# rainerzufalldererste/limg

Measured on AMD Instinct MI355X. Metric: encode Mpixels/s, 8K RGBA (limg_encode3d_test-equivalent: all 11 planes stored), higher is better.
Workload: dtype u8/i32 integer stage + f32 float stage (bit-exact vs the reference's strict SSE build)

## Files before the change

include/limg_hip_test_hooks.h:

```cpp
#ifndef LIMG_HIP_TEST_HOOKS_H
#define LIMG_HIP_TEST_HOOKS_H

#include "limg_hip.h"

#ifdef __cplusplus
extern "C" {
#endif

typedef struct limg_hip_test_options
{
  uint32_t struct_size;
  int32_t record_limit;
  int32_t batch_chunk;
  int32_t wg_per_cu;
  int32_t whole_image_ragged;
  int32_t pipeline;
  int32_t fail_chain_phase1;
  int32_t blocked_no_bound;
  int32_t lookback_spins;
  int32_t base_error_strip;
  int32_t skip_publish_strip;
  int32_t blocked_no_order;
  int32_t blocked_no_vec_store;
  int32_t resize_tile_pixels;
} limg_hip_test_options;

void limg_hip_default_test_options_sized(limg_hip_test_options *pOptions, size_t structSize);
static inline void limg_hip_default_test_options(limg_hip_test_options *pOptions) { limg_hip_default_test_options_sized(pOptions, sizeof(limg_hip_test_options)); }
limg_hip_result limg_hip_set_test_options(limg_hip_context *pCtx, const limg_hip_test_options *pOptions);

void limg_hip_test_live_resources(uint64_t out[5]);

#ifdef __cplusplus
}
#endif
#endif
```

limg_amd/__init__.py:

```python
import ctypes as C
import os

import numpy as np

HERE = os.path.dirname(os.path.abspath(__file__))
TEST_LIB_PATH = os.path.join(HERE, "liblimg_hip_test.so")
LIB_PATH = os.environ.get("LIMG_HIP_LIB") or os.path.join(HERE, "liblimg_hip.so")
if LIB_PATH == "test":
    LIB_PATH = TEST_LIB_PATH

P32 = ("pDecoded", "pShiftABCX", "pColAMin", "pColAMax", "pColBMin", "pColBMax", "pColCMin", "pColCMax")
P8 = ("pFactorsA", "pFactorsB", "pFactorsC")
PLANES = P32 + P8

ABI_SYMBOLS = (
    "limg_hip_init", "limg_hip_shutdown", "limg_hip_default_options_sized", "limg_hip_set_options", "limg_hip_get_options", "limg_hip_encode3d", "limg_hip_encode3d_perf",
    "limg_hip_encode3d_stats", "limg_hip_blocked_encode3d_stats",
    "limg_hip_encode3d_device", "limg_hip_encode3d_batch_device", "limg_hip_last_stats", "limg_hip_compare", "limg_hip_compare_device", "limg_hip_synth_random_gradient_device",
    "limg_hip_synth_photo_noise_device", "limg_hip_context_device_bytes", "limg_hip_version", "limg_hip_profile_begin", "limg_hip_profile_end",
    "limg_hip_host_noise_table", "limg_hip_noise_table_device", "limg_hip_host_chain_call", "limg_hip_host_chain_checkpoints", "limg_hip_host_dense_checkpoints", "limg_hip_host_partition", "limg_hip_check_device_status",
    "limg_hip_stream_bound", "limg_hip_encode_stream_device", "limg_hip_decode_stream_device", "limg_hip_encode_stream", "limg_hip_decode_stream",
    "limg_hip_stream_info", "limg_hip_encode_stream_batch_device", "limg_hip_encode_stream_batch",
    "limg_hip_stream_sizes_device", "limg_hip_stream_sizes", "limg_hip_encode_stream_budget_device", "limg_hip_encode_stream_budget",
    "limg_hip_encode_stream_budget_batch_device", "limg_hip_encode_stream_budget_batch",
    "limg_hip_blocked_stream_bound", "limg_hip_blocked_encode_stream_device", "limg_hip_blocked_decode_stream_device", "limg_hip_blocked_encode_stream",
    "limg_hip_blocked_decode_stream", "limg_hip_blocked_stream_info", "limg_hip_blocked_last_stream",
    "limg_hip_decode_stream_window_device", "limg_hip_blocked_decode_stream_window_device", "limg_hip_decode_stream_window", "limg_hip_blocked_decode_stream_window",
    "limg_hip_decode_stream_windows_device", "limg_hip_blocked_decode_stream_windows_device", "limg_hip_decode_stream_windows", "limg_hip_blocked_decode_stream_windows",
    "limg_hip_decode_stream_windows_tensor_device", "limg_hip_blocked_decode_stream_windows_tensor_device", "limg_hip_decode_stream_windows_tensor",
    "limg_hip_blocked_decode_stream_windows_tensor",
    "limg_hip_decode_stream_windows_scaled_device", "limg_hip_blocked_decode_stream_windows_scaled_device", "limg_hip_decode_stream_windows_scaled_tensor_device",
    "limg_hip_blocked_decode_stream_windows_scaled_tensor_device", "limg_hip_decode_stream_windows_scaled", "limg_hip_blocked_decode_stream_windows_scaled",
    "limg_hip_decode_stream_windows_scaled_tensor", "limg_hip_blocked_decode_stream_windows_scaled_tensor",
    "limg_hip_decode_stream_windows_resized_device", "limg_hip_blocked_decode_stream_windows_resized_device", "limg_hip_decode_stream_windows_resized_tensor_device",
    "limg_hip_blocked_decode_stream_windows_resized_tensor_device", "limg_hip_decode_stream_windows_resized", "limg_hip_blocked_decode_stream_windows_resized",
    "limg_hip_decode_stream_windows_resized_tensor", "limg_hip_blocked_decode_stream_windows_resized_tensor",
    "limg_hip_blocked_encode3d", "limg_hip_blocked_encode3d_device", "limg_hip_blocked_regions", "limg_hip_blocked_timing", "limg_hip_blocked_kernel_timing", "limg_hip_blocked_match_bits", "limg_hip_host_blocked_matches",
    "limg_hip_host_blocked_merge", "limg_hip_host_blocked_match_words", "limg_hip_host_blocked_match_bits",
    "limg_hip_comm_unique_id", "limg_hip_comm_init", "limg_hip_comm_destroy", "limg_hip_comm_info", "limg_hip_gather_stream", "limg_hip_encode3d_single_chain_device",
    "limg_hip_encode3d_chain_device", "limg_hip_host_gather_offsets", "limg_hip_host_chain_bases",
)
TEST_ABI_SYMBOLS = ("limg_hip_default_test_options_sized", "limg_hip_set_test_options", "limg_hip_test_live_resources")
COMM_ID_BYTES = 128

BLOCKED_PLANES = (("pDecoded", np.uint32), ("pFactorsA", np.uint8), ("pFactorsB", np.uint8), ("pFactorsC", np.uint8), ("pBlockError", np.uint8), ("pBitsPerPixel", np.uint8),
                  ("pShiftABCX", np.uint32), ("pColAMin", np.uint32), ("pColAMax", np.uint32), ("pColBMin", np.uint32), ("pColBMax", np.uint32), ("pColCMin", np.uint32),
                  ("pColCMax", np.uint32), ("pBlockIndex", np.uint32))
REGION_DTYPE = np.dtype([("ox", "<u4"), ("oy", "<u4"), ("rx", "<u4"), ("ry", "<u4")])

STREAM_HEADER_DTYPE = np.dtype([("magic", "<u4"), ("version", "<u4"), ("sizeX", "<u4"), ("sizeY", "<u4"), ("channels", "<u4"), ("errorFactor", "<u4"),
                                ("blocksX", "<u4"), ("blocksY", "<u4"), ("payloadWords", "<u8"), ("totalBytes", "<u8"), ("flags", "<u4"), ("reserved", "<u4", 3)])
STREAM_BLOCK_DTYPE = np.dtype([("dirA_min", "<i2", 4), ("dirA_max", "<i2", 4), ("dirB_offset", "<i2", 4), ("dirB_mag", "<i2", 4), ("dirC_offset", "<i2", 4),
                               ("dirC_mag", "<i2", 4), ("shift", "<u4"), ("payloadWord", "<u4")])

STREAM_VERSION_BLOCKED = 2
STREAM_FLAG_MERGED = 4
STREAM_RECT_DTYPE = np.dtype([("dirA_min", "<i2", 4), ("dirA_max", "<i2", 4), ("dirB_offset", "<i2", 4), ("dirB_mag", "<i2", 4), ("dirC_offset", "<i2", 4),
                              ("dirC_mag", "<i2", 4), ("shift", "<u4"), ("payloadWord", "<u4"), ("ox", "<u2"), ("oy", "<u2"), ("rx", "<u2"), ("ry", "<u2")])

RECORD_DTYPE = np.dtype([("avg", "<f4", 4), ("dirA_min", "<i2", 4), ("dirA_max", "<i2", 4), ("dirB_offset", "<i2", 4),
                         ("dirB_mag", "<i2", 4), ("dirC_offset", "<i2", 4), ("dirC_mag", "<i2", 4)])


class LimgHipError(RuntimeError):
    pass


class Info(C.Structure):
    _fields_ = [(k, C.c_void_p) for k in PLANES]


class CompactOut(C.Structure):
    _fields_ = [("pRecords", C.c_void_p), ("pShifts", C.c_void_p)]


class Window(C.Structure):
    _fields_ = [("x0", C.c_size_t), ("y0", C.c_size_t), ("width", C.c_size_t), ("height", C.c_size_t), ("pOut", C.c_void_p), ("outStridePixels", C.c_size_t)]


class WindowJob(C.Structure):
    _fields_ = [("pStream", C.c_void_p), ("streamBytes", C.c_size_t), ("sizeX", C.c_size_t), ("sizeY", C.c_size_t), ("window", Window)]


TENSOR_F32, TENSOR_F16 = 0, 1


class TensorFormat(C.Structure):
    _fields_ = [("type", C.c_uint32), ("planes", C.c_uint32), ("scale", C.c_float * 4), ("bias", C.c_float * 4)]


class TensorWindow(C.Structure):
    _fields_ = [("x0", C.c_size_t), ("y0", C.c_size_t), ("width", C.c_size_t), ("height", C.c_size_t), ("pOut", C.c_void_p), ("rowStride", C.c_size_t),
                ("planeStride", C.c_size_t)]


class TensorWindowJob(C.Structure):
    _fields_ = [("pStream", C.c_void_p), ("streamBytes", C.c_size_t), ("sizeX", C.c_size_t), ("sizeY", C.c_size_t), ("window", TensorWindow)]


class ScaledWindow(C.Structure):
    _fields_ = Window._fields_ + [("log2Scale", C.c_uint32)]


class ScaledWindowJob(C.Structure):
    _fields_ = [("pStream", C.c_void_p), ("streamBytes", C.c_size_t), ("sizeX", C.c_size_t), ("sizeY", C.c_size_t), ("window", ScaledWindow)]


class ScaledTensorWindow(C.Structure):
    _fields_ = TensorWindow._fields_ + [("log2Scale", C.c_uint32)]


class ScaledTensorWindowJob(C.Structure):
    _fields_ = [("pStream", C.c_void_p), ("streamBytes", C.c_size_t), ("sizeX", C.c_size_t), ("sizeY", C.c_size_t), ("window", ScaledTensorWindow)]


RESIZE_AUTO, RESIZE_FLIP_X = 0xFFFFFFFF, 1


class ResizedWindow(C.Structure):
    _fields_ = Window._fields_ + [("outWidth", C.c_size_t), ("outHeight", C.c_size_t), ("log2Scale", C.c_uint32), ("flags", C.c_uint32)]


class ResizedWindowJob(C.Structure):
    _fields_ = [("pStream", C.c_void_p), ("streamBytes", C.c_size_t), ("sizeX", C.c_size_t), ("sizeY", C.c_size_t), ("window", ResizedWindow)]


class ResizedTensorWindow(C.Structure):
    _fields_ = TensorWindow._fields_ + [("outWidth", C.c_size_t), ("outHeight", C.c_size_t), ("log2Scale", C.c_uint32), ("flags", C.c_uint32)]


class ResizedTensorWindowJob(C.Structure):
    _fields_ = [("pStream", C.c_void_p), ("streamBytes", C.c_size_t), ("sizeX", C.c_size_t), ("sizeY", C.c_size_t), ("window", ResizedTensorWindow)]


_WINDOW_TYPES = {(False, False): (Window, WindowJob), (False, True): (TensorWindow, TensorWindowJob),
                 (True, False): (ScaledWindow, ScaledWindowJob), (True, True): (ScaledTensorWindow, ScaledTensorWindowJob)}


def tensor_format(dtype, planes, scale, bias):
    name = str(dtype).split(".")[-1].replace("'>", "")
    assert name in ("float32", "float16"), dtype
    scale, bias = list(scale) + [1.0] * (4 - len(scale)), list(bias) + [0.0] * (4 - len(bias))
    return TensorFormat(TENSOR_F16 if name == "float16" else TENSOR_F32, planes, (C.c_float * 4)(*scale[:4]), (C.c_float * 4)(*bias[:4]))


class BudgetResult(C.Structure):
    _fields_ = [("struct_size", C.c_uint32), ("errorFactor", C.c_uint32), ("probes", C.c_uint32), ("withinBudget", C.c_uint32), ("bytes", C.c_uint64)]


class Options(C.Structure):
    _fields_ = [("struct_size", C.c_uint32), ("forced_shift", C.c_int32 * 3), ("force_split_kernels", C.c_int32), ("dither_pcg", C.c_int32), ("float_mode", C.c_int32),
                ("legacy_float_stage", C.c_int32), ("collect_stats", C.c_int32), ("host_noise_table", C.c_int32), ("batch_sub_images", C.c_int32), ("ragged_bands", C.c_int32),
                ("ragged_walk_threads", C.c_int32)]


class TestOptions(C.Structure):
    _fields_ = [("struct_size", C.c_uint32), ("record_limit", C.c_int32), ("batch_chunk", C.c_int32), ("wg_per_cu", C.c_int32), ("whole_image_ragged", C.c_int32),
                ("pipeline", C.c_int32), ("fail_chain_phase1", C.c_int32), ("blocked_no_bound", C.c_int32), ("lookback_spins", C.c_int32), ("base_error_strip", C.c_int32),
                ("skip_publish_strip", C.c_int32), ("blocked_no_order", C.c_int32), ("blocked_no_vec_store", C.c_int32), ("resize_tile_pixels", C.c_int32)]


def load_library(path=None):
    path = path or LIB_PATH
    if not os.path.exists(path):
        raise LimgHipError("%s not built: run `python -c 'import __graft_entry__ as g; g.build()'` (hipcc, gfx950). There is no CPU fallback." % path)
    try:
        import torch
    except ImportError:
        pass
    L = C.CDLL(path)
    L.limg_hip_version.restype = C.c_char_p
    L.limg_hip_init.restype = C.c_int
    L.limg_hip_init.argtypes = [C.c_int, C.POINTER(C.c_void_p)]
    L.limg_hip_shutdown.argtypes = [C.POINTER(C.c_void_p)]
    L.limg_hip_default_options_sized.argtypes = [C.c_void_p, C.c_size_t]
    if hasattr(L, "limg_hip_set_test_options"):
        L.limg_hip_default_test_options_sized.argtypes = [C.c_void_p, C.c_size_t]
        L.limg_hip_set_test_options.restype = C.c_int
        L.limg_hip_set_test_options.argtypes = [C.c_void_p, C.c_void_p]
        L.limg_hip_test_live_resources.restype = None
        L.limg_hip_test_live_resources.argtypes = [C.POINTER(C.c_uint64)]
    L.limg_hip_set_options.restype = C.c_int
    L.limg_hip_set_options.argtypes = [C.c_void_p, C.c_void_p]
    L.limg_hip_get_options.restype = C.c_int
    L.limg_hip_get_options.argtypes = [C.c_void_p, C.c_void_p]
    L.limg_hip_encode3d_stats.restype = C.c_int
    L.limg_hip_encode3d_stats.argtypes = [C.c_void_p, C.c_void_p, C.c_size_t, C.c_size_t, C.c_int, C.c_void_p, C.c_uint32, C.c_int, C.c_int, C.c_void_p, C.c_void_p]
    L.limg_hip_blocked_encode3d_stats.restype = C.c_int
    L.limg_hip_blocked_encode3d_stats.argtypes = [C.c_void_p, C.c_void_p, C.c_size_t, C.c_size_t, C.c_int, C.c_void_p, C.c_uint32, C.c_int, C.c_void_p, C.c_void_p]
    L.limg_hip_encode3d.restype = C.c_int
    L.limg_hip_encode3d.argtypes = [C.c_void_p, C.c_void_p, C.c_size_t, C.c_size_t, C.c_int, C.c_void_p, C.c_uint32, C.c_int, C.c_int]
    L.limg_hip_encode3d_perf.restype = C.c_int
    L.limg_hip_encode3d_perf.argtypes = [C.c_void_p, C.c_void_p, C.c_size_t, C.c_size_t, C.c_int, C.c_uint32, C.c_int, C.c_int]
    L.limg_hip_encode3d_device.restype = C.c_int
    L.limg_hip_encode3d_device.argtypes = [C.c_void_p, C.c_void_p, C.c_size_t, C.c_size_t, C.c_int, C.c_void_p, C.c_void_p, C.c_uint32, C.c_int, C.c_int, C.c_void_p]
    L.limg_hip_encode3d_batch_device.restype = C.c_int
    L.limg_hip_encode3d_batch_device.argtypes = [C.c_void_p, C.c_size_t, C.c_void_p, C.c_size_t, C.c_size_t, C.c_int, C.c_void_p, C.c_uint32, C.c_int, C.c_int, C.c_void_p]
    L.limg_hip_compare.restype = C.c_double
    L.limg_hip_compare.argtypes = [C.c_void_p, C.c_void_p, C.c_void_p, C.c_size_t, C.c_size_t, C.c_int, C.c_void_p, C.c_void_p]
    L.limg_hip_compare_device.restype = C.c_double
    L.limg_hip_compare_device.argtypes = [C.c_void_p, C.c_void_p, C.c_void_p, C.c_size_t, C.c_size_t, C.c_int, C.c_void_p, C.c_void_p, C.c_void_p]
    L.limg_hip_synth_random_gradient_device.restype = C.c_int
    L.limg_hip_synth_random_gradient_device.argtypes = [C.c_void_p, C.c_size_t, C.c_size_t, C.c_uint64, C.c_int, C.c_size_t, C.c_void_p]
    L.limg_hip_synth_photo_noise_device.restype = C.c_int
    L.limg_hip_synth_photo_noise_device.argtypes = [C.c_void_p, C.c_size_t, C.c_size_t, C.c_uint64, C.c_size_t, C.c_void_p]
    L.limg_hip_profile_begin.restype = C.c_int
    L.limg_hip_profile_begin.argtypes = [C.c_void_p]
    L.limg_hip_profile_end.restype = C.c_int
    L.limg_hip_profile_end.argtypes = [C.c_void_p, C.c_void_p, C.c_int]
    L.limg_hip_check_device_status.restype = C.c_int
    L.limg_hip_check_device_status.argtypes = [C.c_void_p]
    L.limg_hip_host_noise_table.restype = C.c_int
    L.limg_hip_host_noise_table.argtypes = [C.c_void_p, C.c_size_t]
    L.limg_hip_last_stats.restype = C.c_int
    L.limg_hip_last_stats.argtypes = [C.c_void_p, C.c_void_p, C.c_void_p]
    L.limg_hip_noise_table_device.restype = C.c_int
    L.limg_hip_noise_table_device.argtypes = [C.c_void_p, C.c_void_p, C.c_size_t, C.c_void_p]
    L.limg_hip_host_chain_call.restype = C.c_uint64
    L.limg_hip_host_chain_call.argtypes = [C.c_uint64, C.c_size_t, C.c_void_p, C.c_int]
    L.limg_hip_host_chain_checkpoints.restype = C.c_uint64
    L.limg_hip_host_chain_checkpoints.argtypes = [C.c_size_t, C.c_size_t, C.c_void_p, C.c_int]
    L.limg_hip_host_dense_checkpoints.restype = C.c_int
    L.limg_hip_host_dense_checkpoints.argtypes = [C.c_size_t, C.c_size_t, C.c_void_p]
    L.limg_hip_host_partition.restype = C.c_int
    L.limg_hip_host_partition.argtypes = [C.c_size_t, C.c_int, C.POINTER(C.c_uint32), C.POINTER(C.c_uint32)]
    L.limg_hip_context_device_bytes.restype = C.c_size_t
    L.limg_hip_context_device_bytes.argtypes = [C.c_void_p]
    L.limg_hip_blocked_encode3d.restype = C.c_int
    L.limg_hip_blocked_encode3d.argtypes = [C.c_void_p, C.c_void_p, C.c_size_t, C.c_size_t, C.c_int, C.c_void_p, C.c_uint32, C.c_int]
    L.limg_hip_blocked_encode3d_device.restype = C.c_int
    L.limg_hip_blocked_encode3d_device.argtypes = [C.c_void_p, C.c_void_p, C.c_size_t, C.c_size_t, C.c_int, C.c_void_p, C.c_uint32, C.c_int, C.c_void_p]
    L.limg_hip_blocked_regions.restype = C.c_int
    L.limg_hip_blocked_regions.argtypes = [C.c_void_p, C.c_void_p, C.c_size_t, C.POINTER(C.c_size_t)]
    L.limg_hip_blocked_timing.restype = C.c_int
    L.limg_hip_blocked_timing.argtypes = [C.c_void_p, C.c_void_p]
    L.limg_hip_blocked_match_bits.restype = C.c_int
    L.limg_hip_blocked_match_bits.argtypes = [C.c_void_p, C.c_void_p, C.c_size_t, C.POINTER(C.c_size_t)]
    L.limg_hip_blocked_kernel_timing.restype = C.c_int
    L.limg_hip_blocked_kernel_timing.argtypes = [C.c_void_p, C.c_void_p]
    L.limg_hip_host_blocked_matches.restype = C.c_int
    L.limg_hip_host_blocked_matches.argtypes = [C.c_int, C.c_void_p, C.c_void_p]
    L.limg_hip_host_blocked_merge.restype = C.c_int
    L.limg_hip_host_blocked_merge.argtypes = [C.c_void_p, C.c_void_p, C.c_size_t, C.c_size_t, C.c_int, C.c_void_p, C.c_size_t, C.POINTER(C.c_size_t)]
    L.limg_hip_host_blocked_match_words.restype = C.c_size_t
    L.limg_hip_host_blocked_match_bits.restype = C.c_int
    L.limg_hip_host_blocked_match_bits.argtypes = [C.c_void_p, C.c_size_t, C.c_size_t, C.c_int, C.c_void_p]
    L.limg_hip_stream_bound.restype = C.c_size_t
    L.limg_hip_stream_bound.argtypes = [C.c_size_t, C.c_size_t]
    L.limg_hip_encode_stream_device.restype = C.c_int
    L.limg_hip_encode_stream_device.argtypes = [C.c_void_p, C.c_void_p, C.c_size_t, C.c_size_t, C.c_int, C.c_void_p, C.c_size_t, C.POINTER(C.c_size_t), C.c_uint32, C.c_int, C.c_int,
                                                C.c_void_p]
    L.limg_hip_decode_stream_device.restype = C.c_int
    L.limg_hip_decode_stream_device.argtypes = [C.c_void_p, C.c_void_p, C.c_size_t, C.c_void_p, C.c_size_t, C.c_size_t, C.c_void_p]
    L.limg_hip_encode_stream.restype = C.c_int
    L.limg_hip_encode_stream.argtypes = [C.c_void_p, C.c_void_p, C.c_size_t, C.c_size_t, C.c_int, C.c_void_p, C.c_size_t, C.POINTER(C.c_size_t), C.c_uint32, C.c_int, C.c_int]
    L.limg_hip_decode_stream.restype = C.c_int
    L.limg_hip_decode_stream.argtypes = [C.c_void_p, C.c_void_p, C.c_size_t, C.c_void_p, C.c_size_t]
    L.limg_hip_stream_info.restype = C.c_int
    L.limg_hip_stream_info.argtypes = [C.c_void_p, C.c_size_t, C.POINTER(C.c_size_t), C.POINTER(C.c_size_t), C.POINTER(C.c_int), C.POINTER(C.c_size_t)]
    L.limg_hip_encode_stream_batch_device.restype = C.c_int
    L.limg_hip_encode_stream_batch_device.argtypes = [C.c_void_p, C.c_size_t, C.c_void_p, C.c_size_t, C.c_size_t, C.c_int, C.c_void_p, C.c_size_t, C.c_void_p, C.c_uint32, C.c_int,
                                                      C.c_int, C.c_void_p]
    L.limg_hip_encode_stream_batch.restype = C.c_int
    L.limg_hip_encode_stream_batch.argtypes = [C.c_void_p, C.c_size_t, C.c_void_p, C.c_size_t, C.c_size_t, C.c_int, C.c_void_p, C.c_size_t, C.c_void_p, C.c_uint32, C.c_int, C.c_int]
    L.limg_hip_stream_sizes_device.restype = C.c_int
    L.limg_hip_stream_sizes_device.argtypes = [C.c_void_p, C.c_void_p, C.c_size_t, C.c_size_t, C.c_int, C.c_void_p, C.c_size_t, C.c_void_p, C.c_int, C.c_int, C.c_void_p]
    L.limg_hip_stream_sizes.restype = C.c_int
    L.limg_hip_stream_sizes.argtypes = [C.c_void_p, C.c_void_p, C.c_size_t, C.c_size_t, C.c_int, C.c_void_p, C.c_size_t, C.c_void_p, C.c_int, C.c_int]
    L.limg_hip_encode_stream_budget_device.restype = C.c_int
    L.limg_hip_encode_stream_budget_device.argtypes = [C.c_void_p, C.c_void_p, C.c_size_t, C.c_size_t, C.c_int, C.c_void_p, C.c_size_t, C.c_size_t, C.c_uint32, C.c_uint32, C.c_int,
                                                       C.c_int, C.c_void_p, C.c_void_p]
    L.limg_hip_encode_stream_budget.restype = C.c_int
    L.limg_hip_encode_stream_budget.argtypes = [C.c_void_p, C.c_void_p, C.c_size_t, C.c_size_t, C.c_int, C.c_void_p, C.c_size_t, C.c_size_t, C.c_uint32, C.c_uint32, C.c_int, C.c_int,
                                                C.c_void_p]
    L.limg_hip_encode_stream_budget_batch_device.restype = C.c_int
    L.limg_hip_encode_stream_budget_batch_device.argtypes = [C.c_void_p, C.c_size_t, C.c_void_p, C.c_size_t, C.c_size_t, C.c_int, C.c_void_p, C.c_size_t, C.c_void_p, C.c_uint32,
                                                             C.c_uint32, C.c_int, C.c_int, C.c_void_p, C.c_void_p]
    L.limg_hip_encode_stream_budget_batch.restype = C.c_int
    L.limg_hip_encode_stream_budget_batch.argtypes = [C.c_void_p, C.c_size_t, C.c_void_p, C.c_size_t, C.c_size_t, C.c_int, C.c_void_p, C.c_size_t, C.c_void_p, C.c_uint32, C.c_uint32,
                                                      C.c_int, C.c_int, C.c_void_p]
    L.limg_hip_blocked_stream_bound.restype = C.c_size_t
    L.limg_hip_blocked_stream_bound.argtypes = [C.c_size_t, C.c_size_t]
    L.limg_hip_blocked_encode_stream_device.restype = C.c_int
    L.limg_hip_blocked_encode_stream_device.argtypes = [C.c_void_p, C.c_void_p, C.c_size_t, C.c_size_t, C.c_int, C.c_void_p, C.c_size_t, C.POINTER(C.c_size_t), C.c_uint32, C.c_int,
                                                        C.c_void_p]
    L.limg_hip_blocked_decode_stream_device.restype = C.c_int
    L.limg_hip_blocked_decode_stream_device.argtypes = [C.c_void_p, C.c_void_p, C.c_size_t, C.c_void_p, C.c_size_t, C.c_size_t, C.c_void_p]
    L.limg_hip_blocked_encode_stream.restype = C.c_int
    L.limg_hip_blocked_encode_stream.argtypes = [C.c_void_p, C.c_void_p, C.c_size_t, C.c_size_t, C.c_int, C.c_void_p, C.c_size_t, C.POINTER(C.c_size_t), C.c_uint32, C.c_int]
    L.limg_hip_blocked_decode_stream.restype = C.c_int
    L.limg_hip_blocked_decode_stream.argtypes = [C.c_void_p, C.c_void_p, C.c_size_t, C.c_void_p, C.c_size_t]
    P, Z = C.c_void_p, C.c_size_t
    for args, names in (
            ([P, P, Z] + [Z] * 6 + [P, Z, P], ("window_device",)),
            ([P, P, Z] + [Z] * 4 + [P, Z], ("window",)),
            ([P, P, Z, P, P], ("windows_device", "windows_scaled_device", "windows_resized_device")),
            ([P, P, Z, P, Z], ("windows", "windows_scaled", "windows_resized")),
            ([P, P, Z, P, P, P], ("windows_tensor_device", "windows_scaled_tensor_device", "windows_resized_tensor_device")),
            ([P, P, Z, P, Z, P], ("windows_tensor", "windows_scaled_tensor", "windows_resized_tensor"))):
        for name in names:
            for version in ("limg_hip_decode_stream_", "limg_hip_blocked_decode_stream_"):
                getattr(L, version + name).restype = C.c_int
                getattr(L, version + name).argtypes = args
    L.limg_hip_blocked_last_stream.restype = C.c_int
    L.limg_hip_blocked_last_stream.argtypes = [C.c_void_p, C.c_void_p, C.c_size_t, C.POINTER(C.c_size_t)]
    L.limg_hip_blocked_stream_info.restype = C.c_int
    L.limg_hip_blocked_stream_info.argtypes = [C.c_void_p, C.c_size_t, C.POINTER(C.c_size_t), C.POINTER(C.c_size_t), C.POINTER(C.c_int), C.POINTER(C.c_size_t),
                                               C.POINTER(C.c_size_t)]
    L.limg_hip_comm_unique_id.restype = C.c_int
    L.limg_hip_comm_unique_id.argtypes = [C.c_void_p]
    L.limg_hip_comm_init.restype = C.c_int
    L.limg_hip_comm_init.argtypes = [C.c_void_p, C.c_void_p, C.c_int, C.c_int]
    L.limg_hip_comm_info.restype = C.c_int
    L.limg_hip_comm_info.argtypes = [C.c_void_p, C.POINTER(C.c_int), C.POINTER(C.c_int), C.POINTER(C.c_int)]
    L.limg_hip_comm_destroy.restype = C.c_int
    L.limg_hip_comm_destroy.argtypes = [C.c_void_p]
    L.limg_hip_gather_stream.restype = C.c_int
    L.limg_hip_gather_stream.argtypes = [C.c_void_p, C.c_void_p, C.c_size_t, C.c_int, C.c_void_p, C.c_size_t, C.c_void_p, C.c_void_p]
    L.limg_hip_encode3d_single_chain_device.restype = C.c_int
    L.limg_hip_encode3d_single_chain_device.argtypes = [C.c_void_p, C.c_void_p, C.c_size_t, C.c_size_t, C.c_int, C.c_void_p, C.c_uint32, C.c_int, C.c_size_t, C.c_void_p]
    L.limg_hip_encode3d_chain_device.restype = C.c_int
    L.limg_hip_encode3d_chain_device.argtypes = [C.c_void_p, C.c_void_p, C.c_size_t, C.c_size_t, C.c_int, C.c_void_p, C.c_uint32, C.c_int, C.c_int, C.c_void_p, C.c_void_p, C.c_size_t,
                                                 C.c_void_p]
    L.limg_hip_host_gather_offsets.restype = C.c_int
    L.limg_hip_host_gather_offsets.argtypes = [C.c_void_p, C.c_int, C.c_void_p]
    L.limg_hip_host_chain_bases.restype = C.c_int
    L.limg_hip_host_chain_bases.argtypes = [C.c_void_p, C.c_int, C.c_void_p]
    return L


def _check(r, what):
    if r != 0:
        raise LimgHipError("%s failed with limg_hip_result %d" % (what, r))


def _np_ptr(a):
    return a.ctypes.data_as(C.c_void_p)


def live_resources(lib):
    out = (C.c_uint64 * 5)()
    lib.limg_hip_test_live_resources(out)
    return tuple(int(v) for v in out)


def stream_info(stream, lib=None):
    lib = lib or load_library()
    stream = np.ascontiguousarray(stream, dtype=np.uint8)
    sx, sy, tb, ha = C.c_size_t(0), C.c_size_t(0), C.c_size_t(0), C.c_int(0)
    _check(lib.limg_hip_stream_info(_np_ptr(stream), stream.size, C.byref(sx), C.byref(sy), C.byref(ha), C.byref(tb)), "limg_hip_stream_info")
    return sx.value, sy.value, bool(ha.value), tb.value


def blocked_stream_bound(w, h, lib=None):
    return (lib or load_library()).limg_hip_blocked_stream_bound(w, h)


def blocked_stream_info(stream, lib=None):
    lib = lib or load_library()
    stream = np.ascontiguousarray(stream, dtype=np.uint8)
    sx, sy, tb, nr, ha = C.c_size_t(0), C.c_size_t(0), C.c_size_t(0), C.c_size_t(0), C.c_int(0)
    _check(lib.limg_hip_blocked_stream_info(_np_ptr(stream), stream.size, C.byref(sx), C.byref(sy), C.byref(ha), C.byref(tb), C.byref(nr)), "limg_hip_blocked_stream_info")
    return sx.value, sy.value, bool(ha.value), tb.value, nr.value


def host_gather_offsets(sizes, lib=None):
    lib = lib or load_library()
    sizes = np.ascontiguousarray(sizes, dtype=np.uint64)
    out = np.zeros(sizes.size + 1, dtype=np.uint64)
    _check(lib.limg_hip_host_gather_offsets(_np_ptr(sizes), sizes.size, _np_ptr(out)), "limg_hip_host_gather_offsets")
    return out


def host_chain_bases(calls, lib=None):
    lib = lib or load_library()
    calls = np.ascontiguousarray(calls, dtype=np.uint64)
    out = np.zeros(calls.size, dtype=np.uint64)
    _check(lib.limg_hip_host_chain_bases(_np_ptr(calls), calls.size, _np_ptr(out)), "limg_hip_host_chain_bases")
    return out


def host_blocked_matches(channels, seed, cand, lib=None):
    lib = lib or load_library()
    a = np.ascontiguousarray(seed); b = np.ascontiguousarray(cand)
    return bool(lib.limg_hip_host_blocked_matches(channels, _np_ptr(a), _np_ptr(b)))


def host_blocked_merge(fits, channels, use_bits=True, lib=None):
    lib = lib or load_library()
    fits = np.ascontiguousarray(fits)
    by, bx = fits.shape
    bits = None
    if use_bits:
        bits = np.zeros(by * bx * lib.limg_hip_host_blocked_match_words(), dtype=np.uint64)
        _check(lib.limg_hip_host_blocked_match_bits(_np_ptr(fits), bx, by, channels, _np_ptr(bits)), "limg_hip_host_blocked_match_bits")
    out = np.zeros(by * bx, dtype=REGION_DTYPE)
    n = C.c_size_t(0)
    _check(lib.limg_hip_host_blocked_merge(_np_ptr(fits), _np_ptr(bits) if bits is not None else None, bx, by, channels, _np_ptr(out), out.size, C.byref(n)), "limg_hip_host_blocked_merge")
    return out[:n.value].copy()


class LimgHip:

    def __init__(self, device=-1, lib_path=None):
        self.lib = load_library(lib_path)
        self.ctx = C.c_void_p()
        self.comm_rank, self.comm_world = 0, 1
        _check(self.lib.limg_hip_init(device, C.byref(self.ctx)), "limg_hip_init")

    def close(self):
        if self.ctx:
            self.lib.limg_hip_shutdown(C.byref(self.ctx))
            self.ctx = C.c_void_p()

    def __del__(self):
        try:
            self.close()
        except Exception:
            pass

    def set_options(self, forced_shift=None, force_split=False, dither_pcg=False, float_fast=False, legacy_float_stage=False, host_noise_table=False, collect_stats=False,
                    batch_sub_images=0, ragged_bands=0, ragged_walk_threads=0, **test_hooks):
        o = Options()
        self.lib.limg_hip_default_options_sized(C.byref(o), C.sizeof(o))
        if forced_shift is not None:
            for i in range(3):
                o.forced_shift[i] = int(forced_shift[i])
        o.force_split_kernels = int(force_split)
        o.dither_pcg = int(dither_pcg)
        o.float_mode = 1 if float_fast else 0
        o.legacy_float_stage = int(legacy_float_stage)
        o.host_noise_table = int(host_noise_table)
        o.collect_stats = int(collect_stats)
        o.batch_sub_images = int(batch_sub_images)
        o.ragged_bands = int(ragged_bands)
        o.ragged_walk_threads = int(ragged_walk_threads)
        _check(self.lib.limg_hip_set_options(self.ctx, C.byref(o)), "limg_hip_set_options")
        hooks = {}
        for k, v in test_hooks.items():
            if not k.startswith("test_") or k[5:] not in dict(TestOptions._fields_):
                raise TypeError("set_options: unknown option %r" % k)
            hooks[k[5:]] = int(v)
        if self.has_test_hooks:
            t = TestOptions()
            self.lib.limg_hip_default_test_options_sized(C.byref(t), C.sizeof(t))
            for k, v in hooks.items():
                setattr(t, k, v)
            _check(self.lib.limg_hip_set_test_options(self.ctx, C.byref(t)), "limg_hip_set_test_options")
        elif any(hooks.values()):
            raise LimgHipError("test hooks %s need liblimg_hip_test.so (LIMG_HIP_LIB=test); the product library has none" % sorted(k for k, v in hooks.items() if v))

    @property
    def has_test_hooks(self):
        return hasattr(self.lib, "limg_hip_set_test_options")

    def get_options(self):
        o = Options()
        o.struct_size = C.sizeof(o)
        _check(self.lib.limg_hip_get_options(self.ctx, C.byref(o)), "limg_hip_get_options")
        return o

    def set_forced_shift(self, shift=None):
        self.set_options(forced_shift=shift)

    def encode3d(self, img, has_alpha, error_factor=100, pool_threads=0, fast=True):
        img = np.ascontiguousarray(img, dtype=np.uint32)
        h, w = img.shape
        out = {k: np.zeros((h, w), dtype=np.uint32) for k in P32}
        out.update({k: np.zeros((h, w), dtype=np.uint8) for k in P8})
        info = Info(*[out[k].ctypes.data for k in PLANES])
        _check(self.lib.limg_hip_encode3d(self.ctx, _np_ptr(img), w, h, int(has_alpha), C.byref(info), error_factor, pool_threads, int(fast)), "limg_hip_encode3d")
        return out

    def encode3d_stats(self, img, has_alpha, error_factor=100, pool_threads=0, fast=True):
        img = np.ascontiguousarray(img, dtype=np.uint32)
        h, w = img.shape
        out = {k: np.zeros((h, w), dtype=np.uint32) for k in P32}
        out.update({k: np.zeros((h, w), dtype=np.uint8) for k in P8})
        info = Info(*[out[k].ctypes.data for k in PLANES])
        cnt = np.zeros(30, dtype=np.uint64)
        px = C.c_uint64(0)
        _check(self.lib.limg_hip_encode3d_stats(self.ctx, _np_ptr(img), w, h, int(has_alpha), C.byref(info), error_factor, pool_threads, int(fast), _np_ptr(cnt), C.byref(px)),
               "limg_hip_encode3d_stats")
        return out, cnt, px.value

    def encode3d_perf(self, img, has_alpha, error_factor=100, pool_threads=0, fast=True):
        img = np.ascontiguousarray(img, dtype=np.uint32)
        h, w = img.shape
        _check(self.lib.limg_hip_encode3d_perf(self.ctx, _np_ptr(img), w, h, int(has_alpha), error_factor, pool_threads, int(fast)), "limg_hip_encode3d_perf")

    def compare(self, a, b, has_alpha):
        a = np.ascontiguousarray(a, dtype=np.uint32)
        b = np.ascontiguousarray(b, dtype=np.uint32)
        mse, mx = C.c_double(), C.c_double()
        p = self.lib.limg_hip_compare(self.ctx, _np_ptr(a), _np_ptr(b), a.shape[1], a.shape[0], int(has_alpha), C.byref(mse), C.byref(mx))
        return p, mse.value

    @staticmethod
    def _stream():
        import torch
        return C.c_void_p(torch.cuda.current_stream().cuda_stream)

    def alloc_planes_device(self, w, h, device="cuda"):
        import torch
        d = {k: torch.empty((h, w), dtype=torch.int32, device=device) for k in P32}
        d.update({k: torch.empty((h, w), dtype=torch.uint8, device=device) for k in P8})
        return d

    def encode3d_device(self, img, has_alpha, planes=None, error_factor=100, pool_threads=0, fast=True, records=None, shifts=None):
        h, w = img.shape
        info = None
        if planes is not None:
            info = Info(*[(planes[k].data_ptr() if k in planes else None) for k in PLANES])
        comp = None
        if records is not None or shifts is not None:
            comp = CompactOut(records.data_ptr() if records is not None else None, shifts.data_ptr() if shifts is not None else None)
        _check(self.lib.limg_hip_encode3d_device(self.ctx, C.c_void_p(img.data_ptr()), w, h, int(has_alpha), C.byref(info) if info else None,
                                                 C.byref(comp) if comp else None, error_factor, pool_threads, int(fast), self._stream()), "limg_hip_encode3d_device")

    def encode3d_batch_device(self, imgs, has_alpha, planes_list, error_factor=100, pool_threads=0, fast=True):
        n = len(imgs)
        h, w = imgs[0].shape
        assert all(tuple(i.shape) == (h, w) for i in imgs) and len(planes_list) == n
        ins = (C.c_void_p * n)(*[i.data_ptr() for i in imgs])
        infos = (Info * n)(*[Info(*[(pl[k].data_ptr() if k in pl else None) for k in PLANES]) for pl in planes_list])
        _check(self.lib.limg_hip_encode3d_batch_device(self.ctx, n, ins, w, h, int(has_alpha), infos, error_factor, pool_threads, int(fast), self._stream()),
               "limg_hip_encode3d_batch_device")

    def last_stats(self):
        out = np.zeros(30, dtype=np.uint64)
        px = C.c_uint64(0)
        _check(self.lib.limg_hip_last_stats(self.ctx, _np_ptr(out), C.byref(px)), "limg_hip_last_stats")
        return out, px.value

    def compare_device(self, a, b, has_alpha):
        mse, mx = C.c_double(), C.c_double()
        h, w = a.shape
        p = self.lib.limg_hip_compare_device(self.ctx, C.c_void_p(a.data_ptr()), C.c_void_p(b.data_ptr()), w, h, int(has_alpha), C.byref(mse), C.byref(mx), self._stream())
        return p, mse.value

    def synth_device(self, kind, w, h, seed=1, opaque=True, y0=0, device="cuda"):
        import torch
        out = torch.empty((h, w), dtype=torch.int32, device=device)
        if kind == "random_gradient":
            _check(self.lib.limg_hip_synth_random_gradient_device(C.c_void_p(out.data_ptr()), w, h, seed, int(opaque), y0, self._stream()), "synth")
        elif kind == "photo_noise":
            _check(self.lib.limg_hip_synth_photo_noise_device(C.c_void_p(out.data_ptr()), w, h, seed, y0, self._stream()), "synth")
        else:
            raise ValueError(kind)
        return out

    def blocked_encode3d(self, img, has_alpha, error_factor=100, fast=True):
        img = np.ascontiguousarray(img, dtype=np.uint32)
        h, w = img.shape
        out = {k: np.zeros((h, w), dtype=t) for k, t in BLOCKED_PLANES}
        info = (C.c_void_p * 14)(*[out[k].ctypes.data for k, _ in BLOCKED_PLANES])
        _check(self.lib.limg_hip_blocked_encode3d(self.ctx, _np_ptr(img), w, h, int(has_alpha), info, error_factor, int(fast)), "limg_hip_blocked_encode3d")
        out["regions"] = self.blocked_regions()
        return out

    def blocked_encode3d_device(self, img, has_alpha, planes, error_factor=100, fast=True):
        h, w = img.shape
        info = (C.c_void_p * 14)(*[(planes[k].data_ptr() if k in planes else None) for k, _ in BLOCKED_PLANES])
        _check(self.lib.limg_hip_blocked_encode3d_device(self.ctx, C.c_void_p(img.data_ptr()), w, h, int(has_alpha), info, error_factor, int(fast), self._stream()),
               "limg_hip_blocked_encode3d_device")

    def alloc_blocked_planes_device(self, w, h, device="cuda"):
        import torch
        return {k: torch.empty((h, w), dtype=(torch.int32 if t == np.uint32 else torch.uint8), device=device) for k, t in BLOCKED_PLANES if k != "pBlockError"}

    def blocked_regions(self):
        n = C.c_size_t(0)
        _check(self.lib.limg_hip_blocked_regions(self.ctx, None, 0, C.byref(n)), "limg_hip_blocked_regions")
        out = np.zeros(n.value, dtype=REGION_DTYPE)
        _check(self.lib.limg_hip_blocked_regions(self.ctx, _np_ptr(out), out.size, C.byref(n)), "limg_hip_blocked_regions")
        return out

    def blocked_timing(self):
        ms = np.zeros(6, dtype=np.float64)
        _check(self.lib.limg_hip_blocked_timing(self.ctx, _np_ptr(ms)), "limg_hip_blocked_timing")
        return dict(zip(("pass1_match_gpu", "merge_host", "fit_search_gpu", "chain_host", "store_gpu", "total"), ms.tolist()))

    def blocked_match_bits(self):
        n = C.c_size_t(0)
        _check(self.lib.limg_hip_blocked_match_bits(self.ctx, None, 0, C.byref(n)), "limg_hip_blocked_match_bits")
        out = np.zeros(n.value, dtype=np.uint64)
        _check(self.lib.limg_hip_blocked_match_bits(self.ctx, _np_ptr(out), out.size, C.byref(n)), "limg_hip_blocked_match_bits")
        return out

    def blocked_kernel_timing(self):
        ms = np.zeros(4, dtype=np.float64)
        _check(self.lib.limg_hip_blocked_kernel_timing(self.ctx, _np_ptr(ms)), "limg_hip_blocked_kernel_timing")
        return dict(zip(("pass1_kernel", "match_kernels", "fit_search_kernel", "expand_store_kernels"), ms.tolist()))

    def _stream_call(self, name, *args):
        _check(getattr(self.lib, name)(self.ctx, *args), name)

    def _encode_stream(self, name, cap, img, has_alpha, opts):
        img = np.ascontiguousarray(img, dtype=np.uint32)
        h, w = img.shape
        out = np.zeros(cap(w, h), dtype=np.uint8)
        n = C.c_size_t(0)
        self._stream_call(name, _np_ptr(img), w, h, int(has_alpha), _np_ptr(out), out.size, C.byref(n), *opts)
        return out[:n.value].copy()

    def _decode_stream(self, name, stream, w, h):
        stream = np.ascontiguousarray(stream, dtype=np.uint8)
        out = np.zeros((h, w), dtype=np.uint32)
# ... 454 lines not shown
```

limg_amd/csrc/limg_hip_api.hip:

```cpp
#include "limg_hip_context.h"

#include <math.h>

using namespace limg_hip;

namespace limg_hip
{
  void mark(limg_hip_context *c, hipStream_t stream)
  {
    if (!c->enc.profiling) return;
    if (c->enc.events.ensure(c->enc.eventsUsed + 1, hipEventDefault) != limg_hip_success) return;
    (void)hipEventRecord(c->enc.events[c->enc.eventsUsed++], stream);
  }
}

extern "C"
{
  const char *limg_hip_version(void) { return "limg_hip 0.1 (gfx950)"; }

  void limg_hip_default_options_sized(limg_hip_options *o, size_t structSize)
  {
    if (!o || structSize < sizeof(uint32_t)) return;
    limg_hip_options d;
    memset(&d, 0, sizeof(d));
    d.forced_shift[0] = d.forced_shift[1] = d.forced_shift[2] = -1;
    const size_t n = structSize < sizeof(d) ? structSize : sizeof(d);
    d.struct_size = (uint32_t)n;
    memcpy(o, &d, n);
  }

#ifdef LIMG_HIP_TEST_HOOKS
  void limg_hip_default_test_options_sized(limg_hip_test_options *o, size_t structSize)
  {
    if (!o || structSize < sizeof(uint32_t)) return;
    limg_hip_test_options d;
    memset(&d, 0, sizeof(d));
    const size_t n = structSize < sizeof(d) ? structSize : sizeof(d);
    d.struct_size = (uint32_t)n;
    memcpy(o, &d, n);
  }

  limg_hip_result limg_hip_set_test_options(limg_hip_context *c, const limg_hip_test_options *o)
  {
    if (!c || !o) return limg_hip_error_ArgumentNull;
    const size_t n = o->struct_size;
    if (n < sizeof(uint32_t) || (n & 3u) != 0) return limg_hip_error_InvalidParameter;
    limg_hip_test_options full;
    limg_hip_default_test_options_sized(&full, sizeof(full));
    memcpy(&full, o, n < sizeof(full) ? n : sizeof(full));
    full.struct_size = (uint32_t)sizeof(full);
    c->topt = full;
    return limg_hip_success;
  }

  void limg_hip_test_live_resources(uint64_t out[5])
  {
    for (int i = 0; out && i < limg_hip_live::kCounts; i++) out[i] = limg_hip_live::count[i].load();
  }
#endif

  limg_hip_result limg_hip_init(int device, limg_hip_context **ppCtx)
  {
    if (!ppCtx) return limg_hip_error_ArgumentNull;
    *ppCtx = nullptr;
    int count = 0;
    if (hipGetDeviceCount(&count) != hipSuccess || count == 0)
    {
      fprintf(stderr, "limg_hip: no HIP device available -- this library has no CPU fallback\n");
      return limg_hip_error_Generic;
    }
    if (device < 0) HIP_TRY(hipGetDevice(&device));
    if (device >= count) return limg_hip_error_InvalidParameter;
    HIP_TRY(hipSetDevice(device));
    limg_hip_context *c = new (std::nothrow) limg_hip_context();
    if (!c) return limg_hip_error_MemoryAllocationFailure;
    c->device = device;
    hipDeviceProp_t prop;
    if (hipGetDeviceProperties(&prop, device) == hipSuccess && prop.multiProcessorCount > 0) c->enc.persistentWorkgroups = 5 * prop.multiProcessorCount;
    limg_hip_default_options_sized(&c->opt, sizeof(c->opt));
#ifdef LIMG_HIP_TEST_HOOKS
    limg_hip_default_test_options_sized(&c->topt, sizeof(c->topt));
#endif
    *ppCtx = c;
    return limg_hip_success;
  }

  void limg_hip_shutdown(limg_hip_context **ppCtx)
  {
    if (!ppCtx || !*ppCtx) return;
    delete *ppCtx;
    *ppCtx = nullptr;
  }

  limg_hip_result limg_hip_set_options(limg_hip_context *c, const limg_hip_options *o)
  {
    if (!c || !o) return limg_hip_error_ArgumentNull;
    const size_t n = o->struct_size;
    if (n < offsetof(limg_hip_options, forced_shift) + sizeof(o->forced_shift) || (n & 3u) != 0) return limg_hip_error_InvalidParameter;
    limg_hip_options full;
    limg_hip_default_options_sized(&full, sizeof(full));
    memcpy(&full, o, n < sizeof(full) ? n : sizeof(full));
    full.struct_size = (uint32_t)sizeof(full);
    c->opt = full;
    return limg_hip_success;
  }

  limg_hip_result limg_hip_get_options(const limg_hip_context *c, limg_hip_options *o)
  {
    if (!c || !o) return limg_hip_error_ArgumentNull;
    size_t n = o->struct_size;
    if (n < sizeof(uint32_t) || (n & 3u) != 0) return limg_hip_error_InvalidParameter;
    if (n > sizeof(c->opt)) n = sizeof(c->opt);
    memcpy(o, &c->opt, n);
    o->struct_size = (uint32_t)n;
    return limg_hip_success;
  }

  limg_hip_result limg_hip_check_device_status(limg_hip_context *c)
  {
    if (!c) return limg_hip_error_ArgumentNull;
    HIP_TRY(hipSetDevice(c->device));
    HIP_TRY(hipDeviceSynchronize());
    if (c->enc.devStatus.p)
    {
      uint32_t word = 0;
      HIP_TRY(hipMemcpy(&word, c->enc.devStatus.p, 4, hipMemcpyDeviceToHost));
      if (word != 0)
      {
        HIP_TRY(hipMemset(c->enc.devStatus.p, 0, 4));
        fprintf(stderr, "limg_hip: look-back timeout in the fused encode kernel\n");
        return limg_hip_error_Generic;
      }
      HIP_TRY(hipMemcpy(&word, (const uint8_t *)c->enc.devStatus.p + 4, 4, hipMemcpyDeviceToHost));
      if (word != 0)
      {
        HIP_TRY(hipMemset((uint8_t *)c->enc.devStatus.p + 4, 0, 4));
        fprintf(stderr, "limg_hip: a rank of the communicator aborted a single-chain encode; this rank's planes of that encode were not written\n");
        return limg_hip_error_Generic;
      }
    }
    if (c->stream.status.p)
    {
      uint32_t word = 0;
      HIP_TRY(hipMemcpy(&word, c->stream.status.p, 4, hipMemcpyDeviceToHost));
      if (word != 0)
      {
        HIP_TRY(hipMemset(c->stream.status.p, 0, 4));
        fprintf(stderr, "limg_hip: stream refused by the decode kernel (%s)\n", (word & 1u) ? "header mismatch" : "inconsistent payload offsets");
        return limg_hip_error_InvalidParameter;
      }
    }
    return limg_hip_success;
  }

  limg_hip_result limg_hip_last_stats(limg_hip_context *c, uint64_t *pCounters30, uint64_t *pPixels)
  {
    if (!c || !pCounters30) return limg_hip_error_ArgumentNull;
    std::lock_guard<std::recursive_mutex> hostLock(c->hostEntry);
    if (c->stats.state == 0) return limg_hip_error_InvalidParameter;
    if (c->stats.state == 1)
    {
      HIP_TRY(hipSetDevice(c->device));
      HIP_TRY(hipMemcpyAsync(c->stats.host, c->stats.counters.p, 30 * 8, hipMemcpyDeviceToHost, c->stats.stream));
      HIP_TRY(hipStreamSynchronize(c->stats.stream));
      c->stats.state = 2;
    }
    memcpy(pCounters30, c->stats.host, 30 * 8);
    if (pPixels) *pPixels = c->stats.pixels;
    return limg_hip_success;
  }

  limg_hip_result limg_hip_profile_begin(limg_hip_context *c)
  {
    if (!c) return limg_hip_error_ArgumentNull;
    c->enc.profiling = true;
    c->enc.eventsUsed = 0;
    return limg_hip_success;
  }

  int limg_hip_profile_end(limg_hip_context *c, float *pMs, int maxEncodes)
  {
    if (!c || !pMs) return -1;
    c->enc.profiling = false;
    const int n = (int)(c->enc.eventsUsed / 4);
    int written = 0;
    for (int i = 0; i < n && i < maxEncodes; i++, written++)
    {
      if (hipEventSynchronize(c->enc.events[4 * i + 3]) != hipSuccess) return -1;
      for (int k = 0; k < 3; k++)
        if (hipEventElapsedTime(&pMs[3 * i + k], c->enc.events[4 * i + k], c->enc.events[4 * i + k + 1]) != hipSuccess) return -1;
    }
    c->enc.eventsUsed = 0;
    return written;
  }

  size_t limg_hip_context_device_bytes(const limg_hip_context *c)
  {
    return c ? c->deviceBytes.load(std::memory_order_relaxed) : 0;
  }

  double limg_hip_compare_device(limg_hip_context *c, const uint32_t *a, const uint32_t *b, size_t sizeX, size_t sizeY, int hasAlpha, double *pMse, double *pMax, void *stream)
  {
    if (!c || !a || !b || sizeX == 0 || sizeY == 0) return NAN;
    if (hipSetDevice(c->device) != hipSuccess) return NAN;
    if (c->enc.cmp.ensure(8) != limg_hip_success) return NAN;
    hipStream_t s = (hipStream_t)stream;
    if (hipMemsetAsync(c->enc.cmp.p, 0, 8, s) != hipSuccess) return NAN;
    launch_compare(a, b, (uint64_t)sizeX * sizeY, hasAlpha ? 4 : 3, (unsigned long long *)c->enc.cmp.p, s);
    unsigned long long err = 0;
    if (hipMemcpyAsync(&err, c->enc.cmp.p, 8, hipMemcpyDeviceToHost, s) != hipSuccess || hipStreamSynchronize(s) != hipSuccess) return NAN;
// ... 35 lines not shown
```

limg_amd/csrc/limg_hip_context.h:

```cpp
#ifndef LIMG_HIP_CONTEXT_H
#define LIMG_HIP_CONTEXT_H

#include "limg_hip_internal.h"
#include "limg_hip_owned.h"
#ifdef LIMG_HIP_TEST_HOOKS
#include "../../include/limg_hip_test_hooks.h"
#define TOPT(c, member) ((c)->topt.member)
#else
#define TOPT(c, member) 0
#endif
#include "limg_hip_rccl.h"

#include <stddef.h>
#include <string.h>
#include <new>
#include <mutex>
#include <thread>

struct limg_hip_context
{
  std::recursive_mutex hostEntry;
  int device = 0;
  limg_hip_options opt;
#ifdef LIMG_HIP_TEST_HOOKS
  limg_hip_test_options topt;
#endif
  typedef std::atomic<size_t> Bytes;
  Bytes deviceBytes{ 0 };
  struct Encode
  {
    Bytes &n;
    DevBuf records{ n }, shifts{ n }, stripCalls{ n }, stripBase{ n };
    DevBuf invN{ n };
    DevBuf park{ n };
    DevBuf batchTable{ n };
    Stream fitStream;
    Events pipeEvents;
    DevBuf lookback{ n };
    DevBuf accTable{ n };
    DevBuf devStatus{ n };
    DevBuf cmp{ n };
    int persistentWorkgroups = 1280;
    bool profiling = false;
    Events events;
    size_t eventsUsed = 0;
  } enc{ deviceBytes };
  struct Noise
  {
    Bytes &n;
    DevBuf table{ n };
    bool pcg = false;
    size_t count = 0;
    uint64_t next = limg_hip::kDitherSeed;
    DevBuf dyn{ n };
    DevBuf states{ n };
    DevBuf ck{ n };
    size_t ckCount = 0;
    std::vector<uint64_t> ckHost;
  } noise{ deviceBytes };
  struct Stats
  {
    Bytes &n;
    DevBuf counters{ n };
    hipStream_t stream = nullptr;
    int state = 0;
    bool accumulate = false;
    uint64_t host[30] = { 0 };
    uint64_t pixels = 0;
  } stats{ deviceBytes };
  struct Chain
  {
    Bytes &n;
    ncclComm_t comm = nullptr;
    int rank = 0, world = 1;
    DevBuf words{ n };
    const void *in = nullptr;
    size_t x = 0, y = 0, before = 0;
    const void *fac[3] = { nullptr, nullptr, nullptr };
    int alpha = 0, fast = 0;
    uint32_t ef = 0;
  } chain{ deviceBytes };
  struct Host
  {
    Bytes &n;
    DevBuf in{ n }, planes{ n };
    Stream copyStream;
    Stream stream;
    Events events;
    DevBuf words{ n };
    HostBuf stage;
    Event stageEvent;
    bool stageBusy = false;
    Events raggedEvents;
  } host{ deviceBytes };
  struct Blocked
  {
    Bytes &n;
    DevBuf flags{ n }, bound{ n };
    DevBuf order{ n };
    DevBuf match{ n }, regions{ n }, out{ n }, px{ n }, fac{ n }, noise{ n }, noiseBase{ n };
    DevBuf calls{ n };
    HostBuf hFlags, hRec, hBits, hDesc, hOut, hNoise, hNoiseBase;
    Stream searchStream;
    Stream storeStream;
    Stream copyStream;
    Events workEvents;
    Events bandEvents;
    std::vector<limg_hip::HostRegion> lastRegions;
    std::vector<uint32_t> regionPx;
    size_t lastBlocks = 0;
    double ms[6] = { 0, 0, 0, 0, 0, 0 };
    double kernelMs[4] = { 0, 0, 0, 0 };
    Events workTimers;
    size_t scratchCap = 0;
    struct { size_t sizeX = 0, sizeY = 0; int channels = 0; uint32_t errorFactor = 0, flags = 0; bool valid = false; } last;
  } blocked{ deviceBytes };
  struct Streams
  {
    Bytes &n;
    DevBuf fac{ n }, tiles{ n }, units{ n }, status{ n }, buf{ n };
    DevBuf rateState{ n }, rateCounter{ n }, rateList{ n };
    DevBuf table{ n }, sizes{ n };
    DevBuf bsUnits{ n }, bsTiles{ n }, bsMap{ n }, bsState{ n };
    Events packTimers;
    bool packTimed = false;
  } stream{ deviceBytes };
  struct WindowSlot { HostBuf host; DevBuf dev; Event done; bool busy = false; WindowSlot(Bytes &n) : dev(n) {} };
  static constexpr unsigned kWindowSlots = 4;
  struct { WindowSlot slots[kWindowSlots]; unsigned next = 0; } window{ { deviceBytes, deviceBytes, deviceBytes, deviceBytes } };

  ~limg_hip_context()
  {
    (void)hipSetDevice(device);
    (void)hipDeviceSynchronize();
    if (chain.comm && limg_hip::rccl().ok) (void)limg_hip::rccl().CommDestroy(chain.comm);
  }
};

namespace limg_hip
{
  uint64_t chain_call(uint64_t h, unsigned n, uint8_t *noise64, bool forceSoft, bool pcg);
  uint64_t fill_noise_table(uint64_t h, uint8_t *noise, size_t count, bool pcg);
  uint64_t chain_checkpoints(uint64_t h, size_t calls, size_t every, uint64_t *pOut, bool pcg);
  void chain_walk_rows(uint64_t &h, size_t &call, uint32_t by0, uint32_t by1, uint32_t blocksX, uint32_t stripsX, size_t sizeX, size_t sizeY, uint32_t chainCount, uint32_t chainRows,
                       const uint32_t *shifts, uint32_t *stripBase, unsigned long long *states, uint8_t *pixels, size_t maxCalls, bool pcg);
  size_t chain_walk_blocks(uint64_t h0, uint32_t blocksX, uint32_t blocksY, uint32_t stripsX, size_t sizeX, size_t sizeY, uint32_t chainCount, uint32_t chainRows, const uint32_t *shifts,
                           uint32_t *stripBase, unsigned long long *states, uint8_t *pixels, size_t maxCalls, bool pcg);

  size_t checkpoint_reach();
  bool dense_checkpoints_host(size_t first, size_t count, uint64_t *pOut);
  limg_hip_result ensure_checkpoints(limg_hip_context *c, size_t calls);
  limg_hip_result grow_noise_table(limg_hip_context *c, size_t entries, hipStream_t stream);
  bool chain_value_at(uint64_t calls, uint64_t *pValue);

  void mark(limg_hip_context *c, hipStream_t stream);

  template <class F>
  void run_on_threads(unsigned n, F &&work) noexcept
  {
    std::thread *pool = n > 1 ? new (std::nothrow) std::thread[n - 1] : nullptr;
    unsigned started = 0;
    if (pool)
      for (; started < n - 1; started++)
      {
        try { pool[started] = std::thread(work, started + 1); }
        catch (...) { break; }
      }
    work(0u);
    for (unsigned t = started + 1; t < n; t++) work(t);
    for (unsigned t = 0; t < started; t++) pool[t].join();
    delete[] pool;
  }

  inline int32_t record_limit(const limg_hip_context *c) { return TOPT(c, record_limit) > 0 ? TOPT(c, record_limit) - 1 : 2700; }
  inline size_t list_chunk(const limg_hip_context *c, size_t blocks, size_t strips) { return list_chunk(blocks, strips, TOPT(c, batch_chunk) > 0 ? (size_t)TOPT(c, batch_chunk) : 0); }

  int device_cus(const limg_hip_context *c);
  limg_hip_result stream_total_bytes(const uint8_t *dStream, hipStream_t s, size_t *pBytes);
  limg_hip_result download_stream(limg_hip_context *c, size_t bytes, uint8_t *pStream, size_t capacity, size_t *pBytes);
  template <class ENCODE>
  limg_hip_result encode_stream_host(limg_hip_context *c, const uint32_t *pIn, size_t sizeX, size_t sizeY, uint8_t *pStream, size_t capacity, size_t *pBytes, size_t bound,
                                     ENCODE &&deviceEncode)
  {
    if (bound == 0) return limg_hip_error_InvalidParameter;
    HIP_TRY(hipSetDevice(c->device));
    limg_hip_result r;
// ... 62 lines not shown
```

limg_amd/csrc/limg_hip_encode.hip:

```cpp
#include "limg_hip_context.h"
#include "limg_search_table_accurate.h"

using namespace limg_hip;

namespace limg_hip
{
  Partition partition(size_t sizeY, int poolThreads)
  {
    Partition pt = { 1, 0 };
    if (poolThreads <= 0) return pt;
    size_t thread_count = (size_t)poolThreads * 4;
    size_t y_range = ((sizeY / kBlock) / thread_count) * kBlock;
    if (y_range == 0)
    {
      thread_count = (size_t)poolThreads;
      y_range = ((sizeY / kBlock) / thread_count) * kBlock;
    }
    if (y_range == 0) return pt;
    pt.chainCount = (uint32_t)thread_count;
    pt.chainRows = (uint32_t)(y_range / kBlock);
    return pt;
  }

  limg_hip_result encode_stats(const EncodeJob &e)
  {
    limg_hip_context *const c = e.c;
    const EncodeParams &p = e.p;
    if (!e.wantStats || e.x.inner) return limg_hip_success;
    limg_hip_result rs;
    if ((rs = c->stats.counters.ensure(30 * 8)) != limg_hip_success) return rs;
    if (!c->stats.accumulate) HIP_TRY(hipMemsetAsync(c->stats.counters.p, 0, 30 * 8, e.stream));
    launch_shift_stats(p.shifts, p.blocksX, p.blocksY, p.blocksY * p.batchCount, p.sizeX, p.sizeY, (unsigned long long *)c->stats.counters.p, e.stream);
    c->stats.stream = e.stream; c->stats.state = 1;
    c->stats.pixels = (c->stats.accumulate ? c->stats.pixels : 0) + (uint64_t)e.sizeX * e.sizeY * e.x.batchCount;
    return limg_hip_success;
  }
}

namespace
{
  limg_hip_result ensure_accurate_table(limg_hip_context *c)
  {
    if (c->enc.accTable.p) return limg_hip_success;
    static const uint32_t compact[LIMG_SEARCH_ACC_STATES][2] = LIMG_SEARCH_ACC_TABLE_INIT;
    static const uint32_t mul[9] = { 1, 2, 4, 8, 17, 36, 85, 255, 256 };
    std::vector<uint32_t> wide((size_t)LIMG_SEARCH_ACC_STATES * 8);
    for (size_t i = 0; i < (size_t)LIMG_SEARCH_ACC_STATES; i++)
    {
      const uint32_t w0 = compact[i][0], w1 = compact[i][1];
      uint32_t *e = &wide[i * 8];
      if (w0 >> 31) { e[0] = 1u << 31; continue; }
      const uint32_t a = w0 & 15u, b = (w0 >> 4) & 15u, cc = (w0 >> 8) & 15u;
      e[0] = a | ((w0 & 0x1000u) ? 0x20u : 0u);
      e[1] = (w1 & 0xFFFFu) * 32u; e[2] = (w1 >> 16) * 32u;
      e[3] = b; e[4] = cc;
      e[5] = mul[a]; e[6] = mul[b]; e[7] = mul[cc];
    }
    static_assert((size_t)LIMG_SEARCH_ACC_STATES * 32u < (1u << 24), "offsets leave bits 24..26 free");
    for (size_t i = 0; i < (size_t)LIMG_SEARCH_ACC_STATES; i++)
    {
      uint32_t *e = &wide[i * 8];
      if (e[0] >> 31) continue;
      for (int k = 1; k <= 2; k++)
      {
        const uint32_t *n = &wide[(e[k] / 32u) * 8];
        uint32_t mask = 0;
        if (!(n[0] >> 31)) mask = ((n[0] & 31u) != (e[0] & 31u) ? 1u : 0u) | (n[3] != e[3] ? 2u : 0u) | (n[4] != e[4] ? 4u : 0u);
        e[k] |= mask << 24;
      }
    }
    limg_hip_result r = c->enc.accTable.ensure(wide.size() * 4);
    if (r != limg_hip_success) return r;
    if (hipMemcpy(c->enc.accTable.p, wide.data(), wide.size() * 4, hipMemcpyHostToDevice) != hipSuccess) { c->enc.accTable.release(); return limg_hip_error_Generic; }
    return limg_hip_success;
  }

  limg_hip_result encode_height_ragged(limg_hip_context *c, const uint32_t *dIn, size_t sizeX, size_t sizeY, int hasAlpha, const limg_hip_encode3d_info *dInfo,
                                       const limg_hip_compact_out *compact, uint32_t errorFactor, int poolThreads, int fast, hipStream_t stream, const EncodeExtra &x);

  limg_hip_result encode_params(EncodeJob &e, const uint32_t *dIn, const limg_hip_compact_out *compact, uint32_t errorFactor, int poolThreads, int fast)
  {
    limg_hip_context *const c = e.c;
    const EncodeExtra &x = e.x;
    const limg_hip_encode3d_info *const dInfo = e.dInfo;
    const size_t sizeX = e.sizeX, sizeY = e.sizeY, batchCount = x.batchCount;
    const ImageIO *const batch = x.batch;
    EncodeParams &p = e.p;
    memset(&p, 0, sizeof(p));
    p.io.in = dIn;
    p.sizeX = (uint32_t)sizeX; p.sizeY = (uint32_t)sizeY;
    p.blocksX = (uint32_t)((sizeX + kBlock - 1) / kBlock);
    p.blocksY = (uint32_t)((sizeY + kBlock - 1) / kBlock);
    p.stripsX = (p.blocksX + kStripBlocks - 1) / kStripBlocks;
    const Thresholds t = thresholds(errorFactor);
    p.maxPixel32 = t.maxPixel32; p.maxBlock = t.maxBlock; p.blockLimitFull = t.blockLimitFull; p.crushBits = (int32_t)t.crushBits;
    p.fast = fast != 0;
    p.accTable = nullptr;
    if (!p.fast && p.crushBits)
    {
      limg_hip_result ra = ensure_accurate_table(c);
      if (ra != limg_hip_success) return ra;
      p.accTable = (const uint32_t *)c->enc.accTable.p;
    }
    forced_shifts(c->opt.forced_shift, p.forced);
    p.floatFast = (c->opt.float_mode == 1 && (!x.fitOnly || x.fitFloatMode)) ? 1 : 0;
    p.recordLimit = record_limit(c);
    const Partition pt = e.pt = x.part ? *x.part : partition(sizeY, poolThreads);
    p.chainCount = pt.chainCount; p.chainRows = pt.chainRows;

    p.batchCount = (uint32_t)batchCount;
    p.imageStrips = p.stripsX * p.blocksY;
    e.blocks = (size_t)p.blocksX * p.blocksY * batchCount; e.strips = (size_t)p.stripsX * p.blocksY * batchCount;
    const size_t scratchRows = x.scratchRows > (size_t)p.blocksY * batchCount ? x.scratchRows : (size_t)p.blocksY * batchCount;
    const size_t scratchBlocks = scratchRows * p.blocksX, scratchStrips = scratchRows * p.stripsX;
    const size_t blockOff = x.scratchRow0 * p.blocksX, stripOff = x.scratchRow0 * p.stripsX;
    limg_hip_result r;
    if (compact && compact->pRecords) p.records = compact->pRecords + blockOff;
    else { if ((r = c->enc.records.ensure(scratchBlocks * sizeof(limg_hip_block_record))) != limg_hip_success) return r; p.records = (limg_hip_block_record *)c->enc.records.p + blockOff; }
    if (compact && compact->pShifts) p.shifts = compact->pShifts + blockOff;
    else { if ((r = c->enc.shifts.ensure(scratchBlocks * 4)) != limg_hip_success) return r; p.shifts = (uint32_t *)c->enc.shifts.p + blockOff; }
    if ((r = c->enc.invN.ensure(scratchBlocks * 16)) != limg_hip_success) return r;
    p.invN = (float *)c->enc.invN.p + blockOff * 4;
    if ((r = c->enc.stripCalls.ensure(scratchStrips * 4)) != limg_hip_success) return r;
    if ((r = c->enc.stripBase.ensure(scratchStrips * 4)) != limg_hip_success) return r;
    p.stripCalls = (uint32_t *)c->enc.stripCalls.p + stripOff; p.stripBase = (uint32_t *)c->enc.stripBase.p + stripOff;
    const bool fullPlanes = e.fullPlanes;
    p.storePlanes = dInfo != nullptr;
    p.fullPlanes = fullPlanes;
    p.streamRaw = x.streamRaw && !fullPlanes;
    p.stripWords = (x.streamRaw && !fullPlanes) ? x.stripWords : nullptr;
    p.fitOnly = x.fitOnly && !dInfo;
    if (dInfo) p.io.info = *dInfo;
    p.vecIn = (sizeX % 4 == 0) && (((uintptr_t)dIn) & 15u) == 0;
    p.vecPlanes = 0;
    if (dInfo && fullPlanes && sizeX % 4 == 0)
    {
      uintptr_t bits = 0;
      const void *const *pp = reinterpret_cast<const void *const *>(dInfo);
      for (int i = 1; i < 8; i++) bits |= (uintptr_t)pp[i];
      p.vecPlanes = (bits & 15u) == 0;
    }
    p.vecFactors8 = dInfo && (sizeX % 8 == 0) && ((((uintptr_t)dInfo->pFactorsA) | ((uintptr_t)dInfo->pFactorsB) | ((uintptr_t)dInfo->pFactorsC)) & 7u) == 0;
    p.vecDecoded = dInfo && fullPlanes && (sizeX % 4 == 0) && (((uintptr_t)dInfo->pDecoded) & 15u) == 0;
    p.vecFactors = dInfo && (sizeX % 16 == 0) && ((((uintptr_t)dInfo->pFactorsA) | ((uintptr_t)dInfo->pFactorsB) | ((uintptr_t)dInfo->pFactorsC)) & 15u) == 0;
    if (batchCount > 1)
    {
      for (size_t i = 1; i < batchCount; i++)
      {
        uintptr_t bits = 0;
        const void *const *pp = reinterpret_cast<const void *const *>(&batch[i].info);
        for (int k = 1; k < 8; k++) bits |= (uintptr_t)pp[k];
        p.vecPlanes = p.vecPlanes && (bits & 15u) == 0;
        p.vecIn = p.vecIn && (((uintptr_t)batch[i].in) & 15u) == 0;
        p.vecDecoded = p.vecDecoded && (((uintptr_t)batch[i].info.pDecoded) & 15u) == 0;
        p.vecFactors8 = p.vecFactors8 && ((((uintptr_t)batch[i].info.pFactorsA) | ((uintptr_t)batch[i].info.pFactorsB) | ((uintptr_t)batch[i].info.pFactorsC)) & 7u) == 0;
        p.vecFactors = p.vecFactors && ((((uintptr_t)batch[i].info.pFactorsA) | ((uintptr_t)batch[i].info.pFactorsB) | ((uintptr_t)batch[i].info.pFactorsC)) & 15u) == 0;
      }
      if ((r = c->enc.batchTable.ensure(batchCount * sizeof(ImageIO))) != limg_hip_success) return r;
      launch_set_batch_table((ImageIO *)c->enc.batchTable.p, batch, batchCount, e.stream);
      p.batch = (const ImageIO *)c->enc.batchTable.p;
    }

    if (dInfo && !e.ragged)
    {
      uint32_t maxRows = p.blocksY;
      if (pt.chainCount > 1 && (pt.chainCount - 1) * pt.chainRows < p.blocksY) maxRows = p.blocksY - (pt.chainCount - 1) * pt.chainRows;
      if ((r = grow_noise_table(c, ((size_t)maxRows * p.blocksX + x.chainBlocksBefore) * 3, e.stream)) != limg_hip_success) return r;
      p.noise = (const uint8_t *)c->noise.table.p;
      p.noiseLast = (uint32_t)(c->noise.count - 1);
    }

    const int chainPhase = x.chainPhase;
    if (chainPhase != 0 && (e.ragged || !dInfo || poolThreads != 0)) return limg_hip_error_InvalidParameter;
    p.chainCallsOut = chainPhase == 1 ? x.dChainCalls : nullptr;
    p.chainBase = chainPhase == 2 ? x.dChainBase : nullptr;
    p.prefit = (!e.ragged && c->opt.legacy_float_stage == 0 && (((uintptr_t)p.records) & 15u) == 0) ? 1 : 0;
    e.fused = dInfo != nullptr && !e.ragged && (c->opt.force_split_kernels == 0 || batchCount > 1) && chainPhase == 0;
    e.wantStats = c->opt.collect_stats != 0 && dInfo != nullptr && chainPhase == 0;
    return limg_hip_success;
  }

  limg_hip_result fused_scratch(EncodeJob &e, const limg_hip_compact_out *compact)
  {
    limg_hip_context *const c = e.c;
    EncodeParams &p = e.p;
    limg_hip_result r;
    if ((r = c->enc.lookback.ensure(16 * (e.x.batchCount + 1) + e.strips * 8)) != limg_hip_success) return r;
    p.ticket = (uint32_t *)c->enc.lookback.p;
    p.desc = (unsigned long long *)((uint8_t *)c->enc.lookback.p + 16);
    p.zeroLookback = p.prefit ? 1 : 0;
    if (!p.prefit) HIP_TRY(hipMemsetAsync(c->enc.lookback.p, 0, 16 + e.strips * 8, e.stream));
    if (!c->enc.devStatus.p)
    {
      if ((r = c->enc.devStatus.ensure(16)) != limg_hip_success) return r;
      HIP_TRY(hipMemsetAsync(c->enc.devStatus.p, 0, 16, e.stream));
    }
    p.timeout = (uint32_t *)c->enc.devStatus.p;
#ifdef LIMG_HIP_TEST_HOOKS
    p.lookbackSpins = c->topt.lookback_spins > 0 ? (uint32_t)c->topt.lookback_spins : (1u << 22);
    p.testSkipStrip = c->topt.skip_publish_strip > 0 ? (uint32_t)c->topt.skip_publish_strip - 1u : ~0u;
    p.testBaseErrStrip = c->topt.base_error_strip > 0 ? (uint32_t)c->topt.base_error_strip - 1u : ~0u;
#endif
    p.compactOut = compact != nullptr || e.wantStats;
    if ((r = c->enc.park.ensure((size_t)(c->enc.persistentWorkgroups / 5 * 6) * 2 * 8192)) != limg_hip_success) return r;
    p.park = (uint8_t *)c->enc.park.p;
    return limg_hip_success;
  }

  int wg_per_cu(const limg_hip_context *c, int deflt)
  {
    const int t = TOPT(c, wg_per_cu);
    return (t >= 1 && t < deflt) ? t : deflt;
  }

  size_t sub_batch_images(const EncodeJob &e)
  {
    const limg_hip_options &o = e.c->opt;
    if (!e.fused || e.x.batchCount <= 1 || !e.p.prefit) return 0;
    if (o.batch_sub_images > 0) return (size_t)o.batch_sub_images;
    if (o.batch_sub_images == 0) return e.x.batchCount >= 32 ? 8 : (e.x.batchCount >= 16 ? 4 : 0);
    return 0;
  }

  limg_hip_result encode_sub_batches(EncodeJob &e, size_t subImages)
  {
    limg_hip_context *const c = e.c;
    const EncodeParams &p = e.p;
    const size_t batchCount = e.x.batchCount;
    const hipStream_t stream = e.stream;
    const uint32_t knobs = (uint32_t)TOPT(c, pipeline);
    const int fitPrio = (knobs & 15u) ? (int)(knobs & 15u) - 1 : 0, wgOverlapRaw = ((knobs >> 4) & 15u) ? (int)((knobs >> 4) & 15u) : 5,
              wgOverlap = wgOverlapRaw > 6 ? 6 : wgOverlapRaw;
    const size_t firstSub = ((knobs >> 8) & 255u) && ((knobs >> 8) & 255u) < subImages ? (size_t)((knobs >> 8) & 255u) : subImages;
    const size_t nSub = 1 + (batchCount - firstSub + subImages - 1) / subImages;
    limg_hip_result r;
    hipStream_t fs;
    if ((r = c->enc.fitStream.get(fs)) != limg_hip_success) return r;
    if ((r = c->enc.pipeEvents.ensure(2 * nSub + 1, hipEventDisableTiming)) != limg_hip_success) return r;
    const size_t imgBlocks = (size_t)p.blocksX * p.blocksY, imgStrips = (size_t)p.imageStrips;
    auto sub = [&](size_t k) -> EncodeParams
    {
      EncodeParams q = p;
      const size_t i0 = k == 0 ? 0 : firstSub + (k - 1) * subImages, want = k == 0 ? firstSub : subImages, n = batchCount - i0 < want ? batchCount - i0 : want;
      q.batch = p.batch + i0; q.batchCount = (uint32_t)n;
      q.io = e.x.batch[i0];
      q.records = p.records + i0 * imgBlocks; q.shifts = p.shifts + i0 * imgBlocks; q.invN = p.invN + i0 * imgBlocks * 4;
      if (p.stripWords) q.stripWords = p.stripWords + i0 * imgStrips;
      uint8_t *lb = (uint8_t *)c->enc.lookback.p + k * 16 + i0 * imgStrips * 8;
      q.ticket = (uint32_t *)lb; q.desc = (unsigned long long *)(lb + 16);
      q.fitPrio = k == 0 ? 0 : fitPrio;
      return q;
    };
    hipEvent_t *ev = c->enc.pipeEvents.data();
    e.mark_if(1);
    HIP_TRY(hipEventRecord(ev[0], stream));
    HIP_TRY(hipStreamWaitEvent(fs, ev[0], 0));
    launch_fit_tpb(sub(0), e.channels, fs);
    HIP_TRY(hipEventRecord(ev[1], fs));
    for (size_t k = 0; k < nSub; k++)
    {
      HIP_TRY(hipStreamWaitEvent(stream, ev[1 + 2 * k], 0));
      if (k == 0) e.mark_if(1);
      if (k + 1 < nSub)
      {
        HIP_TRY(hipEventRecord(ev[2 + 2 * k], stream));
        HIP_TRY(hipStreamWaitEvent(fs, ev[2 + 2 * k], 0));
        launch_fit_tpb(sub(k + 1), e.channels, fs);
        HIP_TRY(hipEventRecord(ev[3 + 2 * k], fs));
      }
      launch_encode_persistent(sub(k), e.channels, c->enc.persistentWorkgroups / 5 * (k + 1 < nSub ? wgOverlap : wg_per_cu(c, 6)), stream);
    }
    e.mark_if(1); e.mark_if(2);
    HIP_TRY(hipGetLastError());
    return encode_stats(e);
  }

  limg_hip_result encode_fused(EncodeJob &e)
  {
    const EncodeParams &p = e.p;
    if (p.prefit)
    {
      e.mark_if(1);
      launch_fit_tpb(p, e.channels, e.stream);
    }
    e.mark_if(1);
    launch_encode_persistent(p, e.channels, e.c->enc.persistentWorkgroups / 5 * wg_per_cu(e.c, p.prefit ? 6 : 5), e.stream);
    e.mark_if(1);
    if (p.prefit) e.mark_if(2); else { e.mark_if(1); e.mark_if(2); }
    HIP_TRY(hipGetLastError());
    return encode_stats(e);
  }

  limg_hip_result encode_chain_phase2(EncodeJob &e)
  {
    mark(e.c, e.stream);
    launch_dither_store(e.p, e.channels, e.stream);
    mark(e.c, e.stream);
    HIP_TRY(hipGetLastError());
    return limg_hip_success;
  }

  limg_hip_result encode_split(EncodeJob &e)
  {
    const EncodeParams &p = e.p;
    if (p.prefit)
    {
      e.mark_if(1);
      launch_fit_tpb(p, e.channels, e.stream);
      if (p.fitOnly)
      {
        e.mark_if(1); e.mark_if(1); e.mark_if(2);
        HIP_TRY(hipGetLastError());
        return limg_hip_success;
      }
    }
    else e.mark_if(1);
    launch_fit_search(p, e.channels, e.stream);
    if (e.x.chainPhase != 1) e.mark_if(1);
    if (!e.dInfo)
    {
      e.mark_if(1); e.mark_if(2);
      HIP_TRY(hipGetLastError());
      return limg_hip_success;
    }
    launch_strip_scan(p, e.stream);
    if (e.x.chainPhase == 1)
    {
      mark(e.c, e.stream);
      HIP_TRY(hipGetLastError());
      return limg_hip_success;
    }
    e.mark_if(1);
    launch_dither_store(p, e.channels, e.stream);
    e.mark_if(2);
    HIP_TRY(hipGetLastError());
    return encode_stats(e);
  }
}

namespace limg_hip
{
  limg_hip_result encode_device(limg_hip_context *c, const uint32_t *dIn, size_t sizeX, size_t sizeY, int hasAlpha, const limg_hip_encode3d_info *dInfo,
                                const limg_hip_compact_out *compact, uint32_t errorFactor, int poolThreads, int fast, hipStream_t stream, const EncodeExtra &x)
  {
    const int chainPhase = x.chainPhase;
    const size_t batchCount = x.batchCount;
    if (!c || !dIn) return limg_hip_error_ArgumentNull;
    if (chainPhase == 0 && !x.inner) c->chain.in = nullptr;
    if (sizeX == 0 || sizeY == 0 || sizeX > 0x7FFFFFF8ull || sizeY > 0x7FFFFFF8ull) return limg_hip_error_InvalidParameter;
    bool fullPlanes = true;
    if (dInfo)
    {
      const void *const *pp = reinterpret_cast<const void *const *>(dInfo);
      int n32 = 0;
      for (int i = 0; i < 8; i++) n32 += pp[i] != nullptr;
      for (int i = 8; i < 11; i++)
        if (!pp[i]) return limg_hip_error_ArgumentNull;
      if (n32 != 0 && n32 != 8) return limg_hip_error_ArgumentNull;
      fullPlanes = n32 == 8;
    }
    HIP_TRY(hipSetDevice(c->device));
    const bool ragged = (sizeX % kBlock) != 0 || (sizeY % kBlock) != 0;
    if (ragged && sizeX % kBlock == 0 && sizeY > (size_t)kBlock && dInfo && chainPhase == 0 && batchCount == 1 && !x.inner && !x.fitOnly && c->opt.force_split_kernels == 0 &&
        c->opt.legacy_float_stage == 0 && c->opt.dither_pcg == 0 && TOPT(c, whole_image_ragged) == 0)
    {
      if (((sizeX / kBlock) * ((sizeY + kBlock - 1) / kBlock)) * 3 <= checkpoint_reach())
        return encode_height_ragged(c, dIn, sizeX, sizeY, hasAlpha, dInfo, compact, errorFactor, poolThreads, fast, stream, x);
    }

    EncodeJob e = { c, stream, x, dInfo, sizeX, sizeY };
    e.channels = hasAlpha ? 4 : 3;
    e.ragged = ragged;
    e.fullPlanes = fullPlanes;
    limg_hip_result r;
    if ((r = encode_params(e, dIn, compact, errorFactor, poolThreads, fast)) != limg_hip_success) return r;
    if (chainPhase == 0 && !x.inner && !c->stats.accumulate) c->stats.state = 0;
    const bool compactList = !fullPlanes && x.streamRaw && x.stripWords && compact && compact->pRecords && compact->pShifts;
    const bool fitList = e.p.fitOnly && e.p.prefit && !ragged && chainPhase == 0;
    if (batchCount > 1 && !fitList && (!e.fused || !e.p.prefit || (!fullPlanes && !compactList))) return limg_hip_error_InvalidParameter;
    if (e.fused && (r = fused_scratch(e, compact)) != limg_hip_success) return r;

    const size_t subImages = sub_batch_images(e);
    if (subImages > 0 && subImages < batchCount) return encode_sub_batches(e, subImages);
    if (e.fused) return encode_fused(e);
    if (chainPhase == 2) return encode_chain_phase2(e);
    if (!ragged) return encode_split(e);
    return encode_ragged(e);
  }
}

namespace
{
  limg_hip_result encode_height_ragged(limg_hip_context *c, const uint32_t *dIn, size_t sizeX, size_t sizeY, int hasAlpha, const limg_hip_encode3d_info *dInfo,
                                       const limg_hip_compact_out *compact, uint32_t errorFactor, int poolThreads, int fast, hipStream_t stream, const EncodeExtra &x)
  {
    const size_t topY = (sizeY / kBlock) * kBlock, blocksX = sizeX / kBlock, blocksY = topY / kBlock + 1, stripsX = (blocksX + kStripBlocks - 1) / kStripBlocks;
    const Partition pt = partition(sizeY, poolThreads);
    c->chain.in = nullptr;
    c->stats.state = 0;
// ... 129 lines not shown
```

limg_amd/csrc/limg_hip_encode_ragged.hip:

```cpp
#include "limg_hip_context.h"

using namespace limg_hip;

namespace
{
  struct RaggedStage
  {
    size_t maxCalls, offPrev, offBase, offStates, offPixels, bytes;
    uint32_t *shifts = nullptr;
    unsigned long long *prev = nullptr;
    uint32_t *base = nullptr;
    unsigned long long *states = nullptr;
    uint8_t *pixels = nullptr;
    RaggedStage(size_t blocks, size_t strips) : maxCalls(blocks * 3)
    {
      offPrev = (blocks * 4 + 15) & ~(size_t)15; offBase = offPrev + 16; offStates = (offBase + strips * 4 + 15) & ~(size_t)15; offPixels = offStates + maxCalls * 8;
      bytes = offPixels + maxCalls + 16;
    }
    RaggedStage(size_t blocks, size_t strips, void *p) : RaggedStage(blocks, strips)
    {
      shifts = (uint32_t *)p;
      prev = (unsigned long long *)((uint8_t *)p + offPrev);
      base = (uint32_t *)((uint8_t *)p + offBase);
      states = (unsigned long long *)((uint8_t *)p + offStates);
      pixels = (uint8_t *)p + offPixels;
    }
  };

  limg_hip_result ensure_stage(EncodeJob &e)
  {
    limg_hip_context *const c = e.c;
    if (c->host.stageBusy) { HIP_TRY(hipEventSynchronize(c->host.stageEvent)); c->host.stageBusy = false; }
    return c->host.stage.ensure(RaggedStage(e.blocks, e.strips).bytes);
  }

  limg_hip_result release_stage(EncodeJob &e)
  {
    limg_hip_context *const c = e.c;
    const limg_hip_result r = c->host.stageEvent.ensure(hipEventDisableTiming);
    if (r != limg_hip_success) return r;
    HIP_TRY(hipEventRecord(c->host.stageEvent, e.stream));
    c->host.stageBusy = true;
    return limg_hip_success;
  }

  limg_hip_result size_noise_calls(EncodeJob &e, size_t calls)
  {
    limg_hip_context *const c = e.c;
    limg_hip_result r;
    if ((r = c->noise.dyn.ensure((calls + 1) * 64)) != limg_hip_success) return r;
    if ((r = c->noise.states.ensure(calls * 9 + 16)) != limg_hip_success) return r;
    e.p.noise = (const uint8_t *)c->noise.dyn.p;
    e.p.noiseLast = (uint32_t)calls;
    return limg_hip_success;
  }

  limg_hip_result upload_calls(EncodeJob &e, const RaggedStage &h, size_t calls, size_t call0, size_t n)
  {
    limg_hip_context *const c = e.c;
    if (!n) return limg_hip_success;
    unsigned long long *dStates = (unsigned long long *)c->noise.states.p;
    uint8_t *dPixels = (uint8_t *)c->noise.states.p + calls * 8;
    HIP_TRY(hipMemcpyAsync(dStates + call0, h.states + call0, n * 8, hipMemcpyHostToDevice, e.stream));
    HIP_TRY(hipMemcpyAsync(dPixels + call0, h.pixels + call0, n, hipMemcpyHostToDevice, e.stream));
    launch_noise_expand((uint8_t *)c->noise.dyn.p + call0 * 64, dStates + call0, dPixels + call0, n, c->opt.dither_pcg != 0, e.stream);
    return limg_hip_success;
  }

  uint32_t band_count(const EncodeJob &e)
  {
    const limg_hip_options &o = e.c->opt;
    const EncodeParams &p = e.p;
    uint32_t nBands = 1;
    if (e.dInfo && !e.x.dPrevDesc && e.pt.chainCount <= 1 && o.ragged_bands >= 0 && p.blocksX >= 2 && p.blocksY >= 2 && (o.ragged_bands > 0 || (p.blocksX >= 32 && p.blocksY >= 64)))
      nBands = o.ragged_bands > 0 ? (uint32_t)o.ragged_bands : 16u;
    if (nBands > p.blocksY / 2) nBands = p.blocksY / 2 ? p.blocksY / 2 : 1;
    if (nBands > 64) nBands = 64;
    return nBands;
  }

  EncodeParams band_params(const EncodeJob &e, uint32_t bandRows, uint32_t b)
  {
    const EncodeParams &p = e.p;
    EncodeParams q = p;
    const uint32_t r0 = b * bandRows, r1 = r0 + bandRows < p.blocksY ? r0 + bandRows : p.blocksY;
    const size_t y0 = (size_t)r0 * kBlock, skip = y0 * e.sizeX;
    q.io.in = p.io.in + skip;
    uint32_t **words[] = { &q.io.info.pDecoded, &q.io.info.pShiftABCX, &q.io.info.pColAMin, &q.io.info.pColAMax, &q.io.info.pColBMin, &q.io.info.pColBMax, &q.io.info.pColCMin, &q.io.info.pColCMax };
    uint8_t **bytes[] = { &q.io.info.pFactorsA, &q.io.info.pFactorsB, &q.io.info.pFactorsC };
    for (uint32_t **w : words) if (*w) *w += skip;
    for (uint8_t **w : bytes) if (*w) *w += skip;
    q.sizeY = (uint32_t)(((size_t)r1 * kBlock < e.sizeY ? (size_t)r1 * kBlock : e.sizeY) - y0);
    q.blocksY = r1 - r0;
    q.imageStrips = q.stripsX * q.blocksY;
    q.records += (size_t)r0 * p.blocksX; q.shifts += (size_t)r0 * p.blocksX; q.invN += (size_t)r0 * p.blocksX * 4;
    q.stripCalls += (size_t)r0 * p.stripsX; q.stripBase += (size_t)r0 * p.stripsX;
    return q;
  }

  limg_hip_result encode_ragged_banded(EncodeJob &e, uint32_t nBands, uint32_t bandRows)
  {
    limg_hip_context *const c = e.c;
    const EncodeParams &p = e.p;
    const hipStream_t stream = e.stream;
    limg_hip_result r;
    e.mark_if(1);
    if ((r = ensure_stage(e)) != limg_hip_success) return r;
    if ((r = c->host.raggedEvents.ensure(nBands, hipEventDisableTiming)) != limg_hip_success) return r;
    const RaggedStage h(e.blocks, e.strips, c->host.stage.p);
    for (uint32_t b = 0; b < nBands; b++)
    {
      const EncodeParams q = band_params(e, bandRows, b);
      launch_fit_search(q, e.channels, stream);
      const size_t off = (size_t)b * bandRows * p.blocksX;
      HIP_TRY(hipMemcpyAsync(h.shifts + off, p.shifts + off, (size_t)q.blocksY * p.blocksX * 4, hipMemcpyDeviceToHost, stream));
      HIP_TRY(hipEventRecord(c->host.raggedEvents[b], stream));
    }
    e.mark_if(1);
    if ((r = size_noise_calls(e, h.maxCalls)) != limg_hip_success) return r;
    const bool pcg = c->opt.dither_pcg != 0;
    uint64_t hv = kDitherSeed;
    size_t call = 0;
    for (uint32_t b = 0; b < nBands; b++)
    {
      EncodeParams q = band_params(e, bandRows, b);
      const uint32_t r0 = b * bandRows, r1 = r0 + q.blocksY;
      HIP_TRY(hipEventSynchronize(c->host.raggedEvents[b]));
      const size_t call0 = call;
      chain_walk_rows(hv, call, r0, r1, p.blocksX, p.stripsX, e.sizeX, e.sizeY, 1, 0, h.shifts, h.base, h.states, h.pixels, h.maxCalls, pcg);
      if ((r = upload_calls(e, h, h.maxCalls, call0, call - call0)) != limg_hip_success) return r;
      HIP_TRY(hipMemcpyAsync(p.stripBase + (size_t)r0 * p.stripsX, h.base + (size_t)r0 * p.stripsX, (size_t)q.blocksY * p.stripsX * 4, hipMemcpyHostToDevice, stream));
      q.noise = p.noise; q.noiseLast = p.noiseLast;
      if (b + 1 == nBands) e.mark_if(1);
      launch_dither_store(q, e.channels, stream);
    }
    if ((r = release_stage(e)) != limg_hip_success) return r;
    e.mark_if(2);
    HIP_TRY(hipGetLastError());
    return encode_stats(e);
  }
}

namespace limg_hip
{
  limg_hip_result encode_ragged(EncodeJob &e)
  {
    limg_hip_context *const c = e.c;
    const EncodeParams &p = e.p;
    const Partition &pt = e.pt;
    const hipStream_t stream = e.stream;
    uint32_t nBands = band_count(e);
    const uint32_t bandRows = (p.blocksY + nBands - 1) / nBands;
    nBands = (p.blocksY + bandRows - 1) / bandRows;
    if (nBands > 1) return encode_ragged_banded(e, nBands, bandRows);

    e.mark_if(1);
    launch_fit_search(p, e.channels, stream);
    e.mark_if(1);
    if (!e.dInfo)
    {
      e.mark_if(1); e.mark_if(2);
      HIP_TRY(hipGetLastError());
      return limg_hip_success;
    }
    limg_hip_result r;
    if ((r = ensure_stage(e)) != limg_hip_success) return r;
    const RaggedStage h(e.blocks, e.strips, c->host.stage.p);
    const size_t blocks = e.blocks, maxCalls = h.maxCalls;
    const bool pcg = c->opt.dither_pcg != 0;
    HIP_TRY(hipMemcpyAsync(h.shifts, p.shifts, blocks * 4, hipMemcpyDeviceToHost, stream));
    if (e.x.dPrevDesc) HIP_TRY(hipMemcpyAsync(h.prev, e.x.dPrevDesc, 8, hipMemcpyDeviceToHost, stream));
    HIP_TRY(hipStreamSynchronize(stream));
    size_t calls = 0;
    {
      size_t sumCalls = 0;
      for (size_t i = 0; i < blocks; i++) sumCalls += h.shifts[i] >> 24;
      calls = sumCalls < maxCalls ? sumCalls : maxCalls;
      if ((r = size_noise_calls(e, calls)) != limg_hip_success) return r;
    }
    uint64_t h0 = kDitherSeed;
    if (e.x.dPrevDesc)
    {
      if ((uint32_t)(*h.prev >> 32) != 2u || (uint32_t)*h.prev == 0xFFFFFFFFu || !chain_value_at((uint32_t)*h.prev, &h0))
      {
        fprintf(stderr, "limg_hip: the chain position of the last block row is unavailable (descriptor %016llx)\n", *h.prev);
        return limg_hip_error_Generic;
      }
    }
    size_t totalCalls = 0;
    unsigned threads = 1;
    if (pt.chainCount > 1 && pt.chainRows != 0 && !e.x.dPrevDesc && (blocks >= 4096 || c->opt.ragged_walk_threads > 1))
    {
      threads = c->opt.ragged_walk_threads > 0 ? (unsigned)c->opt.ragged_walk_threads : 16u;
      const unsigned hw = std::thread::hardware_concurrency();
      if (hw && threads > hw) threads = hw;
      if (threads > pt.chainCount) threads = pt.chainCount;
    }
    if (threads > 1)
    {
      size_t *first = new (std::nothrow) size_t[pt.chainCount + 1];
      uint32_t *row0 = new (std::nothrow) uint32_t[pt.chainCount + 1];
      if (!first || !row0) { delete[] first; delete[] row0; return limg_hip_error_MemoryAllocationFailure; }
      first[0] = 0;
      for (uint32_t k = 0; k < pt.chainCount; k++)
      {
        row0[k] = k * pt.chainRows;
        const uint32_t r1 = k + 1 < pt.chainCount ? (k + 1) * pt.chainRows : p.blocksY;
        size_t n = 0;
        for (size_t i = (size_t)row0[k] * p.blocksX; i < (size_t)r1 * p.blocksX; i++) n += h.shifts[i] >> 24;
        first[k + 1] = first[k] + n;
      }
      row0[pt.chainCount] = p.blocksY;
      run_on_threads(threads, [&](unsigned t) {
        for (uint32_t k = t; k < pt.chainCount; k += threads)
        {
          uint64_t hv = kDitherSeed;
          size_t call = first[k];
          chain_walk_rows(hv, call, row0[k], row0[k + 1], p.blocksX, p.stripsX, e.sizeX, e.sizeY, pt.chainCount, pt.chainRows, h.shifts, h.base, h.states, h.pixels, maxCalls, pcg);
        }
      });
      const size_t allCalls = first[pt.chainCount];
      delete[] first; delete[] row0;
      totalCalls = allCalls < maxCalls ? allCalls : maxCalls;
    }
    else totalCalls = chain_walk_blocks(h0, p.blocksX, p.blocksY, p.stripsX, e.sizeX, e.sizeY, pt.chainCount, pt.chainRows, h.shifts, h.base, h.states, h.pixels, maxCalls, pcg);
    if ((r = upload_calls(e, h, calls, 0, totalCalls)) != limg_hip_success) return r;
    HIP_TRY(hipMemcpyAsync(p.stripBase, h.base, e.strips * 4, hipMemcpyHostToDevice, stream));
    if ((r = release_stage(e)) != limg_hip_success) return r;
    e.mark_if(1);
    launch_dither_store(p, e.channels, stream);
    e.mark_if(2);
    HIP_TRY(hipGetLastError());
    return encode_stats(e);
  }
}
```

limg_amd/csrc/limg_hip_fit_tpb.hip:

```cpp
#include "limg_hip_device.h"

namespace limg_hip
{
  namespace
  {
    constexpr int kTpbStride = 68;

    template <bool DIRECT> constexpr int tpb_waves() { return DIRECT ? 4 : 2; }

    template <class BODY>
    __device__ __forceinline__ void for_rows(const uint32_t *my, const uint32_t pitch, BODY &&body)
    {
      uint4 u0 = *reinterpret_cast<const uint4 *>(my), w0 = *reinterpret_cast<const uint4 *>(my + 4);
      uint4 u1 = *reinterpret_cast<const uint4 *>(my + pitch), w1 = *reinterpret_cast<const uint4 *>(my + pitch + 4);
#pragma unroll 1
      for (int r = 0; r < 8; r += 2)
      {
        const uint32_t *nx = my + (r + 2 < 8 ? r + 2 : 6) * pitch;
        const uint4 nu0 = *reinterpret_cast<const uint4 *>(nx), nw0 = *reinterpret_cast<const uint4 *>(nx + 4);
        const uint4 nu1 = *reinterpret_cast<const uint4 *>(nx + pitch), nw1 = *reinterpret_cast<const uint4 *>(nx + pitch + 4);
        {
          const uint32_t q[8] = { u0.x, u0.y, u0.z, u0.w, w0.x, w0.y, w0.z, w0.w };
          body(r, q);
        }
        {
          const uint32_t q[8] = { u1.x, u1.y, u1.z, u1.w, w1.x, w1.y, w1.z, w1.w };
          body(r + 1, q);
        }
        u0 = nu0; w0 = nw0; u1 = nu1; w1 = nw1;
      }
    }

    template <int CH, bool FAST, bool DIRECT>
    __global__ __launch_bounds__(64 * tpb_waves<DIRECT>(), DIRECT ? 5 : 1) void k_fit_tpb(const EncodeParams p)
    {
      constexpr int kTpbWaves = tpb_waves<DIRECT>();
      __shared__ __attribute__((aligned(16))) uint32_t s_pxAll[kTpbWaves][DIRECT ? 4 : 64 * kTpbStride];
      __shared__ __attribute__((aligned(16))) uint32_t s_tab[FAST ? 4 : 2048];
      const int lane = (int)threadIdx.x & 63, wave = (int)threadIdx.x >> 6;
      if (p.fitPrio == 3) __builtin_amdgcn_s_setprio(3);
      else if (p.fitPrio == 2) __builtin_amdgcn_s_setprio(2);
      else if (p.fitPrio == 1) __builtin_amdgcn_s_setprio(1);
      if (!FAST)
      {
        const uint4 *src = reinterpret_cast<const uint4 *>(d_rsqrt_x86_tab);
        for (int i = (int)threadIdx.x; i < 256; i += 64 * kTpbWaves)
        {
          const uint4 v = src[i];
          const uint32_t q[4] = { v.x, v.y, v.z, v.w };
          uint32_t *dst = s_tab + ((8 * i) ^ 0x400);
#pragma unroll
          for (int k = 0; k < 4; k++) { dst[2 * k] = (q[k] & 0xFFFFu) << 11; dst[2 * k + 1] = (q[k] >> 16) << 11; }
        }
        __syncthreads();
      }
      const unsigned short *tab = reinterpret_cast<const unsigned short *>(s_tab);
      uint32_t *s_px = s_pxAll[wave];
      const uint32_t unitsX = (p.blocksX + 63u) / 64u;
      const uint32_t unitId = blockIdx.x * kTpbWaves + wave;
      if (unitId >= unitsX * p.blocksY * p.batchCount) return;
      const uint32_t unit = unitId % unitsX, byS = unitId / unitsX;
      const uint32_t img = p.batchCount > 1 ? byS / p.blocksY : 0u, by = byS - img * p.blocksY;
      const uint32_t *const pin = p.batchCount > 1 ? p.batch[img].in : p.io.in;
      const uint32_t bx0 = unit * 64u, x0 = bx0 * kBlock, y0 = by * kBlock;
      const uint32_t nBlocks = min(p.blocksX - bx0, 64u), widthPx = nBlocks * kBlock;
      if (p.zeroLookback)
      {
        if ((uint32_t)lane < 2u && unit * 2u + (uint32_t)lane < p.stripsX) p.desc[(size_t)byS * p.stripsX + unit * 2u + (uint32_t)lane] = 0ull;
        if (unitId == 0 && lane < 4) p.ticket[lane] = 0u;
      }

      if (!DIRECT)
      {
      if (p.vecIn)
      {
#pragma unroll
        for (int row = 0; row < 8; row++)
          for (uint32_t col = (uint32_t)lane * 4u; col < widthPx; col += 256u)
          {
            const uint4 v = *reinterpret_cast<const uint4 *>(pin + (size_t)(y0 + row) * p.sizeX + x0 + col);
            *reinterpret_cast<uint4 *>(&s_px[(col >> 3) * kTpbStride + row * 8 + (col & 7u)]) = v;
          }
      }
      else
      {
        for (int row = 0; row < 8; row++)
          for (uint32_t col = (uint32_t)lane; col < widthPx; col += 64u)
            s_px[(col >> 3) * kTpbStride + row * 8 + (col & 7u)] = pin[(size_t)(y0 + row) * p.sizeX + x0 + col];
      }
      }
      wave_lds_fence();
      if ((uint32_t)lane >= nBlocks) return;
      const uint32_t *my = DIRECT ? pin + (size_t)y0 * p.sizeX + x0 + lane * 8 : s_px + lane * kTpbStride;
      const uint32_t pitch = DIRECT ? p.sizeX : 8u;

      uint32_t s02 = 0, s13 = 0;
#pragma unroll
      for (int r = 0; r < 8; r++)
      {
        const uint4 u = *reinterpret_cast<const uint4 *>(my + r * pitch), w = *reinterpret_cast<const uint4 *>(my + r * pitch + 4);
        const uint32_t q[8] = { u.x, u.y, u.z, u.w, w.x, w.y, w.z, w.w };
#pragma unroll
        for (int i = 0; i < 8; i++) { s02 += q[i] & 0x00FF00FFu; s13 += (q[i] >> 8) & 0x00FF00FFu; }
      }
      const float inv_count = 0.015625f;
      V4 avg;
      avg.a = float2_t{ (float)(int)(s02 & 0xFFFF), (float)(int)(s02 >> 16) } * inv_count;
      avg.b = float2_t{ (float)(int)(s13 & 0xFFFF), CH == 4 ? (float)(int)(s13 >> 16) : 0.0f } * inv_count;
      const V4 zero4 = { float2_t{ 0.0f, 0.0f }, float2_t{ 0.0f, 0.0f } };

      auto finish_dir = [&](const V4 &acc, V4 &dir, float &inv, bool &zero)
      {
        dir = acc * inv_count;
        const float pp = dp4<CH>(dir, dir);
        zero = dir.a.x == 0.0f && dir.a.y == 0.0f && dir.b.x == 0.0f && dir.b.y == 0.0f;
        inv = FAST ? __builtin_amdgcn_rcpf(pp) : 1.0f / pp;
      };

      V4 dirA, dirB = zero4, dirC = zero4, est0 = zero4;
      float invA, invB = 0.0f, invC = 0.0f;
      bool zeroA, zeroB = true, zeroC = true;
      float mm[6] = { 0.0f, 0.0f, 0.0f, 0.0f, 0.0f, 0.0f };
      {
        V4 acc = zero4;
        for_rows(my, pitch, [&](const int, const uint32_t (&q)[8])
        {
#pragma unroll
          for (int i = 0; i < 8; i++)
          {
            V4 d = px_to_v4(q[i]) - avg;
            mask_alpha<CH>(d);
            acc = acc + unit4<CH, FAST, true, true>(tab, d, true);
          }
        });
        finish_dir(acc, dirA, invA, zeroA);
      }

      if (!zeroA)
      {
        V4 acc = zero4;
        float mn = 0.0f, mx = 0.0f;
        for_rows(my, pitch, [&](const int, const uint32_t (&q)[8])
        {
#pragma unroll
          for (int i = 0; i < 8; i++)
          {
            const V4 pf = px_to_v4(q[i]);
            const float fA = dp4<CH, FAST>(pf - avg, dirA) * invA;
            mn = vmin(mn, fA); mx = vmax(mx, fA);
            V4 e = pf - (avg + dirA * fA);
            mask_alpha<CH>(e);
            acc = acc + unit4<CH, FAST, true, true>(tab, e, true);
          }
        });
        mm[0] = mn; mm[1] = mx;
        finish_dir(acc, dirB, invB, zeroB);
      }

      if (!zeroA && !zeroB)
      {
        float mnB = FLT_MAX, mxB = -FLT_MAX;
        if (CH == 4)
        {
          V4 acc = zero4;
          for_rows(my, pitch, [&](const int r, const uint32_t (&q)[8])
          {
#pragma unroll
            for (int i = 0; i < 8; i++)
            {
              const V4 pf = px_to_v4(q[i]);
              const float fA = dp4<CH, FAST>(pf - avg, dirA) * invA;
              const V4 estA = avg + dirA * fA;
              const float fB = dp4<CH, FAST>(pf - estA, dirB) * invB;
              mnB = vmin(mnB, fB); mxB = vmax(mxB, fB);
              const V4 estB = estA + dirB * fB;
              if (r == 0 && i == 0) est0 = estB;
              acc = acc + unit4<CH, FAST, true, true>(tab, pf - estB, true);
            }
          });
          mm[2] = mnB; mm[3] = mxB;
          finish_dir(acc, dirC, invC, zeroC);
          if (!zeroC)
          {
            float mnC = FLT_MAX, mxC = -FLT_MAX;
            for_rows(my, pitch, [&](const int, const uint32_t (&q)[8])
            {
#pragma unroll
              for (int i = 0; i < 8; i++)
              {
                const float fC = dp4<CH, FAST>(px_to_v4(q[i]) - est0, dirC) * invC;
                mnC = vmin(mnC, fC); mxC = vmax(mxC, fC);
              }
            });
            mm[4] = mnC; mm[5] = mxC;
          }
        }
        else
        {
          dirC.a.x = dirA.b.x * dirB.a.y - dirA.a.y * dirB.b.x;
          dirC.b.x = dirA.a.y * dirB.a.x - dirA.a.x * dirB.a.y;
          dirC.a.y = dirA.a.x * dirB.b.x - dirA.b.x * dirB.a.x;
          dirC.b.y = 0.0f;
          zeroC = dirC.a.x == 0.0f && dirC.b.x == 0.0f && dirC.a.y == 0.0f;
          if (!zeroC) invC = FAST ? __builtin_amdgcn_rcpf(dp4<CH, FAST>(dirC, dirC)) : 1.0f / dp4<CH, FAST>(dirC, dirC);
          float mnC = zeroC ? 0.0f : FLT_MAX, mxC = zeroC ? 0.0f : -FLT_MAX;
          for_rows(my, pitch, [&](const int, const uint32_t (&q)[8])
          {
#pragma unroll
            for (int i = 0; i < 8; i++)
            {
              const V4 pf = px_to_v4(q[i]);
              const float fA = dp4<CH, FAST>(pf - avg, dirA) * invA;
              const V4 estA = avg + dirA * fA;
              const float fB = dp4<CH, FAST>(pf - estA, dirB) * invB;
              mnB = vmin(mnB, fB); mxB = vmax(mxB, fB);
              if (!zeroC)
              {
                const V4 e = pf - (estA + dirB * fB);
                const float fC = dp4<CH, FAST>(e, dirC) * invC;
                mnC = vmin(mnC, fC); mxC = vmax(mxC, fC);
              }
            }
          });
          mm[2] = mnB; mm[3] = mxB; mm[4] = mnC; mm[5] = mxC;
        }
      }

      const bool deadA = zeroA, deadB = zeroA || zeroB, deadC = zeroA || zeroB || zeroC;
      auto comp = [](const V4 &v, int c) -> float { return c == 0 ? v.a.x : (c == 1 ? v.b.x : (c == 2 ? v.a.y : v.b.y)); };
      uint32_t words[16];
#pragma unroll
      for (int c = 0; c < 4; c++) words[c] = __float_as_uint(comp(avg, c));
      float inv[3];
#pragma unroll
      for (int r = 0; r < 3; r++)
      {
        const bool dead = r == 0 ? deadA : (r == 1 ? deadB : deadC);
        const V4 &dir = r == 0 ? dirA : (r == 1 ? dirB : dirC);
        int16_t lo[4], hi[4];
        float sum = 0.0f;
        bool nz = false;
#pragma unroll
        for (int c = 0; c < 4; c++)
        {
          float dv = comp(dir, c), mLo = mm[2 * r], mHi = mm[2 * r + 1];
          if (dead) { mLo = 0.0f; mHi = 0.0f; dv = 0.0f; }
          float vLo = mLo * dv, vHi = mHi * dv;
          if (r == 0) { vLo = comp(avg, c) + vLo; vHi = comp(avg, c) + vHi; }
          int qLo = cvt_rne(vLo), qHi = cvt_rne(vHi);
          if (CH == 3 && c == 3) { qLo = 0; qHi = 0; }
          lo[c] = (int16_t)qLo; hi[c] = (int16_t)qHi;
          if (CH == 4 || c < 3)
          {
            const float n = (float)((int)hi[c] - (int)lo[c]);
            const float sq = n * n;
            sum = sum + sq;
            nz = nz || sq != 0.0f;
          }
        }
        inv[r] = nz ? (FAST ? __builtin_amdgcn_rcpf(sum) : 1.0f / sum) : 0.0f;
        words[4 + 4 * r] = (uint32_t)(uint16_t)lo[0] | ((uint32_t)(uint16_t)lo[1] << 16);
        words[5 + 4 * r] = (uint32_t)(uint16_t)lo[2] | ((uint32_t)(uint16_t)lo[3] << 16);
        words[6 + 4 * r] = (uint32_t)(uint16_t)hi[0] | ((uint32_t)(uint16_t)hi[1] << 16);
        words[7 + 4 * r] = (uint32_t)(uint16_t)hi[2] | ((uint32_t)(uint16_t)hi[3] << 16);
      }
      uint4 *dst = reinterpret_cast<uint4 *>(p.records + (size_t)byS * p.blocksX + bx0 + lane);
#pragma unroll
      for (int i = 0; i < 4; i++) dst[i] = make_uint4(words[4 * i], words[4 * i + 1], words[4 * i + 2], words[4 * i + 3]);
      reinterpret_cast<float4 *>(p.invN)[(size_t)byS * p.blocksX + bx0 + lane] = make_float4(inv[0], inv[1], inv[2], 0.0f);
    }
  }

  namespace
  {
    struct TableChunk { ImageIO e[32]; uint32_t n; };
    static_assert(sizeof(TableChunk) <= 3584, "kernel-argument segment");
    __global__ void k_set_batch_table(ImageIO *dst, const TableChunk chunk)
    {
      const uint32_t *src = reinterpret_cast<const uint32_t *>(chunk.e);
      uint32_t *out = reinterpret_cast<uint32_t *>(dst);
      for (uint32_t i = threadIdx.x; i < chunk.n * (uint32_t)(sizeof(ImageIO) / 4); i += blockDim.x) out[i] = src[i];
    }
  }

  void launch_set_batch_table(ImageIO *dTable, const ImageIO *hTable, size_t count, hipStream_t s)
  {
    for (size_t i0 = 0; i0 < count; i0 += 32)
    {
      TableChunk ch;
      ch.n = (uint32_t)(count - i0 < 32 ? count - i0 : 32);
      for (uint32_t i = 0; i < ch.n; i++) ch.e[i] = hTable[i0 + i];
      for (uint32_t i = ch.n; i < 32; i++) ch.e[i] = ImageIO{};
      hipLaunchKernelGGL(k_set_batch_table, dim3(1), dim3(256), 0, s, dTable + i0, ch);
    }
  }

  void launch_fit_tpb(const EncodeParams &p, int channels, hipStream_t s)
  {
    const uint32_t units = ((p.blocksX + 63u) / 64u) * p.blocksY * p.batchCount;
    with_flags([&](auto rgba, auto FAST, auto DIRECT)
               { hipLaunchKernelGGL((k_fit_tpb<rgba ? 4 : 3, FAST, DIRECT>), dim3((units + tpb_waves<DIRECT>() - 1) / tpb_waves<DIRECT>()), dim3(64 * tpb_waves<DIRECT>()), 0, s, p); },
               channels == 4, p.floatFast != 0, p.vecIn != 0);
  }
}
```

limg_amd/csrc/limg_hip_float_pixel.h:

```cpp
#ifndef LIMG_HIP_FLOAT_PIXEL_H
#define LIMG_HIP_FLOAT_PIXEL_H

#include "limg_hip_device.h"

namespace limg_hip
{
  namespace
  {
    constexpr int kRowDw = 264;
    constexpr int kVDw = 260;

    struct BlkF
    {
      float avg[4], dirA[4], dirB[4], dirC[4], est0[4];
      float mm[6];
      float inv_count, invA, invB, invC;
      uint32_t flags, n;
      int16_t rec[24];
      float pad[4];
    };
    struct BlkE
    {
      float nrm[3][4];
      float off[3][4];
      float invN[3];
    };
    static_assert(sizeof(BlkE) <= 120, "BlkE must fit the dead float-stage fields");
    static_assert(sizeof(BlkF) == 192, "BlkF layout");

    struct EStrip
    {
      uint32_t strip, by, byS;
      uint32_t x0, y0, stripW, ry;
      int tid, lane, wave;
      uint32_t *pix;
      float *V;
      BlkF *blk;
      uint32_t *calls;
      int *trialc;
    };

    template <class P>
    __device__ __forceinline__ bool block_geom(const P &p, const EStrip g, const uint32_t sb, uint32_t &rx, uint32_t &n)
    {
      const uint32_t bx = g.strip * kStripBlocks + sb;
      if (bx >= p.blocksX) { rx = 0; n = 0; return false; }
      rx = min(p.sizeX - bx * kBlock, (uint32_t)kBlock);
      n = rx * g.ry;
      return true;
    }

    __device__ __forceinline__ uint32_t block_pixel(const EStrip g, const uint32_t sb, const uint32_t rx, const uint32_t n, uint32_t &lx, uint32_t &ly)
    {
      const int lane = g.lane;
      if (rx == 8) { lx = lane & 7; ly = lane >> 3; }
      else { const uint32_t l = (uint32_t)lane < n ? (uint32_t)lane : 0u; ly = l / rx; lx = l - ly * rx; }
      const uint32_t px = g.pix[ly * kRowDw + sb * kBlock + lx];
      return (uint32_t)lane < n ? px : 0u;
    }

    enum : int { kDirA = 0, kDirB = 1, kDirC = 2 };
    constexpr int kBatch = 4;
    constexpr uint32_t kBig = 16u;

    template <int CH, int WHICH, bool FAST>
    __device__ __forceinline__ void serial_sums2(const float *V, BlkF *blk, int lane)
    {
      wave_lds_fence();
      if (lane < 4 * kBatch)
      {
        const int b = lane >> 2, c = lane & 3;
        const float *src = V + b * kVDw + c;
        float s = 0.0f;
#pragma unroll 16
        for (int i = 0; i < 64; i++) s = s + src[i * 4];
        const float dir = s * blk[b].inv_count;
        float *dst = WHICH == kDirA ? blk[b].dirA : (WHICH == kDirB ? blk[b].dirB : blk[b].dirC);
        dst[c] = dir;
        float p = (CH == 3 && c == 3) ? 0.0f : dir * dir;
        p = p + __int_as_float(dpp<0x4E, 0xF>(0, __float_as_int(p)));
        p = p + __int_as_float(dpp<0xB1, 0xF>(0, __float_as_int(p)));
        uint32_t z = (dir == 0.0f) ? 1u : 0u;
        z &= (uint32_t)dpp<0xB1, 0xF>(0, (int)z);
        z &= (uint32_t)dpp<0x4E, 0xF>(0, (int)z);
        const float inv = FAST ? __builtin_amdgcn_rcpf(p) : 1.0f / p;
        if (c == 0)
        {
          if (WHICH == kDirA) { blk[b].invA = inv; if (z) blk[b].flags |= kZeroA | kZeroB | kZeroC; }
          else if (WHICH == kDirB) { blk[b].invB = inv; if (z) blk[b].flags |= kZeroB | kZeroC; }
          else { blk[b].invC = inv; if (z) blk[b].flags |= kZeroC; }
        }
      }
      wave_lds_fence();
    }
  }
}

#endif
```

limg_amd/csrc/limg_hip_internal.h:

```cpp
#ifndef LIMG_HIP_INTERNAL_H
#define LIMG_HIP_INTERNAL_H

#include <hip/hip_runtime.h>
#include <stdint.h>

#include <type_traits>

#include "../../include/limg_hip.h"
#include "limg_hip_blocked_host.h"
#include "limg_hip_rate_step.h"
#include "limg_hip_encode_rules.h"

namespace limg_hip
{
  constexpr int kBlock = 8;
  constexpr int kStripBlocks = 32;
  constexpr int kThreads = 256;
  constexpr int kWaves = 4;
  constexpr int kBlocksPerWave = 8;
  constexpr uint64_t kDitherSeed = 0xCA7F00D15BADF00DULL;

  __host__ __device__ inline uint32_t chain_of_row(uint32_t chainCount, uint32_t chainRows, uint32_t row)
  {
    if (chainCount <= 1 || chainRows == 0) return 0u;
    const uint32_t c = row / chainRows;
    return c < chainCount - 1 ? c : chainCount - 1;
  }
  __host__ __device__ inline uint32_t chain_head_row(uint32_t chainCount, uint32_t chainRows, uint32_t row) { return chain_of_row(chainCount, chainRows, row) * chainRows; }

  struct ImageIO
  {
    const uint32_t *in;
    limg_hip_encode3d_info info;
  };

  struct EncodeParams
  {
    ImageIO io;
    const ImageIO *batch;
    uint32_t batchCount, imageStrips;
    uint32_t sizeX, sizeY, blocksX, blocksY, stripsX;
    uint32_t maxPixel32;
    uint64_t maxBlock;
    uint32_t blockLimitFull;
    int32_t crushBits, fast;
    const uint32_t *accTable;
    int32_t forced[3];
    int32_t recordLimit;
    uint32_t chainCount, chainRows;
    limg_hip_block_record *records;
    float *invN;
    uint32_t *shifts;
    uint32_t *stripCalls;
    uint32_t *stripBase;
    uint32_t *stripWords;
    int32_t storePlanes;
    int32_t fullPlanes;
    const uint8_t *noise;
    uint32_t noiseLast;
    unsigned long long *desc;
    uint32_t *ticket;
    int32_t zeroLookback;
    uint32_t *timeout;
#ifdef LIMG_HIP_TEST_HOOKS
    uint32_t lookbackSpins;
    uint32_t testBaseErrStrip;
    uint32_t testSkipStrip;
#endif
    uint8_t *park;
    int32_t compactOut;
    int32_t streamRaw;
    int32_t fitOnly;
    unsigned long long *chainCallsOut;
    const unsigned long long *chainBase;
    int32_t fitPrio;
    int32_t prefit;
    int32_t floatFast;
    int32_t vecIn;
    int32_t vecPlanes;
    int32_t vecFactors;
    int32_t vecFactors8;
    int32_t vecDecoded;
  };

  struct StreamParams
  {
    uint32_t sizeX, sizeY, blocksX, blocksY, nBlocks, nTiles, channels, errorFactor, flags;
    const uint8_t *fac[3];
    const limg_hip_block_record *records;
    const uint32_t *shifts;
    uint8_t *stream;
    uint32_t *tileBase;
    uint32_t *stripWords;
    uint32_t stripsX, nStrips, nWaves;
  };

  struct StreamImage
  {
    const uint8_t *fac[3];
    uint8_t *stream;
  };
  struct StreamBatchParams
  {
    uint32_t sizeX, sizeY, blocksX, blocksY, nBlocks , channels, errorFactor, flags;
    uint32_t stripsX, imageStrips, nImages, nStrips , nWaves;
    const StreamImage *images;
    const limg_hip_block_record *records;
    const uint32_t *shifts;
    uint32_t *stripWords;
  };

  struct DecodeParams
  {
    uint32_t sizeX, sizeY, blocksX, blocksY, nBlocks;
    const uint8_t *stream;
    unsigned long long streamBytes;
    uint32_t *out;
    uint32_t *status;
    uint32_t *sink;
  };

  const uint64_t *noise_checkpoints_host(size_t *pCount, size_t *pEvery);
  const uint64_t *noise_checkpoints_far_host(size_t *pCount, size_t *pEvery);
  void launch_noise_fill(uint8_t *noise, const uint64_t *dCheckpoints, size_t count, hipStream_t s);
  void launch_noise_expand(uint8_t *noise, const unsigned long long *dStates, const uint8_t *dPixels, size_t calls, bool pcg, hipStream_t s);
  void launch_noise_expand_calls(uint8_t *noise, const unsigned long long *dStates, const unsigned long long *dOffsets, const uint32_t *dPixels, size_t calls, bool pcg, hipStream_t s);
  void launch_set_batch_table(ImageIO *dTable, const ImageIO *hTable, size_t count, hipStream_t s);
  template <class F> void with_flags(F &&f) { f(); }
  template <class F, class... Flags> void with_flags(F &&f, bool flag, Flags... rest)
  {
    if (!flag) with_flags([&](auto... b) { f(std::false_type(), b...); }, rest...);
    else with_flags([&](auto... b) { f(std::true_type(), b...); }, rest...);
  }

  void launch_fit_tpb(const EncodeParams &p, int channels, hipStream_t s);
  void launch_fit_search(const EncodeParams &p, int channels, hipStream_t s);
  void launch_encode_persistent(const EncodeParams &p, int channels, int workgroups, hipStream_t s);
  void launch_strip_scan(const EncodeParams &p, hipStream_t s);
  void launch_dither_store(const EncodeParams &p, int channels, hipStream_t s);
  void launch_shift_stats(const uint32_t *dShifts, uint32_t blocksX, uint32_t blocksY, uint32_t rows, uint32_t sizeX, uint32_t sizeY, unsigned long long *dOut30, hipStream_t s);
  void launch_chain_base(const unsigned long long *dCalls, int rank, int world, unsigned long long *dBase, uint32_t *dAborted, hipStream_t s);

  struct RegionDesc
  {
    uint32_t ox, oy, rx, ry;
    uint32_t keep;
    uint32_t scratch;
    uint32_t pad[2];
  };
  struct RegionOut
  {
    limg_hip_block_record rec;
    uint32_t shiftWord;
    uint32_t pad[3];
  };
  struct BlockedParams
  {
    const uint32_t *in;
    uint32_t sizeX, sizeY, blocksX, blocksY, channels;
    uint32_t maxPixel32;
    uint64_t maxBlock;
    int32_t crushBits, fast, forced[3];
    const limg_hip_block_record *pass1;
    unsigned long long *matchBits;
    uint32_t seedBase, seedCount;
    uint8_t *matchFlags;
    float *matchBound;
    const RegionDesc *regions;
    uint32_t nRegions;
    uint32_t regionBase;
    RegionOut *out;
    int32_t vecStore;
    uint32_t *order;
    uint32_t *scratchPx;
    uint8_t *scratchFac;
    uint32_t scratchCap;
    const uint8_t *noise;
    const unsigned long long *noiseBase;
    limg_hip_blocked_encode3d_info info;
  };

  void launch_blocked_bounds(const BlockedParams &p, hipStream_t s);
  void launch_blocked_match(const BlockedParams &p, hipStream_t s);
  void launch_blocked_fit_search(const BlockedParams &p, hipStream_t s);
  void launch_blocked_store(const BlockedParams &p, hipStream_t s);
  void launch_blocked_order(const BlockedParams &p, hipStream_t s);

  struct BlockedStreamParams
  {
    uint32_t sizeX, sizeY, blocksX, blocksY, channels, errorFactor, flags;
    uint32_t nRegions, nTiles, scratchCap;
    const RegionDesc *regions;
    const RegionOut *out;
    const unsigned long long *noiseBase;
    const uint8_t *scratchFac, *noise;
    uint8_t *stream;
    uint32_t *units;
    uint32_t *tiles;
  };
  void launch_blocked_stream_pack(const BlockedStreamParams &p, int cus, hipStream_t s);

  struct WindowDecodeParams
  {
    uint32_t sizeX, sizeY, blocksX, blocksY, nBlocks;
    const uint8_t *stream;
    unsigned long long streamBytes;
    uint32_t x0, y0, width, height;
    uint32_t bx0, by0, wbx, wby;
    uint32_t *out;
    unsigned long long outStride;
    uint32_t vecOut;
    uint32_t log2Scale;
    uint32_t *map;
    uint32_t *status;
    uint32_t *state;
    unsigned long long planeStride;
  };
  void launch_stream_window_decode(const WindowDecodeParams &p, int cus, hipStream_t s);
  void launch_blocked_stream_window_decode(const WindowDecodeParams &p, int cus, hipStream_t s);

  struct WindowGroup
  {
    uint32_t sizeX, sizeY, blocksX, blocksY, nBlocks;
    uint32_t firstJob, nJobs;
    uint32_t pad;
    const uint8_t *stream;
    unsigned long long streamBytes;
  };
  struct WindowBatchParams
  {
    const WindowDecodeParams *jobs;
    const uint32_t *unitBase;
    uint32_t count, totalUnits;
    uint32_t *status;
    uint32_t *jobStatus;
    const WindowGroup *groups;
    const uint32_t *groupJobs;
    const uint32_t *groupItemBase;
    uint32_t nGroups, totalItems;
  };
  void launch_stream_windows(const WindowBatchParams &b, bool scaled, const limg_hip_tensor_format *f, int cus, hipStream_t s);
  void launch_blocked_stream_windows(const WindowBatchParams &b, bool scaled, const limg_hip_tensor_format *f, int cus, hipStream_t s);
  static_assert(sizeof(WindowDecodeParams) == 128, "the job table's entry: log2Scale must not grow it");

  constexpr uint32_t kResizeTilePixels = 4096;
  constexpr uint32_t kResizeTileEdge = 64;
  struct ResizeJob
  {
    uint32_t outW, outH;
    uint32_t x0, y0, srcW, srcH;
    uint32_t flags;
    uint32_t tileW, tileH;
    uint32_t tilesX;
    uint32_t stepR, pad0;
    unsigned long long stepQ;
    uint32_t pad[2];
  };
  static_assert(sizeof(ResizeJob) == 64, "the second per-job table's entry");
  struct WindowResizeParams
  {
    WindowBatchParams b;
    const ResizeJob *resize;
    const uint32_t *tileBase;
    uint32_t totalTiles;
  };
  struct ResizeTaps { uint32_t a, b, f; };
  __host__ __device__ inline ResizeTaps resize_taps(unsigned long long c16, uint32_t L, uint32_t lo, uint32_t hi)
  {
    const long long u16 = (long long)(c16 >> L) - 32768;
    const long long i0 = u16 >> 16, l = (long long)lo, h = (long long)hi;
    ResizeTaps t;
    t.f = (uint32_t)(((u16 & 0xFFFF) + 128) >> 8);
    t.a = (uint32_t)(i0 < l ? l : i0 > h ? h : i0);
    t.b = (uint32_t)(i0 + 1 < l ? l : i0 + 1 > h ? h : i0 + 1);
    return t;
  }
  __host__ __device__ inline ResizeTaps resize_axis(uint32_t X, uint32_t s0, uint32_t len, uint32_t out, uint32_t L, uint32_t lo, uint32_t hi)
  {
    return resize_taps(((unsigned long long)s0 << 16) + ((((unsigned long long)(2u * X + 1u) * len) << 15) / out), L, lo, hi);
  }
  __host__ __device__ inline uint32_t resize_hi(uint32_t s0, uint32_t len, uint32_t L, uint32_t size)
  {
    const uint32_t e = (s0 + len - 1u) >> L, r = (size >> L) - 1u;
    return e < r ? e : r;
  }
  void launch_stream_windows_resized(const WindowResizeParams &r, const limg_hip_tensor_format *f, int cus, hipStream_t s);
  void launch_blocked_stream_windows_resized(const WindowResizeParams &r, const limg_hip_tensor_format *f, int cus, hipStream_t s);

  void launch_stream_pack(const StreamParams &p, hipStream_t s);
  void launch_stream_pack_batch(const StreamBatchParams &b, hipStream_t s);
  void launch_set_stream_table(StreamImage *dTable, const StreamImage *hTable, size_t count, hipStream_t s);
  void launch_stream_gather_bytes(const StreamImage *dTable, size_t count, unsigned long long *dBytes, hipStream_t s);
  void launch_stream_decode(const DecodeParams &p, int cus, hipStream_t s);

  struct RateDevice
  {
    RateState search;
    uint32_t listNext;
    uint32_t maxPixel32, blockLimitFull, crushBits;
    uint64_t maxBlock;
  };
  struct RateProbeParams
  {
    struct { const uint32_t *in; } io;
    uint32_t sizeX, sizeY, blocksX, blocksY, stripsX;
    int32_t vecIn;
    int32_t recordLimit;
    int32_t forced[3];
    const limg_hip_block_record *records;
    const float *invN;
    const RateDevice *state;
    unsigned long long *counter;
  };
  void launch_rate_begin(RateDevice *dState, unsigned long long *dCounter, const RateState &first, uint32_t firstErrorFactor, hipStream_t s);
  void launch_rate_step(RateDevice *dState, unsigned long long *dCounter, uint64_t fixedBytes, const uint32_t *dList, unsigned long long *dListBytes, uint32_t listCount,
                        hipStream_t s);
  void launch_rate_probe(const RateProbeParams &p, int channels, bool floatFast, hipStream_t s);
  struct RateProbeBatchParams
  {
    const ImageIO *batch;
    uint32_t nImages, imageStrips;
    uint32_t sizeX, sizeY, blocksX, blocksY, stripsX;
    int32_t vecIn;
    int32_t recordLimit;
    int32_t forced[3];
    const limg_hip_block_record *records;
    const float *invN;
    const RateDevice *states;
    unsigned long long *counters;
  };
  struct RateBudgetChunk { uint32_t n; unsigned long long maxBytes[64]; };
  void launch_rate_begin_batch(RateDevice *dStates, unsigned long long *dCounters, const uint64_t *hMaxBytes, size_t count, uint32_t hLo, uint32_t hHi, hipStream_t s);
  void launch_rate_step_batch(RateDevice *dStates, unsigned long long *dCounters, uint32_t nImages, uint64_t fixedBytes, hipStream_t s);
  void launch_rate_probe_batch(const RateProbeBatchParams &p, int channels, bool floatFast, hipStream_t s);

  void launch_synth_random_gradient(uint32_t *out, uint32_t w, uint32_t h, uint64_t seed, int opaque, uint32_t y0, hipStream_t s);
  void launch_synth_photo_noise(uint32_t *out, uint32_t w, uint32_t h, uint64_t seed, uint32_t y0, hipStream_t s);
  void launch_compare(const uint32_t *a, const uint32_t *b, uint64_t count, int channels, unsigned long long *dErrorSum, hipStream_t s);
}

#endif
```

limg_amd/csrc/limg_hip_kernels.hip:

```cpp
#include "limg_hip_phase_e.h"
#include "limg_hip_lookback.h"

namespace limg_hip
{
  namespace
  {
    constexpr int kPrioE = 2;


    template <int CH, bool PERSIST, class P>
    __device__ __forceinline__ void finish_block(const P &p, const EStrip g, const uint32_t sb, const uint32_t bx, const BlkF *blkE, const uint32_t shift[3], const uint32_t fA,
                                                 const uint32_t fB, const uint32_t fC, const bool active, const uint32_t o, uint8_t *park, uint8_t *stage, uint32_t &waveCalls)
    {
      const uint32_t calls = (((shift[0] & 7u) + 7u) >> 3) + (((shift[1] & 7u) + 7u) >> 3) + (((shift[2] & 7u) + 7u) >> 3);
      waveCalls += calls;
      if (p.stripWords)
      {
        uint32_t words = 0;
#pragma unroll
        for (int k = 0; k < 3; k++)
        {
          const uint32_t sk = shift[k];
          if (sk < 8u) words += 8u - sk;
          else if (CH == 4 && sgpr((int)blkE->rec[8 * k + 3]) != sgpr((int)blkE->rec[8 * k + 7])) words += 8u;
        }
        waveCalls += words << 8;
      }

      const size_t bi = (size_t)g.byS * p.blocksX + bx;
      const uint32_t word = shift[0] | (shift[1] << 8) | (shift[2] << 16) | (calls << 24);
      if (g.lane == 0)
      {
        if (!PERSIST || p.compactOut) p.shifts[bi] = word;
        if (PERSIST) reinterpret_cast<uint32_t *>(park + kParkShift)[sb] = word;
      }
      if (p.storePlanes && active) { stage[o] = (uint8_t)fA; stage[kFacPlane + o] = (uint8_t)fB; stage[2 * kFacPlane + o] = (uint8_t)fC; }
    }

    template <bool PERSIST, class P>
    __device__ __forceinline__ void publish_strip(const P &p, const EStrip g, const uint32_t id, const uint32_t head0)
    {
      const uint32_t aggAll = g.calls[0] + g.calls[1] + g.calls[2] + g.calls[3];
      const uint32_t agg = aggAll & 0xFFu;
      if (p.stripWords) p.stripWords[id] = aggAll >> 8;
      if (PERSIST)
      {
        const uint32_t headId = head0 + chain_head_row(p.chainCount, p.chainRows, g.by) * p.stripsX;
#ifdef LIMG_HIP_TEST_HOOKS
        if (id == p.testSkipStrip) {}
        else
#endif
        if (id == headId) desc_store(p.desc + id, kDescInclusive, agg);
        else
        {
          const unsigned long long d = desc_load(p.desc + id - 1);
          if ((uint32_t)(d >> 32) == kDescInclusive) desc_store(p.desc + id, kDescInclusive, (uint32_t)d == kBasePoison ? kBasePoison : (uint32_t)d + agg);
          else desc_store(p.desc + id, kDescAggregate, agg);
        }
      }
      else p.stripCalls[id] = agg;
    }

    template <bool PERSIST, class P, class IO>
    __device__ __forceinline__ void park_or_store_factors(const P &p, const IO &io, const EStrip g, uint8_t *park, uint8_t *stage)
    {
      if (PERSIST)
        for (int i = g.tid; i < 384; i += kThreads) reinterpret_cast<uint4 *>(park + kParkFac)[i] = *reinterpret_cast<const uint4 *>(stage + (i >> 4) * kFacRow + (i & 15) * 16);
      else if (p.storePlanes) copy_factor_planes<true>(p, io, stage, g.x0, g.y0, g.stripW, g.ry, g.tid);
    }

    template <int CH, bool PERSIST, bool FAST, bool PREFIT, bool ACC, class P, class IO>
    __device__ __forceinline__ void fit_search_strip(const P &p, const IO &io, const uint32_t id, const uint32_t local, const uint32_t rowBase, const uint32_t head0, uint8_t *lds,
                                                     uint8_t *park, const int tid)
    {
      constexpr LdsLayout LL = lds_layout<PREFIT>();
      EStrip g;
      g.tid = tid; g.lane = tid & 63; g.wave = tid >> 6;
      g.strip = local % p.stripsX; g.by = local / p.stripsX; g.byS = rowBase + g.by;
      g.x0 = g.strip * (kStripBlocks * kBlock); g.y0 = g.by * kBlock;
      g.stripW = min(p.sizeX - g.x0, (uint32_t)(kStripBlocks * kBlock)); g.ry = min(p.sizeY - g.y0, (uint32_t)kBlock);
      g.pix = reinterpret_cast<uint32_t *>(lds + kLdsStrip); g.V = reinterpret_cast<float *>(lds + LL.v); g.blk = reinterpret_cast<BlkF *>(lds + LL.blk);
      g.calls = reinterpret_cast<uint32_t *>(lds + LL.calls); g.trialc = reinterpret_cast<int *>(lds + LL.trialc);
      const int lane = g.lane;

      uint32_t recVal[2] = { 0u, 0u };
      if (PREFIT) request_prefit_records(p, g, recVal);
      stage_strip_pixels(p, io, g);
      __syncthreads();
      if (PREFIT) take_prefit_records<PERSIST>(p, g, recVal, park);
      else
      {
      const unsigned short *s_rsq = d_rsqrt_x86_tab;
      const int lane = g.lane, wave = g.wave;
      const uint32_t strip = g.strip, by = g.by, byS = g.byS;
      float *V = g.V + wave * kBatch * kVDw;
      BlkF *blk = g.blk + wave * kBlocksPerWave;
      auto geom = [&](int b, uint32_t &rx, uint32_t &n) -> bool { return block_geom(p, g, wave * kBlocksPerWave + b, rx, n); };

#pragma unroll 1
      for (int h = 0; h < kBlocksPerWave / kBatch; h++)
      {
      uint32_t px8[kBatch];
      V4 est8[kBatch];
      BlkF *const blkh = blk + h * kBatch;

#pragma unroll
      for (int i = 0; i < kBatch; i++)
      {
        const int b = h * kBatch + i;
        uint32_t rx, n;
        px8[i] = 0;
        est8[i].a = float2_t{ 0.0f, 0.0f }; est8[i].b = float2_t{ 0.0f, 0.0f };
        if (!geom(b, rx, n))
        {
          if (lane == 0) { blk[b].flags = 0; blk[b].n = 0; blk[b].inv_count = 0.0f; }
          continue;
        }
        const uint32_t sb = wave * kBlocksPerWave + b;
        uint32_t lx, ly;
        const uint32_t px = block_pixel(g, sb, rx, n, lx, ly);
        px8[i] = px;
        const V4 pf = px_to_v4(px);
        uint32_t pxs = px;
        if (n < 4)
        {
          const uint32_t bxx = strip * kStripBlocks + sb;
          const bool hasPrev = bxx > 0 || by > chain_head_row(p.chainCount, p.chainRows, by);
          if (hasPrev && (uint32_t)lane >= n && lane < 4)
          {
            const uint32_t pbx = bxx > 0 ? bxx - 1 : p.blocksX - 1, pby = bxx > 0 ? by : by - 1;
            const uint32_t prx = min(p.sizeX - pbx * kBlock, (uint32_t)kBlock);
            const uint32_t row = (uint32_t)lane / prx, col = (uint32_t)lane - row * prx;
            pxs = io.in[(size_t)(pby * kBlock + row) * p.sizeX + pbx * kBlock + col];
          }
        }
        const uint32_t s02 = wave_sum(pxs & 0x00FF00FFu), s13 = wave_sum((pxs >> 8) & 0x00FF00FFu);
        float inv_count = 0.015625f;
        if (n != 64) inv_count = 1.0f / (float)n;
        V4 avg;
        avg.a = float2_t{ (float)(int)(s02 & 0xFFFF), (float)(int)(s02 >> 16) } * inv_count;
        avg.b = float2_t{ (float)(int)(s13 & 0xFFFF), CH == 4 ? (float)(int)(s13 >> 16) : 0.0f } * inv_count;
        V4 d = pf - avg;
        mask_alpha<CH>(d);
        st4(V + i * kVDw + lane * 4, unit4<CH, FAST>(s_rsq, d, (uint32_t)lane < n));
        if (lane == 0)
        {
          st4(blk[b].avg, avg);
          *reinterpret_cast<float4 *>(blk[b].dirB) = make_float4(0.f, 0.f, 0.f, 0.f);
          *reinterpret_cast<float4 *>(blk[b].dirC) = make_float4(0.f, 0.f, 0.f, 0.f);
          *reinterpret_cast<float4 *>(blk[b].est0) = make_float4(0.f, 0.f, 0.f, 0.f);
          *reinterpret_cast<float4 *>(blk[b].mm) = make_float4(0.f, 0.f, 0.f, 0.f);
          blk[b].mm[4] = 0.0f; blk[b].mm[5] = 0.0f;
          blk[b].inv_count = inv_count; blk[b].n = n; blk[b].flags = kValid;
        }
      }
      serial_sums2<CH, kDirA, FAST>(V, blkh, lane);

      {
        static_assert(kBatch == 4, "wave_reduce4_min_max");
        float mnv[kBatch], mxv[kBatch];
        bool did[kBatch];
#pragma unroll
        for (int i = 0; i < kBatch; i++)
        {
          const int b = h * kBatch + i;
          uint32_t rx, n;
          did[i] = false; mnv[i] = 0.0f; mxv[i] = 0.0f;
          if (!geom(b, rx, n)) continue;
          if ((uint32_t)sgpr((int)blk[b].flags) & kZeroA) continue;
          did[i] = true;
          const V4 dirA = ld4(blk[b].dirA), avg = ld4(blk[b].avg);
          const float invA = blk[b].invA;
          const V4 pf = px_to_v4(px8[i]);
          const bool active = (uint32_t)lane < n;
          const float fA = dp4<CH, FAST>(pf - avg, dirA) * invA;
          mnv[i] = active ? fA : 0.0f; mxv[i] = mnv[i];
          est8[i] = avg + dirA * fA;
          V4 e = pf - est8[i];
          mask_alpha<CH>(e);
          st4(V + i * kVDw + lane * 4, unit4<CH, FAST>(s_rsq, e, active));
        }
        wave_reduce4_min_max(mnv, mxv);
#pragma unroll
        for (int i = 0; i < kBatch; i++)
          if (did[i] && lane == 0) { blk[h * kBatch + i].mm[0] = vmin(mnv[i], 0.0f); blk[h * kBatch + i].mm[1] = vmax(mxv[i], 0.0f); }
      }
      serial_sums2<CH, kDirB, FAST>(V, blkh, lane);

      float mnCv[kBatch], mxCv[kBatch];
      bool didC[kBatch];
#pragma unroll
      for (int i = 0; i < kBatch; i++) { didC[i] = false; mnCv[i] = FLT_MAX; mxCv[i] = -FLT_MAX; }
#pragma unroll
      for (int i = 0; i < kBatch; i++)
      {
        const int b = h * kBatch + i;
        uint32_t rx, n;
        if (!geom(b, rx, n)) continue;
        if ((uint32_t)sgpr((int)blk[b].flags) & kZeroB) continue;
        const V4 dirB = ld4(blk[b].dirB);
        const float invB = blk[b].invB;
        const V4 pf = px_to_v4(px8[i]);
        const bool active = (uint32_t)lane < n;
        const float fB = dp4<CH, FAST>(pf - est8[i], dirB) * invB;
        float mnB = active ? fB : FLT_MAX, mxB = active ? fB : -FLT_MAX;
        if (CH == 4)
        {
          didC[i] = true; mnCv[i] = mnB; mxCv[i] = mxB;
          est8[i] = est8[i] + dirB * fB;
          st4(V + i * kVDw + lane * 4, unit4<CH, FAST>(s_rsq, pf - est8[i], active));
          if (lane == 0) st4(blk[b].est0, est8[i]);
        }
        else
        {
          const V4 dirA = ld4(blk[b].dirA);
          V4 dirC;
          dirC.a.x = dirA.b.x * dirB.a.y - dirA.a.y * dirB.b.x;
          dirC.b.x = dirA.a.y * dirB.a.x - dirA.a.x * dirB.a.y;
          dirC.a.y = dirA.a.x * dirB.b.x - dirA.b.x * dirB.a.x;
          dirC.b.y = 0.0f;
          const bool zeroC = sgpr((dirC.a.x == 0.0f && dirC.b.x == 0.0f && dirC.a.y == 0.0f) ? 1 : 0) != 0;
          float mnC = 0.0f, mxC = 0.0f;
          if (!zeroC)
          {
            const float invC = FAST ? __builtin_amdgcn_rcpf(dp4<CH, FAST>(dirC, dirC)) : 1.0f / dp4<CH, FAST>(dirC, dirC);
            const V4 e = pf - (est8[i] + dirB * fB);
            const float fC = dp4<CH, FAST>(e, dirC) * invC;
            mnC = active ? fC : FLT_MAX; mxC = active ? fC : -FLT_MAX;
            wave_min_max(mnB, mxB);
            wave_min_max(mnC, mxC);
          }
          else
            wave_min_max(mnB, mxB);
          if (lane == 0)
          {
            blk[b].mm[2] = mnB; blk[b].mm[3] = mxB; blk[b].mm[4] = mnC; blk[b].mm[5] = mxC;
            st4(blk[b].dirC, dirC);
            if (zeroC) blk[b].flags |= kZeroC;
          }
        }
      }
      if (CH == 4)
      {
        wave_reduce4_min_max(mnCv, mxCv);
#pragma unroll
        for (int i = 0; i < kBatch; i++)
          if (didC[i] && lane == 0) { blk[h * kBatch + i].mm[2] = mnCv[i]; blk[h * kBatch + i].mm[3] = mxCv[i]; }
        serial_sums2<CH, kDirC, FAST>(V, blkh, lane);
        float mnDv[kBatch], mxDv[kBatch];
        bool didD[kBatch];
#pragma unroll
        for (int i = 0; i < kBatch; i++)
        {
          const int b = h * kBatch + i;
          uint32_t rx, n;
          didD[i] = false; mnDv[i] = FLT_MAX; mxDv[i] = -FLT_MAX;
          if (!geom(b, rx, n)) continue;
          if ((uint32_t)sgpr((int)blk[b].flags) & kZeroC) continue;
          didD[i] = true;
          const V4 dirC = ld4(blk[b].dirC), est0 = ld4(blk[b].est0);
          const float invC = blk[b].invC;
          const V4 pf = px_to_v4(px8[i]);
          const bool active = (uint32_t)lane < n;
          const float fC = dp4<CH, FAST>(pf - est0, dirC) * invC;
          mnDv[i] = active ? fC : FLT_MAX; mxDv[i] = active ? fC : -FLT_MAX;
        }
        wave_reduce4_min_max(mnDv, mxDv);
#pragma unroll
        for (int i = 0; i < kBatch; i++)
          if (didD[i] && lane == 0) { blk[h * kBatch + i].mm[4] = mnDv[i]; blk[h * kBatch + i].mm[5] = mxDv[i]; }
      }
      }
      wave_lds_fence();

      {
        const int b = lane >> 3, j = lane & 7;
        const uint32_t flags = blk[b].flags;
        uint32_t big = 0;
#pragma unroll
        for (int r = 0; r < 3; r++)
        {
          const int kc = j + 8 * r, k = kc >> 2, c = kc & 3;
          const float *dir = r == 0 ? blk[b].dirA : (r == 1 ? blk[b].dirB : blk[b].dirC);
          const int sl = slot_of(c);
          float m = blk[b].mm[k], dv = dir[sl];
          const bool dead = (r == 2 && (flags & kZeroC)) || (r >= 1 && (flags & kZeroB)) || (flags & kZeroA);
          if (dead) { m = 0.0f; dv = 0.0f; }
          float val = m * dv;
          if (r == 0) val = blk[b].avg[sl] + val;
          int q = cvt_rne(val);
          if ((CH == 3 && c == 3) || !(flags & kValid)) q = 0;
          big |= (q > p.recordLimit || q < -p.recordLimit) ? 1u : 0u;
          blk[b].rec[kc] = (int16_t)q;
        }
        big |= (uint32_t)dpp<0xB1, 0xF>(0, (int)big);
        big |= (uint32_t)dpp<0x4E, 0xF>(0, (int)big);
        big |= (uint32_t)dpp<0x141, 0xF>(0, (int)big);
        if (j == 0 && big) blk[b].flags = flags | kBig;
      }
      wave_lds_fence();
      {
#pragma unroll
        for (int r = 0; r < 2; r++)
        {
          const int b = r * 4 + (lane >> 4), w = lane & 15;
          const uint32_t sb = wave * kBlocksPerWave + b, bx = strip * kStripBlocks + sb;
          const uint32_t val = w < 4 ? __float_as_uint(blk[b].avg[slot_of(w)]) : reinterpret_cast<const uint32_t *>(blk[b].rec)[w - 4];
          if (bx < p.blocksX && (!PERSIST || p.compactOut)) reinterpret_cast<uint32_t *>(p.records + (size_t)byS * p.blocksX + bx)[w] = val;
          if (PERSIST && w >= 4) reinterpret_cast<uint32_t *>(park + kParkRec)[sb * 12 + (w - 4)] = val;
        }
      }
    
      }
      if (!PERSIST && p.fitOnly) return;
      phase_e_view<CH, FAST, PREFIT>(g);
      uint32_t *s_queue = g.calls + 4;
      if (tid == 0) *s_queue = 0;
      __syncthreads();

      uint8_t *stage = reinterpret_cast<uint8_t *>(g.V);
      uint32_t waveCalls = 0;

      auto grab = [&]() -> uint32_t { uint32_t v = 0; if (lane == 0) v = atomicAdd(s_queue, 1u); return (uint32_t)sgpr((int)v); };
      uint32_t sbNext = grab();
#pragma unroll 1
      for (;;)
      {
        const uint32_t sb = sbNext;
        if (sb >= (uint32_t)kStripBlocks) break;
        uint32_t qv = 0;
        if (lane == 0) qv = atomicAdd(s_queue, 1u);
        uint32_t rx, n, lx, ly;
        if (!block_geom(p, g, sb, rx, n)) { sbNext = (uint32_t)sgpr((int)qv); continue; }
        const BlkF *const blkE = g.blk + sb;
        const bool active = (uint32_t)lane < n;
        const uint32_t px = block_pixel(g, sb, rx, n, lx, ly);
        uint32_t fA, fB, fC, shift[3] = { 0, 0, 0 };
        pixel_factors<CH, FAST>(reinterpret_cast<const BlkE *>(blkE), px, fA, fB, fC);
        if (p.forced[0] >= 0) { shift[0] = (uint32_t)p.forced[0]; shift[1] = (uint32_t)p.forced[1]; shift[2] = (uint32_t)p.forced[2]; }
        else if (p.crushBits)
        {
          const uint64_t maxBlockN = p.maxBlock * (uint64_t)n;
          uint32_t blockLimit = p.blockLimitFull;
          if (n != 64)
          {
            const uint64_t lim64 = (maxBlockN + 15ull) >> 4;
            blockLimit = (uint32_t)sgpr((int)(lim64 > 0xFFFFFFFFull ? 0xFFFFFFFFu : (uint32_t)lim64));
          }
          const bool big = ((uint32_t)sgpr((int)blkE->flags) & kBig) != 0;
          if (!big)
          {
            TrialState t;
            t.fA = fA; t.fB = fB; t.fC = fC;
            const uint32_t R = px & 0xFF, G = (px >> 8) & 0xFF;
            t.hiRG = (R + 0x8000u) | ((G + 0x8000u) << 16);
            t.loRG = (R + 0x8000u - 255u) | ((G + 0x8000u - 255u) << 16);
            t.pxB = (int)((px >> 16) & 0xFF);
            t.pxBlo = t.pxB - 255;
            if (PREFIT)
            {
              const int *tc = g.trialc + sb * kTrialConstDw;
#pragma unroll
              for (int c = 0; c < 3; c++)
              {
                t.nA[c] = tc[c]; t.nB[c] = tc[3 + c]; t.nC[c] = tc[6 + c];
                t.mA[c] = tc[9 + c]; t.mB[c] = tc[12 + c]; t.mC[c] = tc[15 + c];
              }
            }
            else
            {
#pragma unroll
              for (int c = 0; c < 3; c++)
              {
                const int loA = blkE->rec[c], hiA = blkE->rec[4 + c], loB = blkE->rec[8 + c], hiB = blkE->rec[12 + c], loC = blkE->rec[16 + c], hiC = blkE->rec[20 + c];
                t.nA[c] = loA - hiA; t.nB[c] = loB - hiB; t.nC[c] = loC - hiC;
                t.mA[c] = term_const(0, c, loA); t.mB[c] = term_const(1, c, loB); t.mC[c] = term_const(2, c, loC);
              }
            }
            t.mA[0] += (int)(R << 8); t.mA[1] += (int)(G << 8); t.mA[2] += t.pxB << 8;
            if (!ACC)
            {
              if (n == 64) search_fast_automaton<true>(t, true, p.maxPixel32, blockLimit, shift);
              else search_fast_automaton<false>(t, active, p.maxPixel32, blockLimit, shift);
            }
            else
            {
              if (n == 64) search_accurate_automaton<true>(t, true, p.maxPixel32, blockLimit, p.accTable, shift);
              else search_accurate_automaton<false>(t, active, p.maxPixel32, blockLimit, p.accTable, shift);
            }
          }
          else
          {
            const uint32_t packed = (uint32_t)sgpr((int)search_generic(px, fA, fB, fC, blkE->rec, active, p.maxPixel32, maxBlockN, !ACC));
            shift[0] = packed & 0xFF; shift[1] = (packed >> 8) & 0xFF; shift[2] = (packed >> 16) & 0xFF;
          }
        }
    
        finish_block<CH, PERSIST>(p, g, sb, g.strip * kStripBlocks + sb, blkE, shift, fA, fB, fC, active, ly * kFacRow + sb * kBlock + lx, park, stage, waveCalls);
        sbNext = (uint32_t)sgpr((int)qv);
      }
      if (lane == 0) g.calls[g.wave] = waveCalls;
      __syncthreads();
      if (tid == 0) publish_strip<PERSIST>(p, g, id, head0);
      park_or_store_factors<PERSIST>(p, io, g, park, stage);
    }

    __global__ __launch_bounds__(1024) void k_strip_scan(const EncodeParams p)
    {
      __shared__ uint32_t s_sum[1024];
      __shared__ uint32_t s_flag[1024];
      const uint32_t total = p.blocksY * p.stripsX;
      const uint32_t per = (total + 1023u) / 1024u;
      const uint32_t t = threadIdx.x;
      const uint32_t begin = min(t * per, total), end = min(begin + per, total);
      auto chain_of = [&](uint32_t e) -> uint32_t { return chain_of_row(p.chainCount, p.chainRows, e / p.stripsX); };
      auto is_head = [&](uint32_t e) -> bool { return e == 0 || chain_of(e) != chain_of(e - 1); };

      uint32_t sum = 0, flag = 0;
      for (uint32_t e = begin; e < end; e++)
      {
        if (is_head(e)) { sum = 0; flag = 1; }
        sum += p.stripCalls[e];
      }
      s_sum[t] = sum; s_flag[t] = flag;
      __syncthreads();
      for (uint32_t off = 1; off < 1024; off <<= 1)
      {
        uint32_t vs = s_sum[t], vf = s_flag[t];
        if (t >= off && !vf) { vs += s_sum[t - off]; vf = s_flag[t - off]; }
        __syncthreads();
        s_sum[t] = vs; s_flag[t] = vf;
        __syncthreads();
      }
      uint32_t run = (t == 0) ? 0u : s_sum[t - 1];
      for (uint32_t e = begin; e < end; e++)
      {
        if (is_head(e)) run = 0;
        p.stripBase[e] = run;
        run += p.stripCalls[e];
      }
      if (p.chainCallsOut && end == total && begin < end) *p.chainCallsOut = run;
    }

    static_assert(kPhaseFBytes + kStripBlocks * 48 <= kLdsTotal - kLdsStrip - 16, "the F step's LDS overlays the E step's");

    template <int CH, bool PERSIST, class P, class IO>
    __device__ __forceinline__ void dither_store_strip(const P &p, const IO &io, const uint32_t id, const uint32_t local, const uint32_t rowBase, const uint32_t head0, uint8_t *fbase,
                                                       const uint8_t *park, const int tid)
    {
      int16_t *s_rec = reinterpret_cast<int16_t *>(fbase + kPhaseFBytes);
      const int lane = tid & 63, wave = tid >> 6;
      const uint32_t strip = local % p.stripsX, by = local / p.stripsX;
      const uint32_t byS = rowBase + by;
      const uint32_t x0 = strip * (kStripBlocks * kBlock), y0 = by * kBlock;
      const uint32_t stripW = min(p.sizeX - x0, (uint32_t)(kStripBlocks * kBlock));
      const uint32_t ry = min(p.sizeY - y0, (uint32_t)kBlock);
      const uint32_t nBlocks = min(p.blocksX - strip * kStripBlocks, (uint32_t)kStripBlocks);
      const StripLds L = carve_phase_f(fbase, s_rec, 24);

      if (PERSIST)
      {
        static_assert(kStripBlocks * 12 * 4 == 96 * 16, "record copy");
#pragma unroll 1
        for (int i = tid; i < 384; i += kThreads) *reinterpret_cast<uint4 *>(L.fac + (i >> 4) * kFacRow + (i & 15) * 16) = reinterpret_cast<const uint4 *>(park + kParkFac)[i];
        if (tid < 96) reinterpret_cast<uint4 *>(s_rec)[tid] = reinterpret_cast<const uint4 *>(park + kParkRec)[tid];
        if (tid < kStripBlocks) L.shift[tid] = (uint32_t)tid < nBlocks ? reinterpret_cast<const uint32_t *>(park + kParkShift)[tid] : 0u;
      }
      else
      {
        copy_factor_planes<false>(p, io, L.fac, x0, y0, stripW, ry, tid);
        for (int i = tid; i < kStripBlocks * 12; i += kThreads)
        {
          const int sb = i / 12, w = i - sb * 12;
          uint32_t v = 0;
          if ((uint32_t)sb < nBlocks) v = reinterpret_cast<const uint32_t *>(p.records + (size_t)byS * p.blocksX + strip * kStripBlocks + sb)[4 + w];
          reinterpret_cast<uint32_t *>(s_rec + sb * 24)[w] = v;
        }
        if (tid < kStripBlocks) L.shift[tid] = (uint32_t)tid < nBlocks ? p.shifts[(size_t)byS * p.blocksX + strip * kStripBlocks + tid] : 0u;
      }
      __syncthreads();
      phase_f_prepare<CH>(L, lane, wave, p.recordLimit);
      wave_lds_fence();
      const bool rowsPath = PERSIST || (p.sizeX % kBlock == 0 && ry == (uint32_t)kBlock);
      if (p.fullPlanes) phase_f_store_const(p, io, L, x0, y0, ry, lane, wave, rowsPath ? 1u : 3u);
      if (wave == 0)
      {
        uint32_t base;
        if (PERSIST)
        {
          const uint32_t headId = head0 + chain_head_row(p.chainCount, p.chainRows, by) * p.stripsX;
          const uint32_t w = lane < kStripBlocks ? L.shift[lane] : 0u;
          const uint32_t agg = wave_sum(w >> 24);
          const unsigned long long own = desc_load(p.desc + id);
          if ((uint32_t)(own >> 32) == kDescInclusive) base = (uint32_t)sgpr((int)((uint32_t)own == kBasePoison ? kBasePoison : (uint32_t)own - agg));
          else
          {
            base = lookback_base(p, id, headId, agg, lane);
            if (lane == 0 && publishes(p, id)) desc_store(p.desc + id, kDescInclusive, base == kBasePoison ? kBasePoison : base + agg);
          }
#ifdef LIMG_HIP_TEST_HOOKS
          if (id == p.testBaseErrStrip) base += 1u;
#endif
        }
        else
        {
          base = p.stripBase[id];
          if (p.chainBase) base += (uint32_t)*p.chainBase;
        }
        phase_f_first_calls(L, base, lane);
      }
      __syncthreads();
      if (PERSIST && L.first[0] == kBasePoison) return;
      if (rowsPath) phase_f_rows<CH>(p, io, L, strip, x0, y0, lane, wave, [&]() { if (p.fullPlanes) phase_f_store_const(p, io, L, x0, y0, ry, lane, wave, 2u); });
      else phase_f_pixels<CH>(p, io, L, strip, x0, y0, ry, lane, wave, tid);
    }

    template <int CH, bool FAST, bool PREFIT, bool ACC>
    __global__ __launch_bounds__(kThreads) void k_fit_search(const EncodeParams p)
    {
// ... 146 lines not shown
```

limg_amd/csrc/limg_hip_phase_e.h:

```cpp
#ifndef LIMG_HIP_PHASE_E_H
#define LIMG_HIP_PHASE_E_H

#include "limg_hip_search.h"
#include "limg_hip_phase_f.h"
#include "limg_hip_float_pixel.h"

namespace limg_hip
{
  namespace
  {
    constexpr int kLdsStrip = 0, kLdsV = kLdsStrip + 8 * kRowDw * 4, kLdsVBytes = kWaves * kBatch * kVDw * 4;
    constexpr int kLdsBlk = kLdsV + kLdsVBytes, kLdsCalls = kLdsBlk + kStripBlocks * 192, kLdsTotal = kLdsCalls + 32;
    static_assert(kLdsTotal <= 32768 - 16, "5 workgroups per CU");
    struct LdsLayout { int v, blk, calls, trialc, total; };
    constexpr int kTrialConstDw = 20;
    template <bool PREFIT> __device__ __host__ constexpr LdsLayout lds_layout()
    {
      if (!PREFIT) return LdsLayout{ kLdsV, kLdsBlk, kLdsCalls, kLdsV, kLdsTotal };
      const int v = kLdsStrip + 8 * kRowDw * 4, blk = v + kFacBytes, calls = blk + kStripBlocks * 192, tc = calls + 32, e = tc + kStripBlocks * kTrialConstDw * 4;
      const int f = kLdsStrip + kPhaseFBytes + kStripBlocks * 48 + 16;
      return LdsLayout{ v, blk, calls, tc, e > f ? e : f };
    }
    static_assert(lds_layout<true>().total <= 163840 / 6, "6 workgroups per CU with the float stage in its own kernel");


    constexpr int kParkFac = 0, kParkRec = 6144, kParkShift = 6144 + 1536, kParkBytes = 8192;


    template <class P>
    __device__ __forceinline__ void request_prefit_records(const P &p, const EStrip g, uint32_t recVal[2])
    {
#pragma unroll
      for (int r = 0; r < 2; r++)
      {
        const int b = r * 4 + (g.lane >> 4), w = g.lane & 15;
        const uint32_t bx = g.strip * kStripBlocks + g.wave * kBlocksPerWave + b;
        if (bx < p.blocksX) recVal[r] = w >= 4 ? reinterpret_cast<const uint32_t *>(p.records + (size_t)g.byS * p.blocksX + bx)[w]
                                               : reinterpret_cast<const uint32_t *>(p.invN)[((size_t)g.byS * p.blocksX + bx) * 4 + w];
      }
    }

    template <class P, class IO>
    __device__ __forceinline__ void stage_strip_pixels(const P &p, const IO &io, const EStrip g)
    {
      const int tid = g.tid;
      if (p.vecIn)
      {
#pragma unroll
        for (int pass = 0; pass < 2; pass++)
        {
          const uint32_t row = pass * 4 + (tid >> 6), col = (tid & 63) * 4;
          if (row < g.ry && col < g.stripW)
          {
            const uint4 v = *reinterpret_cast<const uint4 *>(io.in + (size_t)(g.y0 + row) * p.sizeX + g.x0 + col);
            *reinterpret_cast<uint4 *>(&g.pix[row * kRowDw + col]) = v;
          }
        }
      }
      else
      {
        for (uint32_t i = tid; i < 8 * 256; i += kThreads)
        {
          const uint32_t row = i >> 8, col = i & 255;
          if (row < g.ry && col < g.stripW) g.pix[row * kRowDw + col] = io.in[(size_t)(g.y0 + row) * p.sizeX + g.x0 + col];
        }
      }
    }

    template <bool PERSIST, class P>
    __device__ __forceinline__ void take_prefit_records(const P &p, const EStrip g, const uint32_t recVal[2], uint8_t *park)
    {
      BlkF *blk = g.blk + g.wave * kBlocksPerWave;
#pragma unroll
      for (int r = 0; r < 2; r++)
      {
        const int b = r * 4 + (g.lane >> 4), w = g.lane & 15;
        const uint32_t sb = g.wave * kBlocksPerWave + b, bx = g.strip * kStripBlocks + sb;
        const uint32_t val = recVal[r];
        if (w < 3) reinterpret_cast<BlkE *>(&blk[b])->invN[w] = __uint_as_float(val);
        if (w >= 4)
        {
          reinterpret_cast<uint32_t *>(blk[b].rec)[w - 4] = val;
          if (PERSIST) reinterpret_cast<uint32_t *>(park + kParkRec)[sb * 12 + (w - 4)] = val;
        }
        const int lo = (int)(int16_t)(val & 0xFFFFu), hi = (int)(int16_t)(val >> 16);
        uint32_t big = (w >= 4 && (lo > p.recordLimit || lo < -p.recordLimit || hi > p.recordLimit || hi < -p.recordLimit)) ? 1u : 0u;
        big |= (uint32_t)dpp<0xB1, 0xF>(0, (int)big);
        big |= (uint32_t)dpp<0x4E, 0xF>(0, (int)big);
        big |= (uint32_t)dpp<0x141, 0xF>(0, (int)big);
        big |= (uint32_t)dpp<0x140, 0xF>(0, (int)big);
        if (w == 0) { blk[b].flags = (bx < p.blocksX ? kValid : 0u) | (big ? kBig : 0u); blk[b].n = bx < p.blocksX ? 64u : 0u; }
      }
      wave_lds_fence();
    }

    template <int CH, bool FAST, bool PREFIT>
    __device__ __forceinline__ void phase_e_view(const EStrip g)
    {
      const int lane = g.lane;
      BlkF *blk = g.blk + g.wave * kBlocksPerWave;
      float nrm[2], off[2], invn[2];
#pragma unroll
      for (int r = 0; r < 2; r++)
      {
        const int idx = min(r * 64 + lane, 95);
        const int b = idx / 12, fc = idx - b * 12, f = fc >> 2, c = fc & 3;
        const int lo = blk[b].rec[f * 8 + c], hi = blk[b].rec[f * 8 + 4 + c];
        nrm[r] = (float)(hi - lo); off[r] = (float)lo;
        if (PREFIT) { invn[r] = 0.0f; continue; }
        const float sq = nrm[r] * nrm[r];
        const float s0 = __int_as_float(dpp<0x00, 0xF>(0, __float_as_int(sq))), s1 = __int_as_float(dpp<0x55, 0xF>(0, __float_as_int(sq)));
        const float s2 = __int_as_float(dpp<0xAA, 0xF>(0, __float_as_int(sq))), s3 = __int_as_float(dpp<0xFF, 0xF>(0, __float_as_int(sq)));
        float s = ((0.0f + s0) + s1) + s2;
        if (CH == 4) s = s + s3;
        const bool nz = (s0 != 0.0f) || (s1 != 0.0f) || (s2 != 0.0f) || (CH == 4 && s3 != 0.0f);
        invn[r] = nz ? (FAST ? __builtin_amdgcn_rcpf(s) : 1.0f / s) : 0.0f;
      }
      wave_lds_fence();
#pragma unroll
      for (int r = 0; r < 2; r++)
      {
        const int idx = r * 64 + lane;
        if (idx < 96)
        {
          const int b = idx / 12, fc = idx - b * 12, f = fc >> 2, c = fc & 3;
          BlkE *e = reinterpret_cast<BlkE *>(&blk[b]);
          e->nrm[f][slot_of(c)] = nrm[r]; e->off[f][slot_of(c)] = off[r];
          if (!PREFIT && c == 0) e->invN[f] = invn[r];
          if (PREFIT && c < 3)
          {
            int *tc = g.trialc + (g.wave * kBlocksPerWave + b) * kTrialConstDw;
            tc[f * 3 + c] = -(int)nrm[r];
            tc[9 + f * 3 + c] = term_const(f, c, (int)off[r]);
          }
        }
      }
    }

    template <int CH, bool FAST>
    __device__ __forceinline__ void pixel_factors(const BlkE *be, const uint32_t px, uint32_t &fA, uint32_t &fB, uint32_t &fC)
    {
      const V4 pv = px_to_v4(px);
      const V4 nA = ld4(be->nrm[0]), mnA = ld4(be->off[0]);
      const float fa = dp4<CH, FAST>(pv - mnA, nA) * be->invN[0];
      fA = cvt_u8_rne_sat(255.0f * fa);
      const V4 nB = ld4(be->nrm[1]), ofB = ld4(be->off[1]);
      V4 est = mnA + nA * fa;
      const float fb = dp4<CH, FAST>((pv - est) - ofB, nB) * be->invN[1];
      fB = cvt_u8_rne_sat(255.0f * fb);
      const V4 nC = ld4(be->nrm[2]), ofC = ld4(be->off[2]);
      est = est + nB * fb;
      const float fc = dp4<CH, FAST>((pv - est) - ofC, nC) * be->invN[2];
      fC = cvt_u8_rne_sat(255.0f * fc);
    }
  }
}

#endif
```

limg_amd/csrc/limg_hip_rate.hip:

```cpp
#include "limg_hip_phase_e.h"

namespace limg_hip
{
  namespace
  {
    __device__ __forceinline__ void set_thresholds(RateDevice *d, uint32_t errorFactor)
    {
      const Thresholds t = thresholds(errorFactor);
      d->maxPixel32 = t.maxPixel32; d->blockLimitFull = t.blockLimitFull; d->maxBlock = t.maxBlock; d->crushBits = t.crushBits;
    }

    __global__ void k_rate_begin(RateDevice *d, unsigned long long *counter, const RateState first, const uint32_t firstErrorFactor)
    {
      d->search = first;
      d->listNext = 0u;
      set_thresholds(d, firstErrorFactor);
      *counter = 0ull;
    }

    __global__ void k_rate_step(RateDevice *d, unsigned long long *counter, const unsigned long long fixedBytes, const uint32_t *list, unsigned long long *listBytes,
                                const uint32_t listCount)
    {
      const unsigned long long bytes = fixedBytes + 8ull * *counter;
      *counter = 0ull;
      if (list)
      {
        const uint32_t i = d->listNext;
        if (i >= listCount) return;
        listBytes[i] = bytes;
        d->listNext = i + 1u;
        if (i + 1u < listCount) set_thresholds(d, list[i + 1u]);
        return;
      }
      if (d->search.done) return;
      rate_step(d->search, bytes);
      if (!d->search.done) set_thresholds(d, 2u * d->search.next);
    }

    template <int CH, bool FAST, class P, class IO>
    __device__ __forceinline__ void rate_probe_strip(const P &p, const IO &io, const RateDevice *const st, unsigned long long *const counter, uint8_t *const lds,
                                                     const uint32_t strip, const uint32_t by, const uint32_t byS)
    {
      constexpr LdsLayout LL = lds_layout<true>();
      if (st->search.done) return;
      const uint32_t maxPixel32 = (uint32_t)sgpr((int)st->maxPixel32), blockLimit = (uint32_t)sgpr((int)st->blockLimitFull), crushBits = (uint32_t)sgpr((int)st->crushBits);
      const int tid = (int)threadIdx.x;
      EStrip g;
      g.tid = tid; g.lane = tid & 63; g.wave = tid >> 6;
      g.strip = strip; g.by = by; g.byS = byS;
      g.x0 = g.strip * (kStripBlocks * kBlock); g.y0 = g.by * kBlock;
      g.stripW = min(p.sizeX - g.x0, (uint32_t)(kStripBlocks * kBlock)); g.ry = (uint32_t)kBlock;
      g.pix = reinterpret_cast<uint32_t *>(lds + kLdsStrip); g.V = reinterpret_cast<float *>(lds + LL.v); g.blk = reinterpret_cast<BlkF *>(lds + LL.blk);
      g.calls = reinterpret_cast<uint32_t *>(lds + LL.calls); g.trialc = reinterpret_cast<int *>(lds + LL.trialc);
      const int lane = g.lane;

      uint32_t recVal[2] = { 0u, 0u };
      request_prefit_records(p, g, recVal);
      stage_strip_pixels(p, io, g);
      __syncthreads();
      take_prefit_records<false>(p, g, recVal, nullptr);
      phase_e_view<CH, FAST, true>(g);
      uint32_t *s_queue = g.calls + 4;
      if (tid == 0) *s_queue = 0;
      __syncthreads();

      uint32_t waveWords = 0;
      auto grab = [&]() -> uint32_t { uint32_t v = 0; if (lane == 0) v = atomicAdd(s_queue, 1u); return (uint32_t)sgpr((int)v); };
      uint32_t sbNext = grab();
#pragma unroll 1
      for (;;)
      {
        const uint32_t sb = sbNext;
        if (sb >= (uint32_t)kStripBlocks) break;
        uint32_t qv = 0;
        if (lane == 0) qv = atomicAdd(s_queue, 1u);
        uint32_t rx, n, lx, ly;
        if (!block_geom(p, g, sb, rx, n)) { sbNext = (uint32_t)sgpr((int)qv); continue; }
        const BlkF *const blkE = g.blk + sb;
        uint32_t shift[3] = { 0, 0, 0 };
        if (p.forced[0] >= 0) { shift[0] = (uint32_t)p.forced[0]; shift[1] = (uint32_t)p.forced[1]; shift[2] = (uint32_t)p.forced[2]; }
        else if (crushBits)
        {
          const uint32_t px = block_pixel(g, sb, rx, n, lx, ly);
          uint32_t fA, fB, fC;
          pixel_factors<CH, FAST>(reinterpret_cast<const BlkE *>(blkE), px, fA, fB, fC);
          if (!((uint32_t)sgpr((int)blkE->flags) & kBig))
          {
            TrialState t;
            t.fA = fA; t.fB = fB; t.fC = fC;
            const uint32_t R = px & 0xFF, G = (px >> 8) & 0xFF;
            t.hiRG = (R + 0x8000u) | ((G + 0x8000u) << 16);
            t.loRG = (R + 0x8000u - 255u) | ((G + 0x8000u - 255u) << 16);
            t.pxB = (int)((px >> 16) & 0xFF);
            t.pxBlo = t.pxB - 255;
            const int *tc = g.trialc + sb * kTrialConstDw;
#pragma unroll
            for (int c = 0; c < 3; c++)
            {
              t.nA[c] = tc[c]; t.nB[c] = tc[3 + c]; t.nC[c] = tc[6 + c];
              t.mA[c] = tc[9 + c]; t.mB[c] = tc[12 + c]; t.mC[c] = tc[15 + c];
            }
            t.mA[0] += (int)(R << 8); t.mA[1] += (int)(G << 8); t.mA[2] += t.pxB << 8;
            search_fast_automaton<true>(t, true, maxPixel32, blockLimit, shift);
          }
          else
          {
            const uint32_t packed = (uint32_t)sgpr((int)search_generic(px, fA, fB, fC, blkE->rec, true, maxPixel32, st->maxBlock * 64ull, true));
            shift[0] = packed & 0xFF; shift[1] = (packed >> 8) & 0xFF; shift[2] = (packed >> 16) & 0xFF;
          }
        }
#pragma unroll
        for (int k = 0; k < 3; k++)
        {
          const uint32_t sk = shift[k];
          if (sk < 8u) waveWords += 8u - sk;
          else if (CH == 4 && sgpr((int)blkE->rec[8 * k + 3]) != sgpr((int)blkE->rec[8 * k + 7])) waveWords += 8u;
        }
        sbNext = (uint32_t)sgpr((int)qv);
      }
      if (lane == 0) g.calls[g.wave] = waveWords;
      __syncthreads();
      if (tid == 0) atomicAdd(counter, (unsigned long long)(g.calls[0] + g.calls[1] + g.calls[2] + g.calls[3]));
    }

    template <int CH, bool FAST>
    __global__ __launch_bounds__(kThreads, 6) void k_rate_probe(const RateProbeParams p)
    {
      __shared__ __attribute__((aligned(16))) uint8_t lds[lds_layout<true>().total];
      rate_probe_strip<CH, FAST>(p, p.io, p.state, p.counter, lds, blockIdx.x % p.stripsX, blockIdx.x / p.stripsX, blockIdx.x / p.stripsX);
    }

    __global__ void k_rate_begin_batch(RateDevice *d, unsigned long long *counters, const RateBudgetChunk budgets, const uint32_t hLo, const uint32_t hHi)
    {
      const uint32_t i = threadIdx.x;
      if (i >= budgets.n) return;
      d[i].search = rate_begin(hLo, hHi, budgets.maxBytes[i]);
      d[i].listNext = 0u;
      set_thresholds(d + i, 2u * hHi);
      counters[i] = 0ull;
    }

    __global__ void k_rate_step_batch(RateDevice *d, unsigned long long *counters, const uint32_t nImages, const unsigned long long fixedBytes)
    {
      const uint32_t i = blockIdx.x * blockDim.x + threadIdx.x;
      if (i >= nImages) return;
      const unsigned long long bytes = fixedBytes + 8ull * counters[i];
      counters[i] = 0ull;
      if (d[i].search.done) return;
      rate_step(d[i].search, bytes);
      if (!d[i].search.done) set_thresholds(d + i, 2u * d[i].search.next);
    }

    template <int CH, bool FAST>
    __global__ __launch_bounds__(kThreads, 6) void k_rate_probe_batch(const RateProbeBatchParams p)
    {
      __shared__ __attribute__((aligned(16))) uint8_t lds[lds_layout<true>().total];
      const uint32_t img = blockIdx.x / p.imageStrips, local = blockIdx.x - img * p.imageStrips;
      typedef const __attribute__((address_space(4))) ImageIO KernIO;
      KernIO *const io = (KernIO *)p.batch + img;
      const uint32_t by = local / p.stripsX;
      rate_probe_strip<CH, FAST>(p, *io, p.states + img, p.counters + img, lds, local - by * p.stripsX, by, img * p.blocksY + by);
    }
  }

  void launch_rate_begin(RateDevice *dState, unsigned long long *dCounter, const RateState &first, uint32_t firstErrorFactor, hipStream_t s)
  {
    hipLaunchKernelGGL(k_rate_begin, dim3(1), dim3(1), 0, s, dState, dCounter, first, firstErrorFactor);
  }

  void launch_rate_step(RateDevice *dState, unsigned long long *dCounter, uint64_t fixedBytes, const uint32_t *dList, unsigned long long *dListBytes, uint32_t listCount,
                        hipStream_t s)
  {
    hipLaunchKernelGGL(k_rate_step, dim3(1), dim3(1), 0, s, dState, dCounter, (unsigned long long)fixedBytes, dList, dListBytes, listCount);
  }

  void launch_rate_probe(const RateProbeParams &p, int channels, bool floatFast, hipStream_t s)
  {
    const dim3 grid(p.stripsX * p.blocksY), block(kThreads);
    with_flags([&](auto rgba, auto fast) { hipLaunchKernelGGL((k_rate_probe<rgba ? 4 : 3, fast>), grid, block, 0, s, p); }, channels == 4, floatFast);
  }

  void launch_rate_begin_batch(RateDevice *dStates, unsigned long long *dCounters, const uint64_t *hMaxBytes, size_t count, uint32_t hLo, uint32_t hHi, hipStream_t s)
  {
    for (size_t i0 = 0; i0 < count; i0 += 64)
    {
      RateBudgetChunk ch;
      ch.n = (uint32_t)(count - i0 < 64 ? count - i0 : 64);
      for (uint32_t i = 0; i < 64; i++) ch.maxBytes[i] = i < ch.n ? (unsigned long long)hMaxBytes[i0 + i] : 0ull;
      hipLaunchKernelGGL(k_rate_begin_batch, dim3(1), dim3(64), 0, s, dStates + i0, dCounters + i0, ch, hLo, hHi);
    }
  }

  void launch_rate_step_batch(RateDevice *dStates, unsigned long long *dCounters, uint32_t nImages, uint64_t fixedBytes, hipStream_t s)
  {
    hipLaunchKernelGGL(k_rate_step_batch, dim3((nImages + 63u) / 64u), dim3(64), 0, s, dStates, dCounters, nImages, (unsigned long long)fixedBytes);
  }

  void launch_rate_probe_batch(const RateProbeBatchParams &p, int channels, bool floatFast, hipStream_t s)
  {
    const dim3 grid(p.nImages * p.imageStrips), block(kThreads);
    with_flags([&](auto rgba, auto fast) { hipLaunchKernelGGL((k_rate_probe_batch<rgba ? 4 : 3, fast>), grid, block, 0, s, p); }, channels == 4, floatFast);
  }
}
```

limg_amd/csrc/limg_hip_stream_encode_api.hip:

```cpp
#include "limg_hip_context.h"

#include <algorithm>
#include <vector>

using namespace limg_hip;

namespace
{
  struct StreamShape
  {
    size_t sizeX, sizeY, px, planeStride, blocksX, blocksY, blocks, tiles, stripsX, strips, bound;
    uint64_t fixedBytes;
    bool whole;
    StreamShape(size_t x, size_t y)
      : sizeX(x), sizeY(y), px(x * y), planeStride((px + 255) & ~(size_t)255), blocksX((x + kBlock - 1) / kBlock), blocksY((y + kBlock - 1) / kBlock), blocks(blocksX * blocksY),
        tiles((blocks + 255) / 256), stripsX((blocksX + kStripBlocks - 1) / kStripBlocks), strips(stripsX * blocksY), bound(limg_hip_stream_bound(x, y)),
        fixedBytes(sizeof(limg_hip_stream_header) + (uint64_t)blocks * sizeof(limg_hip_stream_block)), whole((x % kBlock) == 0 && (y % kBlock) == 0) {}
  };

  bool batch_applies(const limg_hip_context *c, const StreamShape &sh) { return sh.whole && c->opt.force_split_kernels == 0 && c->opt.legacy_float_stage == 0; }
  bool rate_probe_applies(const limg_hip_context *c, const StreamShape &sh, int fast) { return batch_applies(c, sh) && fast != 0; }

  limg_hip_result check_single(const void *c, const void *pIn, bool pointers, const StreamShape &sh, const uint8_t *dStream = nullptr, size_t capacity = 0)
  {
    if (!c || !pIn || !pointers) return limg_hip_error_ArgumentNull;
    if (sh.bound == 0) return limg_hip_error_InvalidParameter;
    if (dStream && capacity < sh.bound) return limg_hip_error_OutOfBounds;
    if (((uintptr_t)dStream & 15u) != 0) return limg_hip_error_InvalidParameter;
    return limg_hip_success;
  }
  limg_hip_result check_list(const void *c, bool pointers, size_t count, const uint32_t *const *ppIn, uint8_t *const *ppStreams, const StreamShape &sh, size_t capacityEach,
                             bool deviceStreams)
  {
    if (!c || !ppIn || !ppStreams || !pointers) return limg_hip_error_ArgumentNull;
    for (size_t i = 0; i < count; i++)
      if (!ppIn[i] || !ppStreams[i]) return limg_hip_error_ArgumentNull;
    if (sh.bound == 0) return limg_hip_error_InvalidParameter;
    if (capacityEach < sh.bound) return limg_hip_error_OutOfBounds;
    for (size_t i = 0; deviceStreams && i < count; i++)
      if (((uintptr_t)ppStreams[i] & 15u) != 0) return limg_hip_error_InvalidParameter;
    return limg_hip_success;
  }

  limg_hip_result check_budgets(size_t count, const size_t *pMaxBytes, uint32_t minErrorFactor, uint32_t maxErrorFactor, const limg_hip_budget_result *pResults, uint32_t &hLo,
                                uint32_t &hHi)
  {
    const uint32_t lo = minErrorFactor ? minErrorFactor : 2u, hi = maxErrorFactor ? maxErrorFactor : 1024u;
    if ((lo & 1u) || (hi & 1u) || lo < 2u || hi < 2u || lo > hi) return limg_hip_error_InvalidParameter;
    for (size_t i = 0; i < count; i++)
      if (pMaxBytes[i] == 0 || pResults[i].struct_size < sizeof(limg_hip_budget_result)) return limg_hip_error_InvalidParameter;
    hLo = lo / 2u; hHi = hi / 2u;
    return limg_hip_success;
  }

  void fill_result(limg_hip_budget_result &res, uint32_t ef, uint32_t probes, uint32_t within, uint64_t bytes) { res.errorFactor = ef; res.probes = probes; res.withinBudget = within; res.bytes = bytes; }

  limg_hip_result download_sizes(const void *dSizes, size_t count, size_t *pBytes, hipStream_t s)
  {
    std::vector<unsigned long long> sizes(count);
    HIP_TRY(hipMemcpyAsync(sizes.data(), dSizes, count * 8, hipMemcpyDeviceToHost, s));
    HIP_TRY(hipStreamSynchronize(s));
    for (size_t i = 0; i < count; i++) pBytes[i] = (size_t)sizes[i];
    return limg_hip_success;
  }

  uint32_t stream_flags(const limg_hip_context *c, int fast) { return (fast ? 1u : 0u) | (c->opt.dither_pcg ? 2u : 0u); }
  uint32_t pack_waves(const limg_hip_context *c, size_t strips)
  {
    const size_t slots = (size_t)device_cus(c) * 16;
    return (uint32_t)(strips < slots ? strips : slots);
  }

  struct StagedList { std::vector<const uint32_t *> in; std::vector<uint8_t *> streams; size_t slice; };
  limg_hip_result stage_list(limg_hip_context *c, const StreamShape &sh, size_t count, const uint32_t *const *ppIn, StagedList &l)
  {
    HIP_TRY(hipSetDevice(c->device));
    l.slice = (sh.bound + 255) & ~(size_t)255;
    limg_hip_result r;
    if ((r = c->host.in.ensure(count * sh.px * 4)) != limg_hip_success) return r;
    if ((r = c->stream.buf.ensure(count * l.slice)) != limg_hip_success) return r;
    l.in.resize(count); l.streams.resize(count);
    for (size_t i = 0; i < count; i++)
    {
      l.in[i] = (const uint32_t *)c->host.in.p + i * sh.px;
      l.streams[i] = (uint8_t *)c->stream.buf.p + i * l.slice;
      HIP_TRY(hipMemcpy((void *)l.in[i], ppIn[i], sh.px * 4, hipMemcpyHostToDevice));
    }
    return limg_hip_success;
  }

  struct Probe
  {
    size_t n; int channels; bool floatFast; uint64_t fixedBytes;
    RateDevice *states; unsigned long long *counters;
    RateProbeParams one; RateProbeBatchParams many;
    void launch(hipStream_t s) const { if (n == 1) launch_rate_probe(one, channels, floatFast, s); else launch_rate_probe_batch(many, channels, floatFast, s); }
  };

  template <class P>
  void fill_probe(P &p, const limg_hip_context *c, const StreamShape &sh, bool aligned)
  {
    memset(&p, 0, sizeof(p));
    p.sizeX = (uint32_t)sh.sizeX; p.sizeY = (uint32_t)sh.sizeY; p.blocksX = (uint32_t)sh.blocksX; p.blocksY = (uint32_t)sh.blocksY; p.stripsX = (uint32_t)sh.stripsX;
    p.vecIn = (sh.sizeX % 4 == 0) && aligned;
    p.recordLimit = record_limit(c);
    forced_shifts(c->opt.forced_shift, p.forced);
    p.records = (const limg_hip_block_record *)c->enc.records.p; p.invN = (const float *)c->enc.invN.p;
  }

  limg_hip_result probe_setup(limg_hip_context *c, const StreamShape &sh, const uint32_t *const *ppIn, size_t n, int hasAlpha, int poolThreads, hipStream_t s, Probe &pr)
  {
    limg_hip_result r;
    if ((r = c->stream.rateState.ensure(n * sizeof(RateDevice))) != limg_hip_success) return r;
    if ((r = c->stream.rateCounter.ensure(n * 8)) != limg_hip_success) return r;
    std::vector<ImageIO> table(n > 1 ? n : 0);
    bool aligned = true;
    for (size_t i = 0; i < n; i++) { aligned = aligned && (((uintptr_t)ppIn[i]) & 15u) == 0; if (n > 1) table[i].in = ppIn[i]; }
    EncodeExtra x;
    x.fitOnly = true; x.fitFloatMode = true;
    if (n > 1) { x.batch = table.data(); x.batchCount = n; }
    if ((r = encode_device(c, ppIn[0], sh.sizeX, sh.sizeY, hasAlpha, nullptr, nullptr, 0, poolThreads, 1, s, x)) != limg_hip_success) return r;
    pr.n = n; pr.channels = hasAlpha ? 4 : 3; pr.floatFast = c->opt.float_mode == 1; pr.fixedBytes = sh.fixedBytes;
    pr.states = (RateDevice *)c->stream.rateState.p; pr.counters = (unsigned long long *)c->stream.rateCounter.p;
    fill_probe(pr.one, c, sh, aligned);
    pr.one.io.in = ppIn[0]; pr.one.state = pr.states; pr.one.counter = pr.counters;
    fill_probe(pr.many, c, sh, aligned);
    pr.many.batch = (const ImageIO *)c->enc.batchTable.p; pr.many.nImages = (uint32_t)n; pr.many.imageStrips = (uint32_t)sh.strips;
    pr.many.states = pr.states; pr.many.counters = pr.counters;
    return limg_hip_success;
  }

  limg_hip_result run_searches(limg_hip_context *c, const StreamShape &sh, const uint32_t *const *ppIn, const size_t *budgets, size_t n, uint32_t hLo, uint32_t hHi,
                               int hasAlpha, int poolThreads, hipStream_t s, RateDevice *hStates)
  {
    Probe pr;
    const limg_hip_result r = probe_setup(c, sh, ppIn, n, hasAlpha, poolThreads, s, pr);
    if (r != limg_hip_success) return r;
    if (n == 1) launch_rate_begin(pr.states, pr.counters, rate_begin(hLo, hHi, budgets[0]), 2u * hHi, s);
    else launch_rate_begin_batch(pr.states, pr.counters, budgets, n, hLo, hHi, s);
    for (uint32_t i = 0, probes = rate_max_probes(hLo, hHi); i < probes; i++)
    {
      pr.launch(s);
      if (n == 1) launch_rate_step(pr.states, pr.counters, pr.fixedBytes, nullptr, nullptr, 0, s);
      else launch_rate_step_batch(pr.states, pr.counters, (uint32_t)n, pr.fixedBytes, s);
    }
    HIP_TRY(hipGetLastError());
    HIP_TRY(hipMemcpyAsync(hStates, pr.states, n * sizeof(RateDevice), hipMemcpyDeviceToHost, s));
    HIP_TRY(hipStreamSynchronize(s));
    for (size_t i = 0; i < n; i++)
      if (!hStates[i].search.done) return limg_hip_error_Generic;
    return limg_hip_success;
  }
}

extern "C"
{
  limg_hip_result limg_hip_encode_stream_device(limg_hip_context *c, const uint32_t *pIn, size_t sizeX, size_t sizeY, int hasAlpha, uint8_t *pStream, size_t capacity,
                                                size_t *pBytes, uint32_t errorFactor, int poolThreads, int fastBitCrushing, void *stream)
  {
    const StreamShape sh(sizeX, sizeY);
    limg_hip_result r;
    if ((r = check_single(c, pIn, pStream != nullptr, sh, pStream, capacity)) != limg_hip_success) return r;
    HIP_TRY(hipSetDevice(c->device));
    hipStream_t s = (hipStream_t)stream;
    if ((r = c->stream.fac.ensure(sh.planeStride * 3)) != limg_hip_success) return r;
    const bool stripForm = sh.whole && c->opt.force_split_kernels == 0;
    if ((r = c->stream.tiles.ensure(sh.tiles * 4)) != limg_hip_success) return r;
    if (stripForm && (r = c->stream.units.ensure(sh.strips * 4)) != limg_hip_success) return r;
    if ((r = c->enc.records.ensure(sh.blocks * sizeof(limg_hip_block_record))) != limg_hip_success) return r;
    if ((r = c->enc.shifts.ensure(sh.blocks * 4)) != limg_hip_success) return r;
    limg_hip_encode3d_info info;
    memset(&info, 0, sizeof(info));
    info.pFactorsA = (uint8_t *)c->stream.fac.p; info.pFactorsB = info.pFactorsA + sh.planeStride; info.pFactorsC = info.pFactorsB + sh.planeStride;
    limg_hip_compact_out comp = { (limg_hip_block_record *)c->enc.records.p, (uint32_t *)c->enc.shifts.p };
    EncodeExtra xs;
    xs.streamRaw = true; xs.stripWords = stripForm ? (uint32_t *)c->stream.units.p : nullptr;
    if ((r = encode_device(c, pIn, sizeX, sizeY, hasAlpha, &info, &comp, errorFactor, poolThreads, fastBitCrushing, s, xs)) != limg_hip_success) return r;

    StreamParams sp;
    memset(&sp, 0, sizeof(sp));
    sp.sizeX = (uint32_t)sizeX; sp.sizeY = (uint32_t)sizeY; sp.blocksX = (uint32_t)sh.blocksX; sp.blocksY = (uint32_t)sh.blocksY;
    sp.nBlocks = (uint32_t)sh.blocks; sp.nTiles = (uint32_t)sh.tiles; sp.channels = hasAlpha ? 4 : 3; sp.errorFactor = errorFactor;
    sp.flags = stream_flags(c, fastBitCrushing);
    sp.fac[0] = info.pFactorsA; sp.fac[1] = info.pFactorsB; sp.fac[2] = info.pFactorsC;
    sp.records = comp.pRecords; sp.shifts = comp.pShifts;
    sp.stream = pStream; sp.tileBase = (uint32_t *)c->stream.tiles.p;
    if (stripForm)
    {
      sp.stripWords = (uint32_t *)c->stream.units.p;
      sp.stripsX = (uint32_t)sh.stripsX; sp.nStrips = (uint32_t)sh.strips;
      sp.nWaves = pack_waves(c, sh.strips);
    }
    mark(c, s);
    launch_stream_pack(sp, s);
    mark(c, s); mark(c, s); mark(c, s);
    HIP_TRY(hipGetLastError());
    return pBytes ? stream_total_bytes(pStream, s, pBytes) : limg_hip_success;
  }

  limg_hip_result limg_hip_encode_stream(limg_hip_context *c, const uint32_t *pIn, size_t sizeX, size_t sizeY, int hasAlpha, uint8_t *pStream, size_t capacity, size_t *pBytes,
                                         uint32_t errorFactor, int poolThreads, int fastBitCrushing)
  {
    const StreamShape sh(sizeX, sizeY);
    const limg_hip_result ok = check_single(c, pIn, pStream && pBytes, sh);
    if (ok != limg_hip_success) return ok;
    std::lock_guard<std::recursive_mutex> hostLock(c->hostEntry);
    return encode_stream_host(c, pIn, sizeX, sizeY, pStream, capacity, pBytes, sh.bound, [&](const uint32_t *dIn, uint8_t *dStream, size_t bound, size_t *bytes) {
      return limg_hip_encode_stream_device(c, dIn, sizeX, sizeY, hasAlpha, dStream, bound, bytes, errorFactor, poolThreads, fastBitCrushing, nullptr);
    });
  }

  limg_hip_result limg_hip_stream_sizes_device(limg_hip_context *c, const uint32_t *pIn, size_t sizeX, size_t sizeY, int hasAlpha, const uint32_t *pErrorFactors, size_t count,
                                               size_t *pBytes, int poolThreads, int fastBitCrushing, void *stream)
  {
    const StreamShape sh(sizeX, sizeY);
    limg_hip_result r;
    if ((r = check_single(c, pIn, pErrorFactors && pBytes, sh)) != limg_hip_success) return r;
    if (count == 0) return limg_hip_success;
    if (count > 0x7FFFFFFFull) return limg_hip_error_InvalidParameter;
    HIP_TRY(hipSetDevice(c->device));
    hipStream_t s = (hipStream_t)stream;
    if (!rate_probe_applies(c, sh, fastBitCrushing))
    {
      if ((r = c->stream.buf.ensure(sh.bound)) != limg_hip_success) return r;
      for (size_t i = 0; i < count; i++)
        if ((r = limg_hip_encode_stream_device(c, pIn, sizeX, sizeY, hasAlpha, (uint8_t *)c->stream.buf.p, sh.bound, &pBytes[i], pErrorFactors[i], poolThreads, fastBitCrushing,
                                               stream)) != limg_hip_success)
          return r;
      return limg_hip_success;
    }
    if ((r = c->stream.rateList.ensure(count * 12)) != limg_hip_success) return r;
    Probe pr;
    if ((r = probe_setup(c, sh, &pIn, 1, hasAlpha, poolThreads, s, pr)) != limg_hip_success) return r;
    unsigned long long *dBytes = (unsigned long long *)c->stream.rateList.p;
    uint32_t *dList = (uint32_t *)(dBytes + count);
    std::vector<uint32_t> list(pErrorFactors, pErrorFactors + count);
    HIP_TRY(hipMemcpyAsync(dList, list.data(), count * 4, hipMemcpyHostToDevice, s));
    launch_rate_begin(pr.states, pr.counters, rate_begin(0, 0, 0), list[0], s);
    for (size_t i = 0; i < count; i++)
    {
      pr.launch(s);
      launch_rate_step(pr.states, pr.counters, pr.fixedBytes, dList, dBytes, (uint32_t)count, s);
    }
    HIP_TRY(hipGetLastError());
    return download_sizes(dBytes, count, pBytes, s);
  }

  limg_hip_result limg_hip_stream_sizes(limg_hip_context *c, const uint32_t *pIn, size_t sizeX, size_t sizeY, int hasAlpha, const uint32_t *pErrorFactors, size_t count,
                                        size_t *pBytes, int poolThreads, int fastBitCrushing)
  {
    const StreamShape sh(sizeX, sizeY);
    limg_hip_result r;
    if ((r = check_single(c, pIn, pErrorFactors && pBytes, sh)) != limg_hip_success) return r;
    if (count == 0) return limg_hip_success;
    std::lock_guard<std::recursive_mutex> hostLock(c->hostEntry);
    HIP_TRY(hipSetDevice(c->device));
    if ((r = c->host.in.ensure(sh.px * 4)) != limg_hip_success) return r;
    HIP_TRY(hipMemcpy(c->host.in.p, pIn, sh.px * 4, hipMemcpyHostToDevice));
    r = limg_hip_stream_sizes_device(c, (const uint32_t *)c->host.in.p, sizeX, sizeY, hasAlpha, pErrorFactors, count, pBytes, poolThreads, fastBitCrushing, nullptr);
    return r != limg_hip_success ? r : limg_hip_check_device_status(c);
// ... 228 lines not shown
```

Measured before the change: 56270.

## Have fit kernel emit precomputed per-block view layout for prefit phase E

The fit kernel now writes a 256-byte per-block 'prefit view' that holds normalised/offset floats, inverse norms, flags, records and trial constants, arranged in 16-byte pieces interleaved per 64-block unit. The encode and rate kernels load this view with two coalesced uint4 loads per thread and place it straight into LDS. This removes the per-strip phase_e_view recomputation, the DPP big-flag reduction and one barrier in the prefit path. In exchange the fit kernel does more work and writes a larger scratch buffer, and a test hook for reading the view back is added.

```diff
diff --git a/include/limg_hip_test_hooks.h b/include/limg_hip_test_hooks.h
--- a/include/limg_hip_test_hooks.h
+++ b/include/limg_hip_test_hooks.h
@@ -31,6 +31,8 @@
 
 void limg_hip_test_live_resources(uint64_t out[5]);
 
+limg_hip_result limg_hip_test_copy_prefit_view(limg_hip_context *pCtx, void *pDst, size_t bytes);
+
 #ifdef __cplusplus
 }
 #endif
diff --git a/limg_amd/__init__.py b/limg_amd/__init__.py
--- a/limg_amd/__init__.py
+++ b/limg_amd/__init__.py
@@ -40,7 +40,7 @@
     "limg_hip_comm_unique_id", "limg_hip_comm_init", "limg_hip_comm_destroy", "limg_hip_comm_info", "limg_hip_gather_stream", "limg_hip_encode3d_single_chain_device",
     "limg_hip_encode3d_chain_device", "limg_hip_host_gather_offsets", "limg_hip_host_chain_bases",
 )
-TEST_ABI_SYMBOLS = ("limg_hip_default_test_options_sized", "limg_hip_set_test_options", "limg_hip_test_live_resources")
+TEST_ABI_SYMBOLS = ("limg_hip_default_test_options_sized", "limg_hip_set_test_options", "limg_hip_test_live_resources", "limg_hip_test_copy_prefit_view")
 COMM_ID_BYTES = 128
 
 BLOCKED_PLANES = (("pDecoded", np.uint32), ("pFactorsA", np.uint8), ("pFactorsB", np.uint8), ("pFactorsC", np.uint8), ("pBlockError", np.uint8), ("pBitsPerPixel", np.uint8),
@@ -180,6 +180,8 @@
         L.limg_hip_set_test_options.argtypes = [C.c_void_p, C.c_void_p]
         L.limg_hip_test_live_resources.restype = None
         L.limg_hip_test_live_resources.argtypes = [C.POINTER(C.c_uint64)]
+        L.limg_hip_test_copy_prefit_view.restype = C.c_int
+        L.limg_hip_test_copy_prefit_view.argtypes = [C.c_void_p, C.c_void_p, C.c_size_t]
     L.limg_hip_set_options.restype = C.c_int
     L.limg_hip_set_options.argtypes = [C.c_void_p, C.c_void_p]
     L.limg_hip_get_options.restype = C.c_int
@@ -454,6 +456,12 @@
     def has_test_hooks(self):
         return hasattr(self.lib, "limg_hip_set_test_options")
 
+    def prefit_view(self, blocks_x, rows):
+        units = (int(blocks_x) + 63) // 64
+        raw = np.zeros((int(rows), units, 16, 64, 4), dtype=np.uint32)
+        _check(self.lib.limg_hip_test_copy_prefit_view(self.ctx, _np_ptr(raw), raw.nbytes), "limg_hip_test_copy_prefit_view")
+        return np.ascontiguousarray(raw.transpose(0, 1, 3, 2, 4).reshape(int(rows), units * 64, 64)[:, :int(blocks_x)]).reshape(-1, 64)
+
     def get_options(self):
         o = Options()
         o.struct_size = C.sizeof(o)
diff --git a/limg_amd/csrc/limg_hip_api.hip b/limg_amd/csrc/limg_hip_api.hip
--- a/limg_amd/csrc/limg_hip_api.hip
+++ b/limg_amd/csrc/limg_hip_api.hip
@@ -56,6 +56,16 @@
   void limg_hip_test_live_resources(uint64_t out[5])
   {
     for (int i = 0; out && i < limg_hip_live::kCounts; i++) out[i] = limg_hip_live::count[i].load();
+  }
+
+  limg_hip_result limg_hip_test_copy_prefit_view(limg_hip_context *c, void *dst, size_t bytes)
+  {
+    if (!c || !dst) return limg_hip_error_ArgumentNull;
+    if (bytes > c->enc.view.cap) return limg_hip_error_InvalidParameter;
+    HIP_TRY(hipSetDevice(c->device));
+    HIP_TRY(hipDeviceSynchronize());
+    if (bytes) HIP_TRY(hipMemcpy(dst, c->enc.view.p, bytes, hipMemcpyDeviceToHost));
+    return limg_hip_success;
   }
 #endif
 
diff --git a/limg_amd/csrc/limg_hip_context.h b/limg_amd/csrc/limg_hip_context.h
--- a/limg_amd/csrc/limg_hip_context.h
+++ b/limg_amd/csrc/limg_hip_context.h
@@ -31,7 +31,7 @@
   {
     Bytes &n;
     DevBuf records{ n }, shifts{ n }, stripCalls{ n }, stripBase{ n };
-    DevBuf invN{ n };
+    DevBuf view{ n };
     DevBuf park{ n };
     DevBuf batchTable{ n };
     Stream fitStream;
diff --git a/limg_amd/csrc/limg_hip_encode.hip b/limg_amd/csrc/limg_hip_encode.hip
--- a/limg_amd/csrc/limg_hip_encode.hip
+++ b/limg_amd/csrc/limg_hip_encode.hip
@@ -119,8 +119,8 @@
     else { if ((r = c->enc.records.ensure(scratchBlocks * sizeof(limg_hip_block_record))) != limg_hip_success) return r; p.records = (limg_hip_block_record *)c->enc.records.p + blockOff; }
     if (compact && compact->pShifts) p.shifts = compact->pShifts + blockOff;
     else { if ((r = c->enc.shifts.ensure(scratchBlocks * 4)) != limg_hip_success) return r; p.shifts = (uint32_t *)c->enc.shifts.p + blockOff; }
-    if ((r = c->enc.invN.ensure(scratchBlocks * 16)) != limg_hip_success) return r;
-    p.invN = (float *)c->enc.invN.p + blockOff * 4;
+    if ((r = c->enc.view.ensure(scratchRows * view_row_chunks(p.blocksX) * 16)) != limg_hip_success) return r;
+    p.view = (uint4 *)c->enc.view.p + x.scratchRow0 * view_row_chunks(p.blocksX);
     if ((r = c->enc.stripCalls.ensure(scratchStrips * 4)) != limg_hip_success) return r;
     if ((r = c->enc.stripBase.ensure(scratchStrips * 4)) != limg_hip_success) return r;
     p.stripCalls = (uint32_t *)c->enc.stripCalls.p + stripOff; p.stripBase = (uint32_t *)c->enc.stripBase.p + stripOff;
@@ -244,7 +244,7 @@
       const size_t i0 = k == 0 ? 0 : firstSub + (k - 1) * subImages, want = k == 0 ? firstSub : subImages, n = batchCount - i0 < want ? batchCount - i0 : want;
       q.batch = p.batch + i0; q.batchCount = (uint32_t)n;
       q.io = e.x.batch[i0];
-      q.records = p.records + i0 * imgBlocks; q.shifts = p.shifts + i0 * imgBlocks; q.invN = p.invN + i0 * imgBlocks * 4;
+      q.records = p.records + i0 * imgBlocks; q.shifts = p.shifts + i0 * imgBlocks; q.view = p.view + i0 * p.blocksY * view_row_chunks(p.blocksX);
       if (p.stripWords) q.stripWords = p.stripWords + i0 * imgStrips;
       uint8_t *lb = (uint8_t *)c->enc.lookback.p + k * 16 + i0 * imgStrips * 8;
       q.ticket = (uint32_t *)lb; q.desc = (unsigned long long *)(lb + 16);
diff --git a/limg_amd/csrc/limg_hip_encode_ragged.hip b/limg_amd/csrc/limg_hip_encode_ragged.hip
--- a/limg_amd/csrc/limg_hip_encode_ragged.hip
+++ b/limg_amd/csrc/limg_hip_encode_ragged.hip
@@ -93,7 +93,7 @@
     q.sizeY = (uint32_t)(((size_t)r1 * kBlock < e.sizeY ? (size_t)r1 * kBlock : e.sizeY) - y0);
     q.blocksY = r1 - r0;
     q.imageStrips = q.stripsX * q.blocksY;
-    q.records += (size_t)r0 * p.blocksX; q.shifts += (size_t)r0 * p.blocksX; q.invN += (size_t)r0 * p.blocksX * 4;
+    q.records += (size_t)r0 * p.blocksX; q.shifts += (size_t)r0 * p.blocksX; q.view += (size_t)r0 * view_row_chunks(p.blocksX);
     q.stripCalls += (size_t)r0 * p.stripsX; q.stripBase += (size_t)r0 * p.stripsX;
     return q;
   }
diff --git a/limg_amd/csrc/limg_hip_fit_tpb.hip b/limg_amd/csrc/limg_hip_fit_tpb.hip
--- a/limg_amd/csrc/limg_hip_fit_tpb.hip
+++ b/limg_amd/csrc/limg_hip_fit_tpb.hip
@@ -1,4 +1,6 @@
 #include "limg_hip_device.h"
+#include "limg_hip_search.h"
+#include "limg_hip_float_pixel.h"
 
 namespace limg_hip
 {
@@ -57,7 +59,7 @@
       const unsigned short *tab = reinterpret_cast<const unsigned short *>(s_tab);
       uint32_t *s_px = s_pxAll[wave];
       const uint32_t unitsX = (p.blocksX + 63u) / 64u;
-      const uint32_t unitId = blockIdx.x * kTpbWaves + wave;
+      const uint32_t unitId = (uint32_t)sgpr((int)(blockIdx.x * kTpbWaves + wave));
       if (unitId >= unitsX * p.blocksY * p.batchCount) return;
       const uint32_t unit = unitId % unitsX, byS = unitId / unitsX;
       const uint32_t img = p.batchCount > 1 ? byS / p.blocksY : 0u, by = byS - img * p.blocksY;
@@ -231,7 +233,11 @@
       uint32_t words[16];
 #pragma unroll
       for (int c = 0; c < 4; c++) words[c] = __float_as_uint(comp(avg, c));
+      uint4 *const viewUnit = p.view + (size_t)byS * view_row_chunks(p.blocksX) + (size_t)unit * (kViewUnit * kViewChunks);
+      auto view_piece = [&](int k) -> uint4 & { return (viewUnit + (k & ~3) * kViewUnit)[(uint32_t)(lane + (k & 3) * kViewUnit)]; };
       float inv[3];
+      int mRest[3][2];
+      int recMax = 0, recMin = 0;
 #pragma unroll
       for (int r = 0; r < 3; r++)
       {
@@ -263,11 +269,27 @@
         words[5 + 4 * r] = (uint32_t)(uint16_t)lo[2] | ((uint32_t)(uint16_t)lo[3] << 16);
         words[6 + 4 * r] = (uint32_t)(uint16_t)hi[0] | ((uint32_t)(uint16_t)hi[1] << 16);
         words[7 + 4 * r] = (uint32_t)(uint16_t)hi[2] | ((uint32_t)(uint16_t)hi[3] << 16);
-      }
+        float nf[4], of[4];
+#pragma unroll
+        for (int c = 0; c < 4; c++)
+        {
+          nf[slot_of(c)] = (float)((int)hi[c] - (int)lo[c]); of[slot_of(c)] = (float)(int)lo[c];
+          recMax = max(recMax, max((int)lo[c], (int)hi[c])); recMin = min(recMin, min((int)lo[c], (int)hi[c]));
+        }
+        view_piece(r) = make_uint4(__float_as_uint(nf[0]), __float_as_uint(nf[1]), __float_as_uint(nf[2]), __float_as_uint(nf[3]));
+        view_piece(3 + r) = make_uint4(__float_as_uint(of[0]), __float_as_uint(of[1]), __float_as_uint(of[2]), __float_as_uint(of[3]));
+        view_piece(8 + r) = make_uint4(words[4 + 4 * r], words[5 + 4 * r], words[6 + 4 * r], words[7 + 4 * r]);
+        view_piece(12 + r) = make_uint4((uint32_t)((int)lo[0] - (int)hi[0]), (uint32_t)((int)lo[1] - (int)hi[1]), (uint32_t)((int)lo[2] - (int)hi[2]), (uint32_t)term_const(r, 0, (int)lo[0]));
+        mRest[r][0] = term_const(r, 1, (int)lo[1]); mRest[r][1] = term_const(r, 2, (int)lo[2]);
+      }
+      view_piece(6) = make_uint4(__float_as_uint(inv[0]), __float_as_uint(inv[1]), __float_as_uint(inv[2]), (uint32_t)mRest[2][0]);
+      const bool big = recMax > p.recordLimit || recMin < -p.recordLimit;
+      view_piece(7) = make_uint4((uint32_t)mRest[2][1], 0u, kValid | (big ? kBig : 0u), 64u);
+      view_piece(11) = make_uint4(0u, 0u, 0u, 0u);
+      view_piece(15) = make_uint4((uint32_t)mRest[0][0], (uint32_t)mRest[0][1], (uint32_t)mRest[1][0], (uint32_t)mRest[1][1]);
       uint4 *dst = reinterpret_cast<uint4 *>(p.records + (size_t)byS * p.blocksX + bx0 + lane);
 #pragma unroll
       for (int i = 0; i < 4; i++) dst[i] = make_uint4(words[4 * i], words[4 * i + 1], words[4 * i + 2], words[4 * i + 3]);
-      reinterpret_cast<float4 *>(p.invN)[(size_t)byS * p.blocksX + bx0 + lane] = make_float4(inv[0], inv[1], inv[2], 0.0f);
     }
   }
 
diff --git a/limg_amd/csrc/limg_hip_float_pixel.h b/limg_amd/csrc/limg_hip_float_pixel.h
--- a/limg_amd/csrc/limg_hip_float_pixel.h
+++ b/limg_amd/csrc/limg_hip_float_pixel.h
@@ -24,9 +24,34 @@
       float nrm[3][4];
       float off[3][4];
       float invN[3];
+      int tcx[2];
     };
     static_assert(sizeof(BlkE) <= 120, "BlkE must fit the dead float-stage fields");
     static_assert(sizeof(BlkF) == 192, "BlkF layout");
+
+    constexpr int kTrialConstDw = 16;
+    struct PrefitView
+    {
+      BlkF blk;
+      int tc[kTrialConstDw];
+    };
+    static_assert(sizeof(PrefitView) == kViewChunks * 16, "a block's view is whole 16-byte pieces, 256 bytes");
+    static_assert(offsetof(BlkF, flags) == 120 && offsetof(BlkF, rec) == 128 && offsetof(BlkF, pad) == 176, "the pieces k_fit_tpb writes");
+    struct TrialConsts { int n[3][3], m[3][3]; };
+    __device__ __forceinline__ TrialConsts load_trial_consts(const int *tc, const BlkF *blk)
+    {
+      TrialConsts t;
+#pragma unroll
+      for (int f = 0; f < 3; f++)
+      {
+#pragma unroll
+        for (int c = 0; c < 3; c++) t.n[f][c] = tc[4 * f + c];
+        t.m[f][0] = tc[4 * f + 3];
+      }
+      t.m[0][1] = tc[12]; t.m[0][2] = tc[13]; t.m[1][1] = tc[14]; t.m[1][2] = tc[15];
+      t.m[2][1] = reinterpret_cast<const BlkE *>(blk)->tcx[0]; t.m[2][2] = reinterpret_cast<const BlkE *>(blk)->tcx[1];
+      return t;
+    }
 
     struct EStrip
     {
diff --git a/limg_amd/csrc/limg_hip_internal.h b/limg_amd/csrc/limg_hip_internal.h
--- a/limg_amd/csrc/limg_hip_internal.h
+++ b/limg_amd/csrc/limg_hip_internal.h
@@ -17,6 +17,8 @@
   constexpr int kStripBlocks = 32;
   constexpr int kThreads = 256;
   constexpr int kWaves = 4;
+  constexpr int kViewChunks = 16, kViewUnit = 64;
+  __host__ __device__ inline size_t view_row_chunks(uint32_t blocksX) { return (size_t)((blocksX + kViewUnit - 1) / kViewUnit) * kViewUnit * kViewChunks; }
   constexpr int kBlocksPerWave = 8;
   constexpr uint64_t kDitherSeed = 0xCA7F00D15BADF00DULL;
 
@@ -49,7 +51,7 @@
     int32_t recordLimit;
     uint32_t chainCount, chainRows;
     limg_hip_block_record *records;
-    float *invN;
+    uint4 *view;
     uint32_t *shifts;
     uint32_t *stripCalls;
     uint32_t *stripBase;
@@ -308,7 +310,7 @@
     int32_t recordLimit;
     int32_t forced[3];
     const limg_hip_block_record *records;
-    const float *invN;
+    const uint4 *view;
     const RateDevice *state;
     unsigned long long *counter;
   };
@@ -325,7 +327,7 @@
     int32_t recordLimit;
     int32_t forced[3];
     const limg_hip_block_record *records;
-    const float *invN;
+    const uint4 *view;
     const RateDevice *states;
     unsigned long long *counters;
   };
diff --git a/limg_amd/csrc/limg_hip_kernels.hip b/limg_amd/csrc/limg_hip_kernels.hip
--- a/limg_amd/csrc/limg_hip_kernels.hip
+++ b/limg_amd/csrc/limg_hip_kernels.hip
@@ -83,12 +83,23 @@
       g.calls = reinterpret_cast<uint32_t *>(lds + LL.calls); g.trialc = reinterpret_cast<int *>(lds + LL.trialc);
       const int lane = g.lane;
 
-      uint32_t recVal[2] = { 0u, 0u };
-      if (PREFIT) request_prefit_records(p, g, recVal);
-      stage_strip_pixels(p, io, g);
-      __syncthreads();
-      if (PREFIT) take_prefit_records<PERSIST>(p, g, recVal, park);
+      uint32_t *s_queue = g.calls + 4;
+      if (PREFIT)
+      {
+        uint4 view[2];
+        request_prefit_view(p, g, view);
+        stage_strip_pixels(p, io, g);
+        place_prefit_view(g, view);
+        if (tid == 0) *s_queue = 0;
+        __syncthreads();
+        if (PERSIST) park_prefit_records(g, park);
+      }
       else
+      {
+        stage_strip_pixels(p, io, g);
+        __syncthreads();
+      }
+      if (!PREFIT)
       {
       const unsigned short *s_rsq = d_rsqrt_x86_tab;
       const int lane = g.lane, wave = g.wave;
@@ -313,10 +324,12 @@
     
       }
       if (!PERSIST && p.fitOnly) return;
-      phase_e_view<CH, FAST, PREFIT>(g);
-      uint32_t *s_queue = g.calls + 4;
-      if (tid == 0) *s_queue = 0;
-      __syncthreads();
+      if (!PREFIT)
+      {
+        phase_e_view<CH, FAST>(g);
+        if (tid == 0) *s_queue = 0;
+        __syncthreads();
+      }
 
       uint8_t *stage = reinterpret_cast<uint8_t *>(g.V);
       uint32_t waveCalls = 0;
@@ -359,12 +372,12 @@
             t.pxBlo = t.pxB - 255;
             if (PREFIT)
             {
-              const int *tc = g.trialc + sb * kTrialConstDw;
+              const TrialConsts k = load_trial_consts(g.trialc + sb * kTrialConstDw, blkE);
 #pragma unroll
               for (int c = 0; c < 3; c++)
               {
-                t.nA[c] = tc[c]; t.nB[c] = tc[3 + c]; t.nC[c] = tc[6 + c];
-                t.mA[c] = tc[9 + c]; t.mB[c] = tc[12 + c]; t.mC[c] = tc[15 + c];
+                t.nA[c] = k.n[0][c]; t.nB[c] = k.n[1][c]; t.nC[c] = k.n[2][c];
+                t.mA[c] = k.m[0][c]; t.mB[c] = k.m[1][c]; t.mC[c] = k.m[2][c];
               }
             }
             else
diff --git a/limg_amd/csrc/limg_hip_phase_e.h b/limg_amd/csrc/limg_hip_phase_e.h
--- a/limg_amd/csrc/limg_hip_phase_e.h
+++ b/limg_amd/csrc/limg_hip_phase_e.h
@@ -13,7 +13,6 @@
     constexpr int kLdsBlk = kLdsV + kLdsVBytes, kLdsCalls = kLdsBlk + kStripBlocks * 192, kLdsTotal = kLdsCalls + 32;
     static_assert(kLdsTotal <= 32768 - 16, "5 workgroups per CU");
     struct LdsLayout { int v, blk, calls, trialc, total; };
-    constexpr int kTrialConstDw = 20;
     template <bool PREFIT> __device__ __host__ constexpr LdsLayout lds_layout()
     {
       if (!PREFIT) return LdsLayout{ kLdsV, kLdsBlk, kLdsCalls, kLdsV, kLdsTotal };
@@ -28,16 +27,13 @@
 
 
     template <class P>
-    __device__ __forceinline__ void request_prefit_records(const P &p, const EStrip g, uint32_t recVal[2])
+    __device__ __forceinline__ void request_prefit_view(const P &p, const EStrip g, uint4 view[2])
     {
-#pragma unroll
-      for (int r = 0; r < 2; r++)
-      {
-        const int b = r * 4 + (g.lane >> 4), w = g.lane & 15;
-        const uint32_t bx = g.strip * kStripBlocks + g.wave * kBlocksPerWave + b;
-        if (bx < p.blocksX) recVal[r] = w >= 4 ? reinterpret_cast<const uint32_t *>(p.records + (size_t)g.byS * p.blocksX + bx)[w]
-                                               : reinterpret_cast<const uint32_t *>(p.invN)[((size_t)g.byS * p.blocksX + bx) * 4 + w];
-      }
+      static_assert(kStripBlocks * kViewChunks == 2 * kThreads && kViewUnit == 2 * kStripBlocks && kThreads / kStripBlocks == kViewChunks / 2, "two pieces per thread");
+      const uint32_t b = (uint32_t)g.tid & (kStripBlocks - 1), k = (uint32_t)g.tid / kStripBlocks;
+      const uint4 *src = p.view + (size_t)g.byS * view_row_chunks(p.blocksX) + (size_t)(g.strip >> 1) * (kViewUnit * kViewChunks) + (g.strip & 1u) * kStripBlocks + (k * kViewUnit + b);
+      view[0] = view[1] = make_uint4(0u, 0u, 0u, 0u);
+      if (g.strip * kStripBlocks + b < p.blocksX) { view[0] = src[0]; view[1] = src[(kViewChunks / 2) * kViewUnit]; }
     }
 
     template <class P, class IO>
@@ -67,34 +63,26 @@
       }
     }
 
-    template <bool PERSIST, class P>
-    __device__ __forceinline__ void take_prefit_records(const P &p, const EStrip g, const uint32_t recVal[2], uint8_t *park)
+    __device__ __forceinline__ void place_prefit_view(const EStrip g, const uint4 view[2])
     {
-      BlkF *blk = g.blk + g.wave * kBlocksPerWave;
-#pragma unroll
-      for (int r = 0; r < 2; r++)
-      {
-        const int b = r * 4 + (g.lane >> 4), w = g.lane & 15;
-        const uint32_t sb = g.wave * kBlocksPerWave + b, bx = g.strip * kStripBlocks + sb;
-        const uint32_t val = recVal[r];
-        if (w < 3) reinterpret_cast<BlkE *>(&blk[b])->invN[w] = __uint_as_float(val);
-        if (w >= 4)
-        {
-          reinterpret_cast<uint32_t *>(blk[b].rec)[w - 4] = val;
-          if (PERSIST) reinterpret_cast<uint32_t *>(park + kParkRec)[sb * 12 + (w - 4)] = val;
-        }
-        const int lo = (int)(int16_t)(val & 0xFFFFu), hi = (int)(int16_t)(val >> 16);
-        uint32_t big = (w >= 4 && (lo > p.recordLimit || lo < -p.recordLimit || hi > p.recordLimit || hi < -p.recordLimit)) ? 1u : 0u;
-        big |= (uint32_t)dpp<0xB1, 0xF>(0, (int)big);
-        big |= (uint32_t)dpp<0x4E, 0xF>(0, (int)big);
-        big |= (uint32_t)dpp<0x141, 0xF>(0, (int)big);
-        big |= (uint32_t)dpp<0x140, 0xF>(0, (int)big);
-        if (w == 0) { blk[b].flags = (bx < p.blocksX ? kValid : 0u) | (big ? kBig : 0u); blk[b].n = bx < p.blocksX ? 64u : 0u; }
-      }
-      wave_lds_fence();
+      const int b = g.tid & (kStripBlocks - 1), k = g.tid / kStripBlocks;
+      uint8_t *blk = reinterpret_cast<uint8_t *>(g.blk + b) + k * 16;
+      *reinterpret_cast<uint4 *>(blk) = view[0];
+      if (g.wave < 2) *reinterpret_cast<uint4 *>(blk + 8 * 16) = view[1];
+      else *reinterpret_cast<uint4 *>(g.trialc + b * kTrialConstDw + (k - 4) * 4) = view[1];
     }
 
-    template <int CH, bool FAST, bool PREFIT>
+    __device__ __forceinline__ void park_prefit_records(const EStrip g, uint8_t *park)
+    {
+      static_assert(kStripBlocks * 3 <= kThreads && sizeof(BlkF::rec) == 48, "three pieces per block");
+      if (g.tid < kStripBlocks * 3)
+      {
+        const int sb = g.tid / 3, k = g.tid - sb * 3;
+        reinterpret_cast<uint4 *>(park + kParkRec)[g.tid] = *reinterpret_cast<const uint4 *>(reinterpret_cast<const uint8_t *>(g.blk[sb].rec) + k * 16);
+      }
+    }
+
+    template <int CH, bool FAST>
     __device__ __forceinline__ void phase_e_view(const EStrip g)
     {
       const int lane = g.lane;
@@ -107,7 +95,6 @@
         const int b = idx / 12, fc = idx - b * 12, f = fc >> 2, c = fc & 3;
         const int lo = blk[b].rec[f * 8 + c], hi = blk[b].rec[f * 8 + 4 + c];
         nrm[r] = (float)(hi - lo); off[r] = (float)lo;
-        if (PREFIT) { invn[r] = 0.0f; continue; }
         const float sq = nrm[r] * nrm[r];
         const float s0 = __int_as_float(dpp<0x00, 0xF>(0, __float_as_int(sq))), s1 = __int_as_float(dpp<0x55, 0xF>(0, __float_as_int(sq)));
         const float s2 = __int_as_float(dpp<0xAA, 0xF>(0, __float_as_int(sq))), s3 = __int_as_float(dpp<0xFF, 0xF>(0, __float_as_int(sq)));
@@ -126,13 +113,7 @@
           const int b = idx / 12, fc = idx - b * 12, f = fc >> 2, c = fc & 3;
           BlkE *e = reinterpret_cast<BlkE *>(&blk[b]);
           e->nrm[f][slot_of(c)] = nrm[r]; e->off[f][slot_of(c)] = off[r];
-          if (!PREFIT && c == 0) e->invN[f] = invn[r];
-          if (PREFIT && c < 3)
-          {
-            int *tc = g.trialc + (g.wave * kBlocksPerWave + b) * kTrialConstDw;
-            tc[f * 3 + c] = -(int)nrm[r];
-            tc[9 + f * 3 + c] = term_const(f, c, (int)off[r]);
-          }
+          if (c == 0) e->invN[f] = invn[r];
         }
       }
     }
diff --git a/limg_amd/csrc/limg_hip_rate.hip b/limg_amd/csrc/limg_hip_rate.hip
--- a/limg_amd/csrc/limg_hip_rate.hip
+++ b/limg_amd/csrc/limg_hip_rate.hip
@@ -54,13 +54,11 @@
       g.calls = reinterpret_cast<uint32_t *>(lds + LL.calls); g.trialc = reinterpret_cast<int *>(lds + LL.trialc);
       const int lane = g.lane;
 
-      uint32_t recVal[2] = { 0u, 0u };
-      request_prefit_records(p, g, recVal);
+      uint32_t *s_queue = g.calls + 4;
+      uint4 view[2];
+      request_prefit_view(p, g, view);
       stage_strip_pixels(p, io, g);
-      __syncthreads();
-      take_prefit_records<false>(p, g, recVal, nullptr);
-      phase_e_view<CH, FAST, true>(g);
-      uint32_t *s_queue = g.calls + 4;
+      place_prefit_view(g, view);
       if (tid == 0) *s_queue = 0;
       __syncthreads();
 
@@ -93,12 +91,12 @@
             t.loRG = (R + 0x8000u - 255u) | ((G + 0x8000u - 255u) << 16);
             t.pxB = (int)((px >> 16) & 0xFF);
             t.pxBlo = t.pxB - 255;
-            const int *tc = g.trialc + sb * kTrialConstDw;
+            const TrialConsts k = load_trial_consts(g.trialc + sb * kTrialConstDw, blkE);
 #pragma unroll
             for (int c = 0; c < 3; c++)
             {
-              t.nA[c] = tc[c]; t.nB[c] = tc[3 + c]; t.nC[c] = tc[6 + c];
-              t.mA[c] = tc[9 + c]; t.mB[c] = tc[12 + c]; t.mC[c] = tc[15 + c];
+              t.nA[c] = k.n[0][c]; t.nB[c] = k.n[1][c]; t.nC[c] = k.n[2][c];
+              t.mA[c] = k.m[0][c]; t.mB[c] = k.m[1][c]; t.mC[c] = k.m[2][c];
             }
             t.mA[0] += (int)(R << 8); t.mA[1] += (int)(G << 8); t.mA[2] += t.pxB << 8;
             search_fast_automaton<true>(t, true, maxPixel32, blockLimit, shift);
diff --git a/limg_amd/csrc/limg_hip_stream_encode_api.hip b/limg_amd/csrc/limg_hip_stream_encode_api.hip
--- a/limg_amd/csrc/limg_hip_stream_encode_api.hip
+++ b/limg_amd/csrc/limg_hip_stream_encode_api.hip
@@ -105,7 +105,7 @@
     p.vecIn = (sh.sizeX % 4 == 0) && aligned;
     p.recordLimit = record_limit(c);
     forced_shifts(c->opt.forced_shift, p.forced);
-    p.records = (const limg_hip_block_record *)c->enc.records.p; p.invN = (const float *)c->enc.invN.p;
+    p.records = (const limg_hip_block_record *)c->enc.records.p; p.view = (const uint4 *)c->enc.view.p;
   }
 
   limg_hip_result probe_setup(limg_hip_context *c, const StreamShape &sh, const uint32_t *const *ppIn, size_t n, int hasAlpha, int poolThreads, hipStream_t s, Probe &pr)
```

Result: no change. 55990 (-0.5%).
